# szpajder/dumpvdl2

Measured on AMD Instinct MI355X. Metric: IQ MS/s demodulated end-to-end, higher is better.
Workload: dtype f32

## Files before the change

dumpvdl2_amd/csrc/debug_hooks.inc:

```

static bool hip_ok(hipError_t e) { return e == hipSuccess; }
template<typename T> static bool dbg_up(const DevBuf<T> &d, const void *src, size_t bytes) { return hip_ok(hipMemcpy(d, src, bytes, hipMemcpyHostToDevice)); }
template<typename T> static bool dbg_up(const DevBuf<T> &d, const void *src) { return dbg_up(d, src, d.bytes()); }
template<typename T> static bool dbg_fill(const DevBuf<T> &d, int v) { return hip_ok(hipMemset(d, v, d.bytes())); }
template<typename T> static bool dbg_down(void *dst, const DevBuf<T> &d, size_t bytes) { return hip_ok(hipMemcpy(dst, d, bytes, hipMemcpyDeviceToHost)); }
template<typename T> static bool dbg_down(void *dst, const DevBuf<T> &d) { return dbg_down(dst, d, d.bytes()); }
static bool dbg_tables(const DevBuf<Tables> &d) { auto tab = std::make_unique<Tables>(); build_tables(*tab); return dbg_up(d, tab.get()); }

template<int K> static int prof_read(const void *symbol, unsigned long long *out, int reset) {
	unsigned long long h[64][K];
	if(hipMemcpyFromSymbol(h, symbol, sizeof h) != hipSuccess) return -3;
	for(int k = 0; k < K; k++) { out[k] = 0; for(int s = 0; s < 64; s++) out[k] += h[s][k]; }
	if(reset) { memset(h, 0, sizeof h); if(hipMemcpyToSymbol(symbol, h, sizeof h) != hipSuccess) return -3; }
	return 0;
}

extern "C" {

int vdl2hip_debug_live_resources(long long out[3]) {
	if(!out) return VDL2HIP_E_INVAL;
	for(int i = 0; i < 3; i++) out[i] = hostmem::g_live[i].load();
	return VDL2HIP_OK;
}

int vdl2hip_debug_option(vdl2hip_ctx *c, const char *name, long value) {
	if(!c || !name) return VDL2HIP_E_INVAL;
	OnDevice dev_guard(c);
	int r = collect_pending(c);
	if(r != VDL2HIP_OK && r != VDL2HIP_E_OVERFLOW) return r;
	if(strcmp(name, "no_fuse") == 0) { c->fuse_k2 = value == 0; return VDL2HIP_OK; }
	if(strcmp(name, "force_timeout") == 0) { c->debug_force_timeout = value != 0; return VDL2HIP_OK; }
	if(strcmp(name, "force_mismatch") == 0) { c->debug_force_mismatch = value != 0; return VDL2HIP_OK; }
	if(strcmp(name, "walk_ahead_below") == 0) { c->walk_ahead_below = (double)value; c->walk_ahead_auto = true; return VDL2HIP_OK; }
	if(strcmp(name, "walk_ahead") == 0) { if(value != 0 && value != 1) return VDL2HIP_E_INVAL; c->walk_ahead = (int)value; c->walk_ahead_auto = false; return VDL2HIP_OK; }
	if(strcmp(name, "exact_tier") == 0) { if(value != 0 && value != 1) return VDL2HIP_E_INVAL; c->debug_exact_tier = (int)value; return VDL2HIP_OK; }
	if(strcmp(name, "screen_all") == 0) { c->debug_screen_all = value != 0; return VDL2HIP_OK; }
	if(strcmp(name, "force_again") == 0) { c->debug_force_again = value != 0; return VDL2HIP_OK; }
	if(strcmp(name, "referee") == 0) { if(value && !c->d_refhist) return VDL2HIP_E_INVAL; c->referee = value != 0; return VDL2HIP_OK; }
	if(strcmp(name, "ref_warm") == 0) { if(value < 0 || value > c->ref_T - 4096) return VDL2HIP_E_INVAL; c->ref_warm = value; return VDL2HIP_OK; }
	return VDL2HIP_E_INVAL;
}

int vdl2hip_debug_exact_window_many(vdl2hip_ctx *c, uint32_t chan, int64_t n_lo, int64_t n_hi, uint32_t count, int64_t stride, float *ms) {
	if(!c || !c->d_refhist || chan >= (uint32_t)c->C || c->feed_no == 0 || count == 0 || count > 65536) return VDL2HIP_E_INVAL;
	OnDevice dev_guard(c);
	int r = collect_pending(c);
	if(r != VDL2HIP_OK && r != VDL2HIP_E_OVERFLOW) return r;
	DevBuf<int> d_out; std::vector<int> h(count, 0);
	if(!hip_ok(d_out.alloc(count))) return VDL2HIP_E_NOMEM;
	Event e0, e1;
	if(!hip_ok(e0.ensure()) || !hip_ok(e1.ensure())) return VDL2HIP_E_DEVICE;
	hipExtLaunchKernelGGL(k_ref_probe, dim3(count), dim3(64), 0, c->streams.front, e0, e1, 0, c->d_ref[(c->feed_no - 1) % kSlots].get(), (int)chan, c->C, n_lo, n_hi, stride, d_out.get());
	if(!hip_ok(hipStreamSynchronize(c->streams.front)) || !dbg_down(h.data(), d_out)) return VDL2HIP_E_DEVICE;
	if(ms) { float t = 0.f; (void)hipEventElapsedTime(&t, e0, e1); *ms = t; }
	int n = 0; for(int v : h) n += v;
	return n;
}
int vdl2hip_debug_scan_multi2(vdl2hip_ctx *c, const int32_t *chan, const int64_t *lo, const int64_t *hi, uint32_t count, int with_retry, float *ms) {
	if(!c || !c->d_refhist || c->feed_no == 0 || count == 0 || count > 65536 || !chan || !lo || !hi) return VDL2HIP_E_INVAL;
	OnDevice dev_guard(c);
	int r = collect_pending(c);
	if(r != VDL2HIP_OK && r != VDL2HIP_E_OVERFLOW) return r;
	std::vector<ScanReq> h(count);
	for(uint32_t i = 0; i < count; i++) { if(chan[i] < 0 || chan[i] >= c->C) return VDL2HIP_E_INVAL; h[i] = ScanReq{ chan[i], REF_CANDIDATE, lo[i], hi[i] }; }
	DevBuf<ScanReq> d_sq, d_rt; DevBuf<uint32_t> d_n;
	if(!hip_ok(d_sq.alloc(count)) || !hip_ok(d_n.alloc(2)) || !hip_ok(d_rt.alloc(kRetryScans))) return VDL2HIP_E_NOMEM;
	uint32_t before[8] = {0}, after[8] = {0};
	const uint32_t nn[2] = { count, 0u };
	Event e0, e1;
	if(!hip_ok(e0.ensure()) || !hip_ok(e1.ensure()) || !dbg_up(d_sq, h.data()) || !dbg_up(d_n, nn) || !dbg_down(before, c->d_refstats, sizeof before)) return VDL2HIP_E_DEVICE;
	RefChan *ref = c->d_ref[(c->feed_no - 1) % kSlots];
	launch_scans(c, c->streams.front, ref, 0xfffeu, d_sq, nullptr, d_n, count, c->k_total, with_retry ? d_rt.get() : nullptr, d_n + 1, e0, e1);
	if(!hip_ok(hipStreamSynchronize(c->streams.front)) || !dbg_down(after, c->d_refstats, sizeof after)) return VDL2HIP_E_DEVICE;
	if(ms) { float t = 0.f; (void)hipEventElapsedTime(&t, e0, e1); *ms = t; }
	return (int)(after[0] - before[0]);
}
int vdl2hip_debug_exact_window(vdl2hip_ctx *c, uint32_t chan, int64_t n_lo, int64_t n_hi) { return vdl2hip_debug_exact_window_many(c, chan, n_lo, n_hi, 1, 0, nullptr); }

int vdl2hip_debug_u8_levels(float out[512]) {
	DevBuf<float> d;
	if(!hip_ok(d.alloc(512))) return VDL2HIP_E_NOMEM;
	hipLaunchKernelGGL(k_u8_level_probe, dim3(1), dim3(256), 0, 0, d);
	return dbg_down(out, d) ? VDL2HIP_OK : VDL2HIP_E_DEVICE;
}

int vdl2hip_debug_s8_levels(float out[512]) {
	DevBuf<float> d;
	if(!hip_ok(d.alloc(512))) return VDL2HIP_E_NOMEM;
	hipLaunchKernelGGL(k_s8_level_probe, dim3(1), dim3(256), 0, 0, d);
	return dbg_down(out, d) ? VDL2HIP_OK : VDL2HIP_E_DEVICE;
}

int vdl2hip_debug_dpp_probe(const float in[64], float out[256]) {
	DevBuf<float> d_in, d_out;
	if(!hip_ok(d_in.alloc(64)) || !hip_ok(d_out.alloc(256))) return VDL2HIP_E_NOMEM;
	if(!dbg_up(d_in, in)) return VDL2HIP_E_DEVICE;
	hipLaunchKernelGGL(k_dpp_probe, dim3(1), dim3(64), 0, 0, (const float *)d_in, d_out);
	return dbg_down(out, d_out) ? VDL2HIP_OK : VDL2HIP_E_DEVICE;
}

int vdl2hip_debug_core_probe(int kind, const void *in, size_t n, void *out) {
	if(kind < 0 || kind >= PROBE_KINDS || !in || !out || n == 0 || n > (size_t)1 << 26) return VDL2HIP_E_INVAL;
	DevBuf<float> d_in, d_out; DevBuf<Tables> d_tab;
	if(!hip_ok(d_in.alloc(n * (size_t)core_probe_in_words(kind))) || !hip_ok(d_out.alloc(n * (size_t)core_probe_out_words(kind))) || !hip_ok(d_tab.alloc(1))) return VDL2HIP_E_NOMEM;
	if(!dbg_tables(d_tab) || !dbg_up(d_in, in) || !dbg_fill(d_out, 0)) return VDL2HIP_E_DEVICE;
	hipLaunchKernelGGL(k_core_probe, dim3((unsigned)((n + 255) / 256)), dim3(256), 0, 0, kind, (const float *)d_in, (uint32_t)n, d_out, (const Tables *)d_tab);
	return hip_ok(hipGetLastError()) && dbg_down(out, d_out) ? VDL2HIP_OK : VDL2HIP_E_DEVICE;
}

int vdl2hip_debug_burst_probe(int kind, const void *in, size_t n, unsigned grid, void *out, const uint32_t *freq, uint32_t nchan, const float *y, uint32_t ring_len,
		uint32_t cap_frames, uint32_t cap_pool, uint32_t guard_frames, uint32_t guard_pool, void *frames, uint8_t *pool, void *ctl, unsigned long long *cnt) {
	if(kind < 0 || kind >= BPROBE_KINDS || !in || n == 0 || n > (size_t)1 << 20 || grid == 0 || grid > 1024) return VDL2HIP_E_INVAL;
	const uint32_t nwaves = grid * (uint32_t)kBurstWaves;
	const bool burst = kind == BPROBE_BURST;
	size_t nin = 0, nout = 0;
	if(kind == BPROBE_WAVE) { nin = n * 64 * 4; nout = n * (size_t)kBProbeWaveOut * 4; }
// ... 407 lines not shown
```

dumpvdl2_amd/csrc/kernels.h:

```cpp
#pragma once
#include <hip/hip_runtime.h>
#include <type_traits>
#include "vdl2_core.h"
#include "design.h"

#ifndef VDL2_K1_UNROLL
#define VDL2_K1_UNROLL 5
#endif

#ifndef VDL2_K1_WAVES_PER_EU
#define VDL2_K1_WAVES_PER_EU 3
#endif

namespace vdl2 {

constexpr int kK1Unroll = VDL2_K1_UNROLL;
typedef float v2f __attribute__((ext_vector_type(2)));
typedef float v4f __attribute__((ext_vector_type(4)));

#ifndef VDL2_REF_PRIO
#define VDL2_REF_PRIO 3
#endif
#ifndef VDL2_K1_PRIO
#define VDL2_K1_PRIO 0
// ... 975 lines not shown
		const uint32_t r0 = (uint32_t)(nblk - 150) + tid;
		cf32 v[kFull + 1];
		#pragma unroll
		for(int k = 0; k <= kFull; k++) if(k < kFull || tid < kRest) v[k] = y[(r0 + kK3Threads * k) & a.mask];
		#pragma unroll
		for(int k = 0; k <= kFull; k++) if(k < kFull || tid < kRest) tile[tid + kK3Threads * k] = phase_fast(v[k]);
	} else {
		for(int j = tid; j < kK3Tile + 150; j += kK3Threads) {
			const int64_t t = nblk - 150 + j;
			tile[j] = (t < 0 || t >= a.k1) ? 0.f : phase_fast(y[(uint32_t)t & a.mask]);
		}
	}
	__syncthreads();
	const int s0 = 10 * kK3Share * (tid / 10) + tid % 10;
	constexpr int kEarlyPh = kScreenEarly + kK3Share - 1;
	float ph[kEarlyPh], d[kEarlyPh];
	#pragma unroll
	for(int k = 0; k < kEarlyPh; k++) ph[k] = tile[s0 + 10 * k];
	#pragma unroll
	for(int k = 1; k < kEarlyPh; k++) d[k] = ph[k] - ph[k - 1];
	#pragma unroll
	for(int q = 0; q < kK3Share; q++) {
		ScreenAcc acc;
		screen_begin(acc);
		screen_taps(&d[q], 1, kScreenEarly, acc);
		float ps = screen_value(acc, kScreenEarly);
		if(__any(ps < kScreenEarlyThr)) {
			float pl[kPreamble - kScreenEarly + 1], dl[kPreamble];
			#pragma unroll
			for(int j = 0; j <= kPreamble - kScreenEarly; j++) pl[j] = tile[s0 + 10 * (q + kScreenEarly - 1 + j)];
			#pragma unroll
			for(int j = 0; j < kPreamble - kScreenEarly; j++) dl[kScreenEarly + j] = pl[j + 1] - pl[j];
			screen_taps(dl, kScreenEarly, kPreamble, acc);
			ps = screen_value(acc, kPreamble);
		}
		verdict[s0 + 10 * q] = !(ps >= kScreenThr);
	}
	__syncthreads();
	constexpr int kWordsPerWave = (kK3Tile / 64) / (kK3Threads / 64);
	if(full_tile) {
		const int lane = tid & 63;
		const uint32_t w0 = (uint32_t)(nblk >> 6) + (uint32_t)__builtin_amdgcn_readfirstlane(tid >> 6) * kWordsPerWave;
		uint64_t *frow = a.flag + (size_t)c * (a.cap >> 6);
		const uint8_t *vrow = verdict + 64 * kWordsPerWave * (tid >> 6) + lane;
		const unsigned long long all = a.screen_all != 0 ? ~0ull : 0ull;
		uint8_t vb[kWordsPerWave];
		unsigned long long bits[kWordsPerWave];
		#pragma unroll
		for(int j = 0; j < kWordsPerWave; j++) vb[j] = vrow[64 * j];
		#pragma unroll
		for(int j = 0; j < kWordsPerWave; j++) bits[j] = __builtin_amdgcn_ballot_w64(vb[j] != 0) | all;
		if(lane == 0) {
			#pragma unroll
			for(int j = 0; j < kWordsPerWave; j++) frow[(w0 + j) & (a.mask >> 6)] = bits[j];
		}
		return;
	}
	#pragma unroll
	for(int j = 0; j < kWordsPerWave; j++) {
		const int word = (tid >> 6) * kWordsPerWave + j;
		const int64_t n = nblk + 64 * word + (tid & 63);
		const unsigned long long bits = __ballot(n < a.k1 && (verdict[64 * word + (tid & 63)] != 0 || a.screen_all != 0));
		if((tid & 63) == 0 && n < a.k1) a.flag[(size_t)c * (a.cap >> 6) + ((uint32_t)(n >> 6) & (a.mask >> 6))] = bits;
	}
}

constexpr int kK3bWordsPerLane = 4;
#ifdef VDL2_K3B_PROF
__device__ unsigned long long vdl2_k3b_prof[64][16];
#define K3B_BEGIN() unsigned k3b_t0_ = (unsigned)__builtin_readcyclecounter(), k3b_acc_[6] = {0, 0, 0, 0, 0, 0}, k3b_cnt_[3] = {0, 0, 0}
#define K3B_MARK(k) do { if(__builtin_amdgcn_readfirstlane(threadIdx.x >> 6) == 0) { const unsigned t_ = (unsigned)__builtin_readcyclecounter(); \
	k3b_acc_[k] += t_ - k3b_t0_; k3b_t0_ = t_; } } while(0)
#define K3B_COUNT(k, v) do { k3b_cnt_[k] += (unsigned)__builtin_amdgcn_readfirstlane((int)(v)); } while(0)
#define K3B_END() do { if(threadIdx.x == 0) { const int s_ = (blockIdx.x + blockIdx.y) & 63; for(int k_ = 0; k_ < 6; k_++) atomicAdd(&vdl2_k3b_prof[s_][k_], (unsigned long long)k3b_acc_[k_]); \
	atomicAdd(&vdl2_k3b_prof[s_][8], 1ull); for(int k_ = 0; k_ < 3; k_++) atomicAdd(&vdl2_k3b_prof[s_][9 + k_], (unsigned long long)k3b_cnt_[k_]); } } while(0)
#else
#define K3B_BEGIN() do {} while(0)
#define K3B_MARK(k) do {} while(0)
#define K3B_COUNT(k, v) do {} while(0)
#define K3B_END() do {} while(0)
#endif
template<bool FULL>
__global__ __launch_bounds__(256, 4) void k_sync_exact4(K3Args a) {
	if(blockIdx.x == 0 && blockIdx.y == 0 && threadIdx.x == 0) { reset_out_ctl(a.ctl, a.k5_waves); if(a.ref) *a.ref = a.refv; if(a.rq_n) { a.rq_n[0] = 0u; a.rq_n[1] = 0u; a.rq_n[2] = 0u; a.rq_n[4] = 0u; a.rq_n[5] = 0u; a.rq_n[6] = 0u; } }
	if(blockIdx.x == 0 && threadIdx.x == 0 && a.rq_flag) { a.rq_flag[blockIdx.y] = 0u; a.rq_bad[blockIdx.y].n = 0u; if(a.rq_flag2) a.rq_flag2[blockIdx.y] = 0u; }
	constexpr int kBack = 160, kSpan = kBack + 64;
	__shared__ float psh[4][64 + 6], fsh[4][64 + 6], esh[4][64 + 6], ash[4][64 + 6], bsh[4][64 + 6];
	__shared__ float phs[4][kSpan], e2s[4][kSpan];
	__shared__ uint64_t s_need[4][64 * kK3bWordsPerLane];
	__shared__ uint8_t s_fprev[4][64 * kK3bWordsPerLane];
	__shared__ uint16_t s_list[4][64 * kK3bWordsPerLane];
	const int c = blockIdx.y, lane = threadIdx.x & 63, wave = threadIdx.x >> 6;
	const cf32 *y = a.y + (size_t)c * a.cap;
	const uint64_t *flag = a.flag + (size_t)c * (a.cap >> 6);
	uint64_t *cand = a.cand + (size_t)c * (a.cap >> 6);
	const uint32_t wmask = a.mask >> 6;
	const Tables &T = *a.tab;
	const bool ref_on = a.ref != nullptr && a.ref_on != 0;
	const float ppm_thr = ref_on ? a.ppm_thr[c] : 0.f;
	const int64_t w0 = a.nbase >> 6, w1 = (a.k1 + 63) >> 6;
	const int64_t wb = w0 + ((int64_t)blockIdx.x * 4 + wave) * (64 * a.wpl);
	int nwork = 0;
	K3B_BEGIN();
	for(int g = 0; g < a.wpl; g++) {
		const int64_t w = wb + 64 * g + lane;
		uint64_t need = 0, fprev = 0, fpp = 0, f0 = 0;
		if(w < w1) {
			f0 = flag[(uint32_t)w & wmask];
			fprev = w > 0 ? flag[(uint32_t)(w - 1) & wmask] : 0ull;
			fpp = w > 1 ? flag[(uint32_t)(w - 2) & wmask] : 0ull;
			const uint64_t fnext = w + 1 < w1 ? flag[(uint32_t)(w + 1) & wmask] : 0ull;
			need = f0 | (f0 << 3) | (f0 >> 3) | (fprev >> 61) | (fnext << 61);
			const int64_t base = w << 6;
			if(a.k1 - 3 < base + 64) {
				const int64_t lo = a.k1 - 3 - base;
				need |= lo <= 0 ? ~0ull : (~0ull << lo);
			}
			if(a.k1 < base + 64) need &= (a.k1 - base <= 0) ? 0ull : (~0ull >> (64 - (a.k1 - base)));
			if(need == 0) cand[(uint32_t)w & wmask] = 0;
		}
		const uint64_t need_prev = fprev | (fprev << 3) | (fprev >> 3) | (fpp >> 61) | (f0 << 61);
		s_need[wave][64 * g + lane] = need; s_fprev[wave][64 * g + lane] = (uint8_t)(need_prev >> 58);
		const unsigned long long busy = __ballot(need != 0);
		if(need != 0) s_list[wave][nwork + __builtin_popcountll(busy & ((1ull << lane) - 1ull))] = (uint16_t)(64 * g + lane);
		nwork += __builtin_popcountll(busy);
	}
	WAVE_SYNC();
	K3B_MARK(0); if(wave == 0) K3B_COUNT(0, nwork);
	float *ps = psh[wave], *fs = fsh[wave], *es = esh[wave], *as = ash[wave], *bs = bsh[wave], *ph = phs[wave], *e2 = e2s[wave];
	#pragma unroll 1
	for(int it = 0; it < nwork; it++) {
		const int idx = (int)s_list[wave][it];
		const uint64_t needj = s_need[wave][idx];
		const uint32_t fprevj = s_fprev[wave][idx] & 63u;
		const int64_t wj = wb + idx, r0 = (wj << 6) - kBack;
		{
			cf32 yv[4]; bool in[4];
			#pragma unroll
			for(int k = 0; k < 4; k++) {
				const int64_t t = r0 + lane + 64 * k;
				in[k] = 64 * k + lane < kSpan && t >= 0 && t < a.k1;
				yv[k] = in[k] ? y[(uint32_t)t & a.mask] : cf32{0.f, 0.f};
			}
			#pragma unroll
			for(int k = 0; k < 4; k++) if(64 * k + lane < kSpan) {
				ph[64 * k + lane] = in[k] ? phase_of(yv[k]) : 0.f;
				e2[64 * k + lane] = in[k] ? yv[k].re * yv[k].re + yv[k].im * yv[k].im : -1.f;
			}
		}
		ps[6 + lane] = kPherrBig; if(lane < 6) ps[lane] = kPherrBig;
		WAVE_SYNC();
		K3B_MARK(1); if(wave == 0) { K3B_COUNT(1, __builtin_popcountll(needj) + __builtin_popcount(fprevj)); K3B_COUNT(2, 1 + (fprevj != 0)); }
		if(ref_on) {
			float ev[4];
			#pragma unroll
			for(int k = 0; k < 4; k++) {
				const int i = 64 * k + lane;
				ev[k] = 0.f;
				if(i >= 3 && i < kSpan) {
					const float m0 = e2[i], m1 = e2[i - 1], m2 = e2[i - 2], m3 = e2[i - 3];
					ev[k] = m0 < 0.f ? 0.f : ref_eps2_of(m0, fmaxf(m1, 0.f), fmaxf(m2, 0.f), fmaxf(m3, 0.f));
				}
			}
			WAVE_SYNC();
			#pragma unroll
			for(int k = 0; k < 4; k++) if(64 * k + lane < kSpan) e2[64 * k + lane] = ev[k];
			WAVE_SYNC();
		}
		K3B_MARK(2);
		#pragma unroll 1
		for(int round = 0; round < 2; round++) {
			const int bit = round == 0 ? lane : lane - 6;
			const bool todo = round == 0 ? ((needj >> lane) & 1ull) != 0 : (lane < 6 && ((fprevj >> lane) & 1u) && (wj << 6) + bit >= 0);
			if(todo) {
				const int i0 = bit + kBack - 150;
				float p[kPreamble];
				#pragma unroll
				for(int i = 0; i < kPreamble; i++) p[i] = ph[i0 + 10 * i];
				float pv, fv, E = 0.f, pa, pb;
				if(ref_on) sync_metric_ref(p, e2 + i0, 10, T, pv, fv, E, pa, pb, FULL);
				else { sync_metric(p, T, pv, fv); pa = pb = pv; }
				ps[6 + bit] = pv; fs[6 + bit] = fv; es[6 + bit] = E; as[6 + bit] = pa; bs[6 + bit] = pb;
			}
			K3B_MARK(3 + round);
		}
		WAVE_SYNC();
		const int64_t n = (wj << 6) + lane;
		const float p0 = ps[6 + lane], p3 = ps[3 + lane], p6 = ps[lane];
		int vd = 0;
		if(n >= 3 && n < a.k1) {
			if(!ref_on) vd = is_candidate(p3, p0) ? 1 : 0;
			else vd = ref_candidate_verdict(ref_pherr_range(p0, as[6 + lane], bs[6 + lane], es[6 + lane]), ref_pherr_range(p3, as[3 + lane], bs[3 + lane], es[3 + lane]), fs[3 + lane], es[3 + lane],
			                                ref_pherr_range(p6, as[lane], bs[lane], es[lane]), a.max_ppm, ppm_thr);
		}
		if((needj >> lane) & 1ull) a.pf[(size_t)c * a.cap + ((uint32_t)n & a.mask)] = cf32{ (vd & 2) ? -p0 : p0, fs[6 + lane] };
		const unsigned long long bits = __ballot((vd & 1) != 0);
		if(lane == 0) cand[(uint32_t)wj & wmask] = bits;
		if(a.pq) {
			const unsigned long long mk = __ballot((vd & 2) != 0 && ((needj >> lane) & 1ull) != 0);
			if(mk && lane == 0) {
				const int64_t nf = (wj << 6) + __builtin_ctzll(mk), nl = (wj << 6) + 63 - __builtin_clzll(mk);
				int64_t lo = (nf - kRefPre) & ~255ll, hi = (nl + kRefPost) | 255; if(lo < 0) lo = 0; if(hi > a.k1 - 1) hi = a.k1 - 1;
				const uint32_t i = atomicAdd(a.rq_n + 3, 1u);
				if(i < a.pq_cap) a.pq[i] = ScanReq{ c, REF_CANDIDATE, lo, hi };
			}
		}
		WAVE_SYNC();
		K3B_MARK(5);
	}
	K3B_END();
}

constexpr int kK3dEvals = 320;
constexpr int kK3dFlush = kK3dEvals - 64;
constexpr int kK3dList = kK3dFlush + 256;
constexpr int kK3dMinGroups = 2048;
constexpr int kK3dGroup = 4;
constexpr int kK3dRounds = 32;
static_assert(kK3dEvals >= 70 && kK3dEvals <= 512 && kK3dList * 70 < (1 << 20) && kK3dList < (1 << 11) && kK3dRounds * 256 <= (1 << 16),
              "tile map: 9 bits of word, 7 of position; list head: 11 bits of words, 21 of evaluations; 16 bits of word index");
#define K3D_BARRIER() do { __builtin_amdgcn_fence(__ATOMIC_RELEASE, "workgroup", "local"); __builtin_amdgcn_s_barrier(); __builtin_amdgcn_fence(__ATOMIC_ACQUIRE, "workgroup", "local"); } while(0)
template<bool FULL>
__global__ __launch_bounds__(256, 4) void k_sync_dense(K3Args a) {
	if(blockIdx.x == 0 && blockIdx.y == 0 && threadIdx.x == 0) { reset_out_ctl(a.ctl, a.k5_waves); if(a.ref) *a.ref = a.refv; if(a.rq_n) { a.rq_n[0] = 0u; a.rq_n[1] = 0u; a.rq_n[2] = 0u; a.rq_n[4] = 0u; a.rq_n[5] = 0u; a.rq_n[6] = 0u; } }
	if(blockIdx.x == 0 && threadIdx.x == 0 && a.rq_flag) { a.rq_flag[blockIdx.y] = 0u; a.rq_bad[blockIdx.y].n = 0u; if(a.rq_flag2) a.rq_flag2[blockIdx.y] = 0u; }
	__shared__ uint64_t s_need[kK3dList], s_cbits[kK3dList], s_mbits[kK3dList];
	__shared__ uint32_t s_end[kK3dList];
	__shared__ uint16_t s_word[kK3dList];
	__shared__ uint8_t s_fprev[kK3dList];
	__shared__ uint16_t s_map[kK3dEvals];
	__shared__ float s_res[5][kK3dEvals];
	__shared__ uint8_t s_neg[kK3dEvals];
	__shared__ uint32_t s_head, s_r1;
	__shared__ uint64_t s_flag[256 * kK3dGroup + 3];
	const int c = blockIdx.y, tid = threadIdx.x, lane = threadIdx.x & 63;
	const cf32 *y = a.y + (size_t)c * a.cap;
	const uint64_t *flag = a.flag + (size_t)c * (a.cap >> 6);
	uint64_t *cand = a.cand + (size_t)c * (a.cap >> 6);
	const uint32_t wmask = a.mask >> 6;
	const Tables &T = *a.tab;
	const bool ref_on = a.ref != nullptr && a.ref_on != 0;
	const float ppm_thr = ref_on ? a.ppm_thr[c] : 0.f;
	const int64_t w0 = a.nbase >> 6, w1 = (a.k1 + 63) >> 6;
	const int64_t wb = w0 + (int64_t)blockIdx.x * (256 * a.wpl);
	K3B_BEGIN();
	if(tid == 0) s_head = 0u;
	K3D_BARRIER();
	#pragma unroll 1
	for(int g = 0; g < a.wpl; g++) {
		if(g % kK3dGroup == 0) {
			const int ng = a.wpl - g < kK3dGroup ? a.wpl - g : kK3dGroup;
			for(int i = tid; i < 256 * ng + 3; i += 256) {
				const int64_t w = wb + 256 * g - 2 + i;
				s_flag[i] = w >= 0 && w < w1 ? flag[(uint32_t)w & wmask] : 0ull;
			}
			K3D_BARRIER();
		}
		{
			const int64_t w = wb + 256 * g + tid;
			const int fi = 256 * (g % kK3dGroup) + tid;
			uint64_t need = 0, fprev = 0, fpp = 0, f0 = 0;
			if(w < w1) {
				f0 = s_flag[fi + 2]; fprev = s_flag[fi + 1]; fpp = s_flag[fi];
				const uint64_t fnext = s_flag[fi + 3];
				need = f0 | (f0 << 3) | (f0 >> 3) | (fprev >> 61) | (fnext << 61);
				const int64_t base = w << 6;
				if(a.k1 - 3 < base + 64) {
					const int64_t lo = a.k1 - 3 - base;
					need |= lo <= 0 ? ~0ull : (~0ull << lo);
				}
				if(a.k1 < base + 64) need &= (a.k1 - base <= 0) ? 0ull : (~0ull >> (64 - (a.k1 - base)));
				if(need == 0) cand[(uint32_t)w & wmask] = 0;
			}
			const uint64_t need_prev = fprev | (fprev << 3) | (fprev >> 3) | (fpp >> 61) | (f0 << 61);
			const uint32_t fp6 = w > 0 ? (uint32_t)(need_prev >> 58) : 0u;
			const uint32_t cnt = need != 0 ? (uint32_t)__builtin_popcountll(need) + (uint32_t)__builtin_popcount(fp6) : 0u;
			const uint32_t inc = cnt << 11 | (need != 0 ? 1u : 0u);
			uint32_t incl = inc;
			#pragma unroll
			for(int d = 1; d < 64; d <<= 1) { const uint32_t o = (uint32_t)__shfl_up((int)incl, d); if(lane >= d) incl += o; }
			const uint32_t tot = (uint32_t)__shfl((int)incl, 63);
			uint32_t at = 0;
			if(lane == 0 && tot != 0) at = atomicAdd(&s_head, tot);
			at = (uint32_t)__shfl((int)at, 0) + incl - inc;
			if(need != 0) {
				const uint32_t r = at & 2047u;
				s_need[r] = need; s_fprev[r] = (uint8_t)fp6; s_word[r] = (uint16_t)(256 * g + tid); s_end[r] = (at >> 11) + cnt;
				s_cbits[r] = 0ull; s_mbits[r] = 0ull;
			}
		}
		K3D_BARRIER();
		const uint32_t head = s_head;
		K3D_BARRIER();
		const int nrec = (int)(head & 2047u);
		K3B_MARK(0);
		if((int)(head >> 11) < kK3dFlush && g + 1 < a.wpl) continue;
		K3B_COUNT(0, nrec); K3B_COUNT(1, head >> 11);
		#pragma unroll 1
		for(int r0 = 0; r0 < nrec; ) {
			const uint32_t e0 = r0 ? s_end[r0 - 1] : 0u;
			if(tid == 0) s_r1 = (uint32_t)r0 + 1u;
			K3D_BARRIER();
			{
				uint32_t best = 0;
				for(int r = r0 + 1 + tid; r < nrec && r < r0 + kK3dEvals; r += 256) if(s_end[r] - e0 <= (uint32_t)kK3dEvals) best = (uint32_t)r + 1u;
				if(best) atomicMax(&s_r1, best);
			}
// ... 213 lines not shown
	const cf32 *y; NfState *nf; EvalChunk *log; uint32_t *nlog; int64_t *sc_first; int64_t *sc_cum;
	NfFeed *feed; float *lpbuf; float *ring; uint32_t ring_mask; uint32_t cap, mask, cap_log, cap_comb, cap_hist; int32_t nchan;
};

constexpr int kNfWaves = 4;
__global__ __launch_bounds__(64 * kNfWaves, 4) void k_nf_prepare(K4bArgs a) {
	extern __shared__ __align__(16) unsigned char nf_lds[];
	NfShared *shw = reinterpret_cast<NfShared *>(nf_lds);
	const int wave = threadIdx.x >> 6, c = blockIdx.x * kNfWaves + wave;
	if(c >= a.nchan) return;
	EvalLog lg{ a.log + (size_t)c * a.cap_log, a.nlog + c };
	NfScratch sc{ a.sc_first + (size_t)c * (a.cap_comb + 1), a.sc_cum + (size_t)c * (a.cap_comb + 1) };
	nf_prepare(&a.nf[c], lg, sc, a.cap_comb, &a.feed[c], shw[wave]);
}

__global__ __launch_bounds__(64 * kNfWaves, 4) void k_nf_replay(K4bArgs a) {
	extern __shared__ __align__(16) unsigned char nf_lds[];
	NfShared *shw = reinterpret_cast<NfShared *>(nf_lds);
	const int c = blockIdx.y, wave = threadIdx.x >> 6;
	ChanView v{ a.y + (size_t)c * a.cap, nullptr, nullptr, a.mask };
	NfScratch sc{ a.sc_first + (size_t)c * (a.cap_comb + 1), a.sc_cum + (size_t)c * (a.cap_comb + 1) };
	const NfFeed fd = a.feed[c];
	for(int64_t g = (int64_t)blockIdx.x * kNfWaves + wave; fd.u0 + 1 + kNfGroup * g <= fd.u1; g += (int64_t)gridDim.x * kNfWaves) {
		nf_replay_group(v, sc, fd, g, a.lpbuf + (size_t)c * a.cap_hist, a.cap_hist, shw[wave]);
		WAVE_SYNC();
	}
}

__global__ __launch_bounds__(64 * kNfWaves, 4) void k_nf_finish(K4bArgs a) {
	extern __shared__ __align__(16) unsigned char nf_lds[];
	NfShared *shw = reinterpret_cast<NfShared *>(nf_lds);
	const int wave = threadIdx.x >> 6, c = blockIdx.x * kNfWaves + wave;
	if(c >= a.nchan) return;
	NfScratch sc{ a.sc_first + (size_t)c * (a.cap_comb + 1), a.sc_cum + (size_t)c * (a.cap_comb + 1) };
	nf_finish(&a.nf[c], sc, a.feed[c], a.lpbuf + (size_t)c * a.cap_hist, a.ring + (size_t)c * (a.ring_mask + 1), a.ring_mask, a.cap_hist, shw[wave]);
}

__device__ __forceinline__ void nf_all_body(const K4bArgs &a, unsigned char *lds, int block) {
	NfShared *shw = reinterpret_cast<NfShared *>(lds);
	const int wave = threadIdx.x >> 6, c = block * kNfWaves + wave;
	if(c >= a.nchan) return;
	ChanView v{ a.y + (size_t)c * a.cap, nullptr, nullptr, a.mask };
	EvalLog lg{ a.log + (size_t)c * a.cap_log, a.nlog + c };
	NfScratch sc{ a.sc_first + (size_t)c * (a.cap_comb + 1), a.sc_cum + (size_t)c * (a.cap_comb + 1) };
	nf_prepare(&a.nf[c], lg, sc, a.cap_comb, &a.feed[c], shw[wave]);
	WAVE_SYNC_GLOBAL();
	const NfFeed fd = a.feed[c];
	for(int64_t g = 0; fd.u0 + 1 + kNfGroup * g <= fd.u1; g++) {
		nf_replay_group(v, sc, fd, g, a.lpbuf + (size_t)c * a.cap_hist, a.cap_hist, shw[wave]);
		WAVE_SYNC();
	}
	WAVE_SYNC_GLOBAL();
	nf_finish(&a.nf[c], sc, fd, a.lpbuf + (size_t)c * a.cap_hist, a.ring + (size_t)c * (a.ring_mask + 1), a.ring_mask, a.cap_hist, shw[wave]);
}
__global__ __launch_bounds__(64 * kNfWaves, 4) void k_nf_all(K4bArgs a) {
	extern __shared__ __align__(16) unsigned char nf_lds[];
	nf_all_body(a, nf_lds, (int)blockIdx.x);
}

struct K5Args {
	const cf32 *y; const Tables *tab; unsigned long long *cnt;
	const Burst *bursts; const uint32_t *nb_chan; uint32_t cap_bursts_chan; int32_t nchan;
	OutFrame *frames; uint8_t *pool; OutCtl *ctl; const uint32_t *freq;
	uint32_t cap, mask;
	RefChan *ref;
	uint32_t ref_launch;
	BurstDefer df;
};

constexpr int kScanLanes = 16, kScanProd = 8, kScanBlock = 64, kScanRow = kScanBlock + 4;
#ifndef VDL2_SCAN_WAVES
#define VDL2_SCAN_WAVES 11
#endif
constexpr int kScanWaves = VDL2_SCAN_WAVES;
struct ScanShared {
	alignas(16) float buf[2][2][kScanLanes][kScanRow];
	int64_t s_beg[kScanLanes], len[kScanLanes], n_lo[kScanLanes], n_hi[kScanLanes];
	uint32_t dphi[kScanLanes]; int32_t chan[kScanLanes], kind[kScanLanes]; uint32_t flags[kScanLanes];
	int64_t lmax, smin;
	v4f lut[256];
};
template<int FMT, int OS>
__global__ __launch_bounds__(64 * kScanWaves) void k_ref_scan_multi(RefChan *rp, uint32_t launch, const ScanReq *sq, const RefReq *rq, const uint32_t *n_ptr, uint32_t cap, int64_t k_end,
                      ScanReq *retry_q, uint32_t *retry_n, uint32_t retry_cap, int32_t warm_mul) {
#if VDL2_DEVICE_PASS
	#pragma clang fp contract(off)
	__shared__ ScanShared sh;
	constexpr int BLK = OS ? (kScanBlock / (OS ? OS : 1)) * OS : kScanBlock;
	const uint32_t ntot = *n_ptr < cap ? *n_ptr : cap;
	const uint32_t base = blockIdx.x * (uint32_t)kScanLanes;
	if(base >= ntot) return;
	const int wave = __builtin_amdgcn_readfirstlane(threadIdx.x >> 6), lane = threadIdx.x & 63;
	const int os = rp->os, npiece = rp->npiece;
	const uint32_t mask = rp->mask, cap_y = rp->cap;
	const int64_t warm = rp->warm * (int64_t)(warm_mul > 1 ? warm_mul : 1);
	int64_t ps0[kRefPieces], pn[kRefPieces]; const void *pp[kRefPieces];
	#pragma unroll
	for(int j = 0; j < kRefPieces; j++) { ps0[j] = j < npiece ? rp->piece[j].s0 : 0; pn[j] = j < npiece ? rp->piece[j].n : 0; pp[j] = j < npiece ? rp->piece[j].p : nullptr; }
	const float A0 = rp->A0, A1 = rp->A1, A2 = rp->A2;
	uint32_t *stats = rp->stats;
	static_assert(kScanLanes == 16, "four lanes of the first wavefront per request");
	if(threadIdx.x < 64) {
		const int r = threadIdx.x & (kScanLanes - 1), part = threadIdx.x >> 4;
		int64_t n_lo = 0, n_hi = -1, s_beg = 0, len = 0; int c = 0, kind = 0; uint32_t fl = 0;
		if(base + r < ntot && npiece > 0) {
			if(sq) { const ScanReq q = sq[base + r]; c = q.chan; kind = q.kind; n_lo = q.lo; n_hi = q.hi; }
			else { const RefReq q = rq[base + r]; c = q.chan; kind = q.kind; ref_request_window(q, k_end, n_lo, n_hi); }
			const int64_t in_end = ps0[npiece - 1] + pn[npiece - 1];
			if(n_lo < 0) n_lo = 0;
			if(kind == REF_STALE) kind = REF_CANDIDATE;
			bool go = n_hi >= n_lo;
			if(go) {
				const int64_t last = in_end / os - 1;
				n_lo &= ~255ll;
				if((n_hi | 255) <= last) n_hi |= 255; else if(n_hi < last) n_hi = last;
				const unsigned long long *done = rp->done + (size_t)c * kRefCache;
				const uint32_t ndv = rp->done_n[c], nd = ndv < (uint32_t)kRefCache ? ndv : (uint32_t)kRefCache;
				bool hit = false;
				for(uint32_t i = (uint32_t)part; i < nd; i += 4u) {
					const unsigned long long e = __hip_atomic_load(done + i, __ATOMIC_RELAXED, __HIP_MEMORY_SCOPE_AGENT);
					const int64_t lo = (int64_t)(e >> 32) << 8, hi = lo + ((int64_t)((e >> 16) & 0xffffull) << 8) + 255;
					hit = hit || (lo <= n_lo && n_hi <= hi && ref_entry_visible((uint32_t)(e & 0xffffull), launch));
				}
				int h = hit ? 1 : 0;
				h |= __shfl_xor(h, 16);
				h |= __shfl_xor(h, 32);
				hit = h != 0;
				if(hit) { if(part == 0) atomicAdd(stats + 1, 1u); go = false; }
			}
			if(go) {
				const int64_t s_end = (int64_t)os * (n_hi + 1);
				s_beg = (int64_t)os * n_lo - warm;
				bool refuse = in_end < s_end;
				if(s_beg < 0) s_beg = 0;
				else {
					if(ps0[0] > s_beg) { fl |= 2u; s_beg = (ps0[0] + os - 1) / os * os; }
					if(s_beg > 0 && (int64_t)os * n_lo - s_beg < rp->warm / 4) refuse = true;
				}
				if(refuse) { if(part == 0) atomicAdd(stats + 2, 1u); go = false; }
				else {
					s_beg -= s_beg % os;
					len = s_end - s_beg;
					if(rp->mix[c]) fl |= 1u;
				}
			}
			if(!go) len = 0;
		}
		if(part == 0) {
			sh.s_beg[r] = s_beg; sh.len[r] = len; sh.n_lo[r] = n_lo; sh.n_hi[r] = n_hi; sh.chan[r] = c; sh.kind[r] = kind; sh.flags[r] = fl;
			sh.dphi[r] = len ? rp->dphi[c] : 0u;
		}
	}
	__syncthreads();
	if(threadIdx.x < kScanLanes) {
		const int r = threadIdx.x;
		bool dup = false;
		for(int q = 0; q < r; q++) dup = dup || (sh.len[q] && sh.chan[q] == sh.chan[r] && sh.n_lo[q] == sh.n_lo[r] && sh.n_hi[q] >= sh.n_hi[r]);
		if(dup && sh.len[r]) { atomicAdd(stats + 1, 1u); sh.len[r] = 0; }
	}
	__syncthreads();
	if(threadIdx.x == 0) {
		int64_t m = 0, lo = INT64_MAX;
		for(int r = 0; r < kScanLanes; r++) { m = sh.len[r] > m ? sh.len[r] : m; if(sh.len[r] > 0 && sh.s_beg[r] < lo) lo = sh.s_beg[r]; }
		sh.lmax = m; sh.smin = lo;
		for(int r = 0; r < kScanLanes; r++) if(sh.len[r] <= 0) sh.s_beg[r] = lo;
	}
	__syncthreads();
	const int64_t lmax = sh.lmax;
	if(lmax <= 0) return;
	__builtin_amdgcn_s_setprio(3);
	const int64_t nblk = ((lmax + BLK - 1) / BLK + 2) / 4 * 4 + 1;
	for(int i = threadIdx.x; i < 256; i += blockDim.x) sh.lut[i] = ((ref_gf4 *)rp->lut)[i];
	__syncthreads();

	auto uni64 = [](int64_t v) -> int64_t { return (int64_t)(((uint64_t)(uint32_t)__builtin_amdgcn_readfirstlane((int)(v >> 32)) << 32) | (uint32_t)__builtin_amdgcn_readfirstlane((int)v)); };
	auto lds_barrier = [&]() { asm volatile("s_waitcnt lgkmcnt(0)\n\ts_barrier" ::: "memory"); };
	constexpr int NQ = kScanLanes / kScanProd;
	const int pidx = kScanWaves == 1 + kScanProd ? wave - 1 : (wave == 0 || (wave & 3) == 0) ? -1 : wave - 1 - (wave > 4) - (wave > 8);
	if(wave > 0 && pidx < 0) return;
	if(wave > 0) {
#if defined(VDL2_SCAN_EXP) && VDL2_SCAN_EXP == 3
		__builtin_amdgcn_s_setprio(1);
#endif
		const uint8_t *q_ptr[NQ]; uint32_t q_pend[NQ], q_ph0[NQ], q_len[NQ], q_dphi[NQ];
		int64_t q_beg[NQ];
		float pre[NQ], pim[NQ];
		constexpr int PF = 4;
		uint32_t wq[PF][NQ], wq2[PF][NQ];
		constexpr int SB = FMT == 2 ? 8 : FMT == 1 ? 4 : 2;
// ... 110 lines not shown
		static_assert(BLK % CH == 0 && CH % OS == 0, "chunks of whole decimation periods");
		(void)cnt;
		for(int64_t b = 0; b < nblk; b++) {
			const float *row = &sh.buf[b & 1][comp][r][0];
			v4f cur[NV], nxt[NV];
			#pragma unroll
			for(int j = 0; j < NV; j++) cur[j] = *reinterpret_cast<const v4f *>(row + 4 * j);
			#pragma unroll
			for(int j0 = 0; j0 < BLK; j0 += CH) {
				if(j0 + CH < BLK) {
					#pragma unroll
					for(int j = 0; j < NV; j++) nxt[j] = *reinterpret_cast<const v4f *>(row + j0 + CH + 4 * j);
				}
				#pragma unroll
				for(int j = 0; j < CH; j++) {
#if defined(VDL2_SCAN_EXP) && VDL2_SCAN_EXP == 2
					if(j) continue;
#endif
					const float m = b1 * y1;
					const float sm = m + t2;
					t2 = b2 * y1;
					y1 = cur[j >> 2][j & 3] + sm;
					if((j + 1) % OS == 0) {
						if(k_out >= my_lo && k_out <= my_hi) yout[2 * ((uint32_t)k_out & mask)] = y1;
						if(k_out == my_lo) { w_y1 = y1; w_t2 = t2; }
						k_out++;
					}
				}
				#pragma unroll
				for(int j = 0; j < NV; j++) cur[j] = nxt[j];
			}
			lds_barrier();
		}
	} else {
	constexpr int kChunk = 16;
	for(int64_t b = 0; b < nblk; b++) {
		const float *row = &sh.buf[b & 1][comp][r][0];
		v4f cur[kChunk / 4], nxt[kChunk / 4];
		#pragma unroll
		for(int j = 0; j < kChunk / 4; j++) cur[j] = *reinterpret_cast<const v4f *>(row + 4 * j);
		#pragma unroll
		for(int j0 = 0; j0 < BLK; j0 += kChunk) {
			if(j0 + kChunk < BLK) {
				#pragma unroll
				for(int j = 0; j < kChunk / 4; j++) nxt[j] = *reinterpret_cast<const v4f *>(row + j0 + kChunk + 4 * j);
			}
			#pragma unroll
			for(int j = 0; j < kChunk; j++) {
				const float m = b1 * y1;
				const float sm = m + t2;
				t2 = b2 * y1;
				y1 = cur[j >> 2][j & 3] + sm;
				if(__builtin_expect(++cnt == os, 0)) {
					cnt = 0;
					if(k_out >= my_lo && k_out <= my_hi) yout[2 * ((uint32_t)k_out & mask)] = y1;
					if(k_out == my_lo) { w_y1 = y1; w_t2 = t2; }
					k_out++;
				}
			}
			#pragma unroll
			for(int j = 0; j < kChunk / 4; j++) cur[j] = nxt[j];
		}
		lds_barrier();
	}
	}
	bool unmet = __float_as_uint(__shfl_xor(w_y1, 32)) != __float_as_uint(w_y1) || __float_as_uint(__shfl_xor(w_t2, 32)) != __float_as_uint(w_t2);
	unmet = unmet || __shfl_xor((int)unmet, kScanLanes) != 0;
	if(lane < kScanLanes && sh.len[r] > 0) {
		const int c = sh.chan[r];
		const int64_t n_lo = sh.n_lo[r], n_hi = sh.n_hi[r];
		bool listed = false;
		if(unmet && retry_q) {
			const uint32_t k = atomicAdd(retry_n, 1u);
			if(k < retry_cap) { retry_q[k] = ScanReq{ c, sh.kind[r], n_lo, n_hi }; listed = true; atomicAdd(stats + 10, 1u); }
		}
		if(unmet && !listed) atomicAdd(stats + 9, 1u);
		const uint32_t i = listed ? 0u : atomicAdd(rp->done_n + c, 1u);
		int64_t len = (n_hi - n_lo) >> 8; if(len > 0xffff) len = 0xffff;
		if(((n_hi + 1) & 255) != 0) len -= 1;
		if(listed) len = -1;
		if(len >= 0) __hip_atomic_store(rp->done + (size_t)c * kRefCache + (i % (uint32_t)kRefCache), ((unsigned long long)(n_lo >> 8) << 32) | ((unsigned long long)len << 16) | (unsigned long long)(launch & 0xffffu), __ATOMIC_RELAXED, __HIP_MEMORY_SCOPE_AGENT);
		atomicAdd(stats + 0, 1u); atomicAdd(stats + 4 + sh.kind[r], 1u);
		if(sh.flags[r] & 2u) atomicAdd(stats + 3, 1u);
	}
#else
	(void)rp; (void)launch; (void)sq; (void)rq; (void)n_ptr; (void)cap; (void)k_end;
#endif
}

#ifndef VDL2_K5_WAVES
#define VDL2_K5_WAVES 2
#endif
constexpr int kBurstWaves = VDL2_K5_WAVES;
constexpr int kK5MaxChan = 1024;
enum { BPROBE_WAVE = 0, BPROBE_RS, BPROBE_BURST, BPROBE_KINDS };
constexpr int kBProbeWaveOut = 68, kBProbeRsStride = 256;
struct BurstProbeArgs {
	uint32_t n; const Tables *tab; OutCtl *ctl;
	const uint32_t *win; uint32_t *wout;
	const uint8_t *rin; uint8_t *rout; int32_t *rret;
	const Burst *bursts; const uint32_t *freq; const cf32 *y; uint32_t cap, mask; unsigned long long *cnt; OutFrame *frames; uint8_t *pool;
};
__global__ __launch_bounds__(64 * kBurstWaves) void k_burst_probe_wave(BurstProbeArgs a) {
	extern __shared__ __align__(16) unsigned char k5_lds[];
	BurstShared &sh = reinterpret_cast<BurstShared *>(k5_lds)[threadIdx.x >> 6];
	const uint32_t wave_id = blockIdx.x * kBurstWaves + (threadIdx.x >> 6), nwaves = gridDim.x * kBurstWaves;
	burst_shared_init(*a.tab, wave_id, a.ctl, sh);
	for(uint32_t i = wave_id; i < a.n; i += nwaves) {
		const uint32_t *x = a.win + (size_t)i * 64;
		uint32_t *o = a.wout + (size_t)i * kBProbeWaveOut;
		WAVE_FOR(l)
			sh.lanek[l] = x[l]; sh.flag_err[l] = (int32_t)x[l];
		WAVE_END
		const int first = wave_first_flag(sh.flag_err), count = wave_count_flags(sh.flag_err);
		const uint32_t mn = wave_min64(sh.lanek);
		WAVE_SYNC();
		const uint32_t total = wave_excl_scan64(sh.lanek);
		WAVE_FOR(l)
			o[2 + l] = sh.lanek[l];
			if(l == 0) { o[0] = (uint32_t)first; o[1] = (uint32_t)count; o[66] = total; o[67] = mn; }
		WAVE_END
		WAVE_SYNC();
	}
}
__global__ __launch_bounds__(64 * kBurstWaves) void k_burst_probe_rs(BurstProbeArgs a) {
	extern __shared__ __align__(16) unsigned char k5_lds[];
	BurstShared &sh = reinterpret_cast<BurstShared *>(k5_lds)[threadIdx.x >> 6];
	const uint32_t wave_id = blockIdx.x * kBurstWaves + (threadIdx.x >> 6), nwaves = gridDim.x * kBurstWaves;
	burst_shared_init(*a.tab, wave_id, a.ctl, sh);
	for(uint32_t i = wave_id; i < a.n; i += nwaves) {
		const uint8_t *x = a.rin + (size_t)i * kBProbeRsStride;
		uint8_t *o = a.rout + (size_t)i * kBProbeRsStride;
		WAVE_FOR(l)
			for(int j = l; j < kRsN; j += 64) sh.tab[j] = x[j];
		WAVE_END
		[[clang::always_inline]] rs_decode_row(sh.tab, (int)x[kRsN], sh);
		WAVE_FOR(l)
			for(int j = l; j < kRsN; j += 64) o[j] = sh.tab[j];
			if(l == 0) a.rret[i] = sh.u_ret;
		WAVE_END
		WAVE_SYNC();
	}
}

__device__ __forceinline__ void burst_body(const K5Args &a, unsigned char *k5_lds, uint32_t block, uint32_t nblocks) {
	if((threadIdx.x >> 6) >= kBurstWaves) return;
	BurstShared &sh = reinterpret_cast<BurstShared *>(k5_lds)[threadIdx.x >> 6];
	uint32_t *bb = reinterpret_cast<uint32_t *>(k5_lds + sizeof(BurstShared) * kBurstWaves) + (size_t)(threadIdx.x >> 6) * (kK5MaxChan + 1);
	const int lane = threadIdx.x & 63;
	const uint32_t wave_id = block * kBurstWaves + (threadIdx.x >> 6);
	uint32_t total = 0;
	for(int c0 = 0; c0 < a.nchan; c0 += 64) {
		const uint32_t v = c0 + lane < a.nchan ? a.nb_chan[c0 + lane] : 0u;
		uint32_t inc = v;
		#pragma unroll
		for(int d = 1; d < 64; d <<= 1) { const uint32_t o = __shfl_up(inc, d); if(lane >= d) inc += o; }
		if(c0 + lane < a.nchan) bb[c0 + lane] = total + inc - v;
		total += __shfl(inc, 63);
	}
	if(lane == 0) { bb[a.nchan] = total; if(wave_id == 0 && a.df.pass != 2) a.ctl->nbursts = total; }
	WAVE_SYNC();
	if(a.df.pass == 2) {
		const uint32_t nd = *a.df.dq_n < a.df.dq_cap ? *a.df.dq_n : a.df.dq_cap;
		if(wave_id >= nd) return;
		burst_shared_init(*a.tab, wave_id, a.ctl, sh, true);
		for(uint32_t i = wave_id; i < nd; i += nblocks * kBurstWaves) {
			const uint32_t g = a.df.dq[i];
			int lo = 0, hi = a.nchan;
			while(hi - lo > 1) { const int mid = (lo + hi) >> 1; if(bb[mid] <= g) lo = mid; else hi = mid; }
			const int c = lo;
			const Burst b = a.bursts[(size_t)c * a.cap_bursts_chan + (g - bb[c])];
			ChanView v{ a.y + (size_t)c * a.cap, nullptr, nullptr, a.mask, a.ref, c, a.ref_launch };
			decode_burst(b, a.freq[c], *a.tab, v, a.cnt + (size_t)c * kNumCounters, a.frames, a.pool, a.ctl, sh, &a.df, g);
			WAVE_SYNC();
		}
		burst_reserve_done(a.frames, sh);
		return;
	}
	if(wave_id >= total) {
		const uint32_t slot = wave_id * (uint32_t)kResSlots + (uint32_t)lane;
		if(lane < kResSlots && slot < a.ctl->cap_frames) { OutFrame &f = a.frames[slot]; f.chan = -1; f.len = 0; f.pool_off = 0; f.nf_upd = 0; }
		return;
	}
	burst_shared_init(*a.tab, wave_id, a.ctl, sh);
	for(uint32_t g = wave_id; g < total; g += nblocks * kBurstWaves) {
		int lo = 0, hi = a.nchan;
		while(hi - lo > 1) { const int mid = (lo + hi) >> 1; if(bb[mid] <= g) lo = mid; else hi = mid; }
		const int c = lo;
		const Burst b = a.bursts[(size_t)c * a.cap_bursts_chan + (g - bb[c])];
		ChanView v{ a.y + (size_t)c * a.cap, nullptr, nullptr, a.mask, a.ref, c, a.ref_launch };
		decode_burst(b, a.freq[c], *a.tab, v, a.cnt + (size_t)c * kNumCounters, a.frames, a.pool, a.ctl, sh, a.df.pass ? &a.df : nullptr, g);
		WAVE_SYNC();
	}
	burst_reserve_done(a.frames, sh);
}

__global__ __launch_bounds__(256, 4) void k_burst(K5Args a) {
	extern __shared__ __align__(16) unsigned char k5_lds[];
	burst_body(a, k5_lds, blockIdx.x, gridDim.x);
}

static_assert(kNfWaves >= kBurstWaves, "a workgroup of the joint launch holds either kind");
__global__ __launch_bounds__(64 * kNfWaves, 4) void k_nf_burst(K4bArgs nf, K5Args k5, uint32_t nf_blocks) {
	extern __shared__ __align__(16) unsigned char back_lds[];
	if(blockIdx.x < nf_blocks) nf_all_body(nf, back_lds, (int)blockIdx.x);
	else burst_body(k5, back_lds, blockIdx.x - nf_blocks, gridDim.x - nf_blocks);
}

constexpr int kFrameWaves = 4, kFrameChunk = 16;
constexpr int kMailFrames = 8, kMailPool = 2048;
struct OutMail { OutCtl ctl; OutFrame frames[kMailFrames]; uint8_t pool[kMailPool]; };
__global__ __launch_bounds__(64 * kFrameWaves) void k_frame_finish(OutFrame *frames, const uint8_t *pool, OutMail *mail, const Tables *tab,
		unsigned long long *acnt, const float *ring, uint32_t ring_mask, OutFrame *frames_out, uint8_t *pool_out) {
	__shared__ FrameShared shw[kFrameWaves];
	__shared__ uint32_t s_off[kFrameWaves][64];
	OutCtl *ctl = &mail->ctl;
	const int wave = threadIdx.x >> 6, lane = threadIdx.x & 63;
	const uint32_t n = ctl->nframes < ctl->cap_frames ? ctl->nframes : ctl->cap_frames;
	const uint32_t first = (blockIdx.x * kFrameWaves + wave) * (uint32_t)kFrameChunk;
	if(first >= n) return;
	FrameShared &sh = shw[wave];
	bool init = false;
	for(uint32_t c0 = first; c0 < n; c0 += gridDim.x * kFrameWaves * (uint32_t)kFrameChunk) {
		const uint32_t i = c0 + (uint32_t)lane;
		const bool valid = lane < kFrameChunk && i < n && frames[i].chan >= 0;
		const uint32_t padded = valid ? (frames[i].len + 3u) & ~3u : 0u;
		const unsigned long long vm = __ballot(valid);
		if(!vm) continue;
		uint32_t inc = padded;
		#pragma unroll
		for(int d = 1; d < kFrameChunk; d <<= 1) { const uint32_t o = __shfl_up(inc, d); if(lane >= d) inc += o; }
		s_off[wave][lane] = inc - padded;
		const uint32_t tot = __shfl(inc, kFrameChunk - 1), cnt = (uint32_t)__popcll(vm);
		uint32_t slot0 = 0, off0 = 0;
		if(lane == 0) { slot0 = atomicAdd(&ctl->nvalid, cnt); off0 = atomicAdd(&ctl->pool_out_used, tot); }
		if(!init) { frame_shared_init(*tab, sh); init = true; }
		slot0 = __shfl(slot0, 0); off0 = __shfl(off0, 0);
		WAVE_SYNC();
		uint32_t rank = 0;
		for(unsigned long long m = vm; m; m &= m - 1, rank++) {
			const int l = __builtin_ctzll(m);
			OutFrame &f = frames[c0 + (uint32_t)l];
			const int c = f.chan;
			finish_frame(f, pool, *tab, acnt + (size_t)c * kNumAvlcCounters, ring + (size_t)c * (ring_mask + 1), ring_mask, sh);
			const uint32_t len = f.len, src_off = f.pool_off, dst_off = off0 + s_off[wave][l], slot = slot0 + rank;
			const bool in_mail = slot < (uint32_t)kMailFrames && dst_off + len <= (uint32_t)kMailPool;
			if(lane == 0) { OutFrame g = f; g.pool_off = dst_off; frames_out[slot] = g; if(slot < (uint32_t)kMailFrames) mail->frames[slot] = g; }
			for(uint32_t k = (uint32_t)lane; k < len; k += 64) {
				const uint8_t o = k < (uint32_t)sizeof sh.buf ? sh.buf[k] : pool[src_off + k];
				pool_out[dst_off + k] = o;
				if(in_mail) mail->pool[dst_off + k] = o;
			}
			WAVE_SYNC();
		}
	}
}

__global__ __launch_bounds__(64 * kBurstWaves) void k_burst_probe(BurstProbeArgs a) {
	extern __shared__ __align__(16) unsigned char k5_lds[];
	BurstShared &sh = reinterpret_cast<BurstShared *>(k5_lds)[threadIdx.x >> 6];
	const uint32_t wave_id = blockIdx.x * kBurstWaves + (threadIdx.x >> 6), nwaves = gridDim.x * kBurstWaves;
	burst_shared_init(*a.tab, wave_id, a.ctl, sh);
	for(uint32_t i = wave_id; i < a.n; i += nwaves) {
		const Burst b = a.bursts[i];
		ChanView v{ a.y + (size_t)i * a.cap, nullptr, nullptr, a.mask };
		decode_burst(b, a.freq[b.chan], *a.tab, v, a.cnt + (size_t)b.chan * kNumCounters, a.frames, a.pool, a.ctl, sh);
		WAVE_SYNC();
	}
	burst_reserve_done(a.frames, sh);
}

}
```

dumpvdl2_amd/csrc/vdl2_core.h:

```cpp
#pragma once
#include <cstdint>
#include <cmath>

#if defined(__HIP_DEVICE_COMPILE__)
#define VDL2_DEVICE_PASS 1
#else
#define VDL2_DEVICE_PASS 0
#endif

#if defined(__HIPCC__)
#define VDL2_HD __host__ __device__ inline
#else
#define VDL2_HD inline
#endif

#if VDL2_DEVICE_PASS
#define VDL2_LANE() ((int)(threadIdx.x & 63))
#define WAVE_SYNC() do { __builtin_amdgcn_fence(__ATOMIC_ACQ_REL, "wavefront"); __builtin_amdgcn_wave_barrier(); } while(0)
#define WAVE_SYNC_GLOBAL() do { __builtin_amdgcn_fence(__ATOMIC_ACQ_REL, "workgroup"); __builtin_amdgcn_wave_barrier(); } while(0)
#define WAVE_FOR(l) { const int l = VDL2_LANE();
#define WAVE_END } WAVE_SYNC();
#define LANE0 if(VDL2_LANE() == 0) {
#define LANE0_END } WAVE_SYNC();
#else
// ... 2005 lines not shown
		for(int i = 0; i < kRsPar; i++) root[i] = 0;
		for(int q = 0; q < 4; q++)
			for(int l = 0; l < 64; l++)
				if((sh.rs_hits[l] >> q) & 1u) {
					const int i = 1 + l + 64 * q;
					for(int c = 0; c < kRsPar; c++) if(c == count) root[c] = i;
					count++;
				}
		int ret;
		if(deg != count) ret = -1;
		else {
			int lam[kRsPar + 1], syn[kRsPar], om[kRsPar];
			for(int i = 0; i <= kRsPar; i++) lam[i] = sh.rs_lam[i];
			for(int i = 0; i < kRsPar; i++) syn[i] = LOG[sh.syn[i]];
			const int deg_om = deg - 1;
			for(int i = 0; i < kRsPar; i++) {
				int acc = 0;
				for(int j = 0; j < kRsPar; j++)
					if(i <= deg_om && j <= i) { const int sy = syn[i - j < 0 ? 0 : i - j]; if(sy != A0 && lam[j] != A0) acc ^= EXP[sy + lam[j]]; }
				om[i] = LOG[acc];
			}
			for(int c = 0; c < kRsPar; c++) {
				if(c < count) {
					const int rt = root[c];
					int num1 = 0, den = 0;
					for(int i = 0; i < kRsPar; i++) if(i <= deg_om && om[i] != A0) num1 ^= EXP[gf_mod255(om[i] + (i * rt) % 255)];
					const int num2 = EXP[gf_mod255((rt * (FCR - 1)) % 255 + 255)];
					const int top = (deg < kRsPar - 1 ? deg : kRsPar - 1) & ~1;
					for(int i = 0; i <= 4; i += 2) if(i <= top && lam[i + 1] != A0) den ^= EXP[gf_mod255(lam[i + 1] + (i * rt) % 255)];
					if(num1 != 0) row[rt - 1] ^= EXP[gf_mod255(LOG[num1] + LOG[num2] + 255 - LOG[den])];
				}
			}
			ret = count;
		}
		sh.u_ret = ret;
	LANE0_END
}


constexpr int kResSlots = 8, kResPool = 1024;
VDL2_HD uint32_t burst_reserve_initial_frames(uint32_t nwaves) { return nwaves * (uint32_t)kResSlots; }
VDL2_HD uint32_t burst_reserve_initial_pool(uint32_t nwaves) { return nwaves * (uint32_t)kResPool; }
VDL2_HD void burst_reserve_release(OutFrame *frames, BurstShared &sh) {
	for(uint32_t i = 0; i < sh.res_nslot; i++) {
		const uint32_t slot = sh.res_slot + i;
		if(slot < sh.res_capf) { OutFrame &f = frames[slot]; f.chan = -1; f.len = 0; f.pool_off = 0; f.nf_upd = 0; }
	}
	sh.res_nslot = 0; sh.res_npool = 0;
}
VDL2_HD void burst_reserve_done(OutFrame *frames, BurstShared &sh) {
	LANE0
		burst_reserve_release(frames, sh);
	LANE0_END
}

VDL2_HD void burst_shared_init(const Tables &T, uint32_t wave, const OutCtl *ctl, BurstShared &sh, bool no_reserve = false) {
	WAVE_FOR(l)
		for(int i = l; i < 512; i += 64) sh.gf_exp[i] = T.gf_exp[i];
		for(int i = l; i < 256; i += 64) sh.gf_log[i] = T.gf_log[i];
	WAVE_END
	WAVE_FOR(l)
		if(l < 2) {
			const int n_era = 2 + 2 * l, npar = kRsPar - n_era;
			int lam[kRsPar + 1];
			for(int i = 0; i <= kRsPar; i++) lam[i] = 0;
			lam[0] = 1;
			lam[1] = sh.gf_exp[gf_mod255(254 - (kRsK + npar))];
			for(int i = 1; i < n_era; i++) {
				const int u = gf_mod255(254 - (kRsK + npar + i));
				for(int j = i + 1; j > 0; j--) { const int lg = sh.gf_log[lam[j - 1]]; if(lg != 255) lam[j] ^= sh.gf_exp[u + lg]; }
			}
			for(int i = 0; i <= kRsPar; i++) sh.gam[l][i] = (uint8_t)lam[i];
		}
		if(l == 0) {
			sh.res_slot = wave * (uint32_t)kResSlots; sh.res_nslot = (uint32_t)kResSlots; sh.res_off = wave * (uint32_t)kResPool; sh.res_npool = (uint32_t)kResPool;
			if(no_reserve) { sh.res_nslot = 0; sh.res_npool = 0; }
			sh.res_capf = ctl->cap_frames; sh.res_capp = ctl->cap_pool;
		}
	WAVE_END
}

constexpr int kRefPieceBits = 10;
struct ScanReq { int32_t chan, kind; int64_t lo, hi; };
struct BurstDefer { uint32_t *dq, *dq_n; uint32_t dq_cap; ScanReq *sq; uint32_t *sq_n; uint32_t sq_cap; int32_t pass; };

VDL2_HD __attribute__((always_inline)) void decode_burst(const Burst &b, uint32_t freq, const Tables &T, const ChanView &v, unsigned long long *cnt,
		OutFrame *frames, uint8_t *pool, OutCtl *ctl, BurstShared &sh, const BurstDefer *df = nullptr, uint32_t tag = 0) {
	const uint32_t octets = b.tl_bits / 8 + (b.tl_bits % 8 != 0);
	uint32_t nblk = octets / kRsK, last = octets % kRsK;
	uint32_t fec = nblk * kRsPar;
	if(last != 0) nblk++;
	fec += (uint32_t)fec_octets_for(last);
	if(last == 0) last = kRsK;
	const int npar_last = fec_octets_for(last);
	const int nsym = b.nsym;
	K5_BEGIN();

	const int per_lane = (nsym + 63) / 64;
	const bool ref_on = v.ref != nullptr;
	float vdphi = b.vdphi, ppm = b.ppm;
	const float verr = fabsf(b.vdphi_err);
	WAVE_FOR(l)
		float pw = 0.f; int neg = 0; float qmin = kRefBig;
		const int m0 = l * per_lane, m1 = m0 + per_lane < nsym ? m0 + per_lane : nsym;
		float prev = b.prev_phi0, pim2 = 0.f, pm2 = 0.f;
		if(m0 < nsym) {
			const int64_t tp = m0 > 0 ? b.t_first + (int64_t)(m0 - 1) * kSpsDec : b.prev_n;
			if(tp >= 0) { const cf32 yp = v.Y(tp); if(m0 > 0) prev = phase_of(yp); pim2 = ref_inv_mag2(yp); pm2 = yp.re * yp.re + yp.im * yp.im; }
			else if(tp == -2) pim2 = kRefBig;
		}
		for(int mb = m0; mb < m1; mb += 4) {
			cf32 yv[4];
			for(int q = 0; q < 4; q++) yv[q] = mb + q < m1 ? v.Y(b.t_first + (int64_t)(mb + q) * kSpsDec) : cf32{0.f, 0.f};
			for(int q = 0; q < 4 && mb + q < m1; q++) {
				const float cur = phase_of(yv[q]);
				int neg1 = 0;
				const int idx = slice_symbol(cur, prev, vdphi, neg1);
				uint8_t sy = (uint8_t)((idx ^ (idx >> 1)) | (neg1 << 6));
				neg += neg1;
				const float m2 = yv[q].re * yv[q].re + yv[q].im * yv[q].im;
				if(ref_on) {
					const float im2 = ref_inv_mag2(yv[q]), a2 = fmaxf(m2, pm2);
					const float d = ref_symbol_dist(cur, prev, vdphi) - verr - 2e-6f, w = sqrtf(im2) + sqrtf(pim2);
					if(d <= kRefKappa * sqrtf(a2) * w) sy |= 0x80;
					const float qv = w > 0.f ? d / w : kRefBig;
					qmin = qv < qmin ? qv : qmin;
					pim2 = im2; pm2 = m2;
				}
				sh.sym[mb + q] = sy;
				prev = cur;
				pw += m2;
			}
		}
		sh.pw[l] = pw; sh.neg[l] = neg; sh.qmin[l] = qmin;
	WAVE_END
	LANE0
		double s = 0.0; int negs = 0;
		for(int l = 0; l < 64; l++) { s += (double)sh.pw[l]; negs += sh.neg[l]; }
		sh.u_pwr = (float)(s / (double)nsym);
		sh.u_negs = negs;
	LANE0_END
	if(ref_on) {
		const float athr = kRefKappa * 2.0f * sqrtf(sh.u_pwr);
		WAVE_FOR(l)
			const int m0 = l * per_lane, m1 = m0 + per_lane < nsym ? m0 + per_lane : nsym;
			uint32_t first = 0xffffffffu, last = 0u;
			if(m0 < nsym) {
				const bool again = sh.qmin[l] <= athr;
				float prev = b.prev_phi0, pim2 = 0.f;
				if(again) {
					const int64_t tp = m0 > 0 ? b.t_first + (int64_t)(m0 - 1) * kSpsDec : b.prev_n;
					if(tp >= 0) { const cf32 yp = v.Y(tp); if(m0 > 0) prev = phase_of(yp); pim2 = ref_inv_mag2(yp); }
					else if(tp == -2) pim2 = kRefBig;
				}
				for(int m = m0; m < m1; m++) {
					if(again) {
						const cf32 y = v.Y(b.t_first + (int64_t)m * kSpsDec);
						const float cur = phase_of(y), im2 = ref_inv_mag2(y);
						if(ref_symbol_dist(cur, prev, vdphi) - verr - 2e-6f <= athr * (sqrtf(im2) + sqrtf(pim2))) sh.sym[m] |= 0x80;
						prev = cur; pim2 = im2;
					}
					if(sh.sym[m] & 0x80) { if(first == 0xffffffffu) first = (uint32_t)m; last = (uint32_t)m; }
				}
			}
			sh.lanek[l] = first; sh.lanet[l] = ~last;
		WAVE_END
		const uint32_t mfirst = wave_min64(sh.lanek), mlast = ~wave_min64(sh.lanet);
		WAVE_SYNC();
		if(mfirst != 0xffffffffu) {
			const bool redo_slope = b.vdphi_err > 0.f;
			const int64_t t_lo = mfirst > 0 ? b.t_first + (int64_t)(mfirst - 1) * kSpsDec : (b.prev_n >= 0 ? b.prev_n : b.t_first);
			const int64_t hi = b.t_first + (int64_t)mlast * kSpsDec;
			const int64_t s_lo = b.sync_sample - kRefPre;
			const int64_t w_lo = (redo_slope && s_lo < t_lo) ? (s_lo < 0 ? 0 : s_lo) : t_lo;
			const int64_t P0 = w_lo >> kRefPieceBits;
			const bool wide = (hi >> kRefPieceBits) - P0 >= 128;
			const int pass = df ? df->pass : 0;
			LANE0
				uint32_t pm[4] = { 0u, 0u, 0u, 0u };
				if(wide) pm[0] = 1u;
				else {
					if(redo_slope) for(int64_t q = ((s_lo < 0 ? 0 : s_lo) >> kRefPieceBits) - P0; q <= (b.sync_sample >> kRefPieceBits) - P0; q++) if(q >= 0 && q < 128) pm[q >> 5] |= 1u << (q & 31);
					for(int l = 0; l < 64; l++) {
						const uint32_t first = sh.lanek[l], last = ~sh.lanet[l];
						if(first == 0xffffffffu) continue;
						const int64_t a_ = first > 0 ? b.t_first + (int64_t)(first - 1) * kSpsDec : (b.prev_n >= 0 ? b.prev_n : b.t_first);
						const int64_t b_ = b.t_first + (int64_t)last * kSpsDec;
						for(int64_t q = (a_ >> kRefPieceBits) - P0; q <= (b_ >> kRefPieceBits) - P0; q++) if(q >= 0 && q < 128) pm[q >> 5] |= 1u << (q & 31);
					}
				}
				for(int i = 0; i < 4; i++) sh.u_pm[i] = pm[i];
				sh.u_defer = 0;
				if(pass == 1) {
#if VDL2_DEVICE_PASS
					const uint32_t i = atomicAdd(df->dq_n, 1u);
#else
					const uint32_t i = (*df->dq_n)++;
#endif
					if(i < df->dq_cap) {
						df->dq[i] = tag; sh.u_defer = 1;
						uint32_t np = 0;
						for(int q = 0; q < 4; q++) np += (uint32_t)popc32(pm[q]);
#if VDL2_DEVICE_PASS
						uint32_t j = atomicAdd(df->sq_n, np);
#else
						uint32_t j = *df->sq_n; *df->sq_n += np;
#endif
						for(int q = 0; q < 128; q++) {
							if(!((pm[q >> 5] >> (q & 31)) & 1u)) continue;
							int64_t lo_ = (P0 + q) << kRefPieceBits, hi_ = ((P0 + q + 1) << kRefPieceBits) - 1;
							if(wide) { lo_ = w_lo; hi_ = hi; }
							if(lo_ < w_lo) lo_ = w_lo;
							if(hi_ > hi) hi_ = hi;
							if(j < df->sq_cap) df->sq[j] = ScanReq{ v.ref_chan, REF_SYMBOLS, lo_, hi_ };
							j++;
						}
					}
				}
			LANE0_END
			if(sh.u_defer) { K5_END(); return; }
			bool ok = true;
			{
				for(int q = 0; q < 128 && ok; ) {
					if(!((sh.u_pm[q >> 5] >> (q & 31)) & 1u)) { q++; continue; }
					int q1 = q;
					if(pass != 2) while(q1 + 1 < 128 && ((sh.u_pm[(q1 + 1) >> 5] >> ((q1 + 1) & 31)) & 1u)) q1++;
					int64_t lo_ = (P0 + q) << kRefPieceBits, hi_ = ((P0 + q1 + 1) << kRefPieceBits) - 1;
					if(wide) { lo_ = w_lo; hi_ = hi; }
					if(lo_ < w_lo) lo_ = w_lo;
					if(hi_ > hi) hi_ = hi;
					ok = ref_exact_window(v, lo_, hi_, sh.xw, REF_SYMBOLS);
					q = q1 + 1;
				}
			}
			if(ok && redo_slope) {
				float *phs = reinterpret_cast<float *>(sh.keptw);
				WAVE_FOR(l)
					if(l < 16) phs[l] = v.Phi(b.sync_sample - 3 - 150 + 10 * l);
				WAVE_END
				LANE0
					float p_, f_;
					sync_metric(phs, T, p_, f_);
					sh.u_pwr_db = f_;
				LANE0_END
				vdphi = sh.u_pwr_db; ppm = ppm_of(vdphi, freq);
				WAVE_SYNC();
			}
			WAVE_FOR(l)
				int negd = 0;
				if(ok) for(uint32_t m = mfirst + (uint32_t)l; m <= mlast; m += 64) {
					if(!(sh.sym[m] & 0x80)) continue;
					const int64_t t = b.t_first + (int64_t)m * kSpsDec;
					const float cur = v.Phi(t);
					const float prev = m > 0 ? v.Phi(t - kSpsDec) : (b.prev_n >= 0 ? v.Phi(b.prev_n) : b.prev_phi0);
					int neg = 0;
					const int idx = slice_symbol(cur, prev, vdphi, neg);
					negd += neg - (int)((sh.sym[m] >> 6) & 1);
					sh.sym[m] = (uint8_t)(idx ^ (idx >> 1));
				}
				sh.neg[l] = negd;
			WAVE_END
			LANE0
				int d = 0;
				for(int l = 0; l < 64; l++) d += sh.neg[l];
				sh.u_negs += d;
			LANE0_END
		}
	}
	LANE0
		if(sh.u_negs > 0) VDL2_CNT_ADD(cnt, CNT_SLICER_NEG_IDX, sh.u_negs);
	LANE0_END

	K5_MARK(0);
	const uint32_t ntot = octets + fec;
	WAVE_FOR(l)
		for(uint32_t i = l; i < ntot; i += 64) {
			uint32_t o = 0, bit0 = kHdrBits + 8 * i;
			for(int j = 0; j < 8; j++) {
				uint32_t bb = bit0 + j;
				o |= (((uint32_t)sh.sym[bb / 3] >> (2 - bb % 3)) & 1u) << j;
			}
			sh.oct[i] = (uint8_t)(o ^ T.prbs_oct[i]);
		}
		for(uint32_t i = l; i < nblk * 256; i += 64) sh.tab[i] = 0;
	WAVE_END

	K5_MARK(1);
	uint32_t fec_rows = nblk; if(npar_last == 0) fec_rows--;
	uint32_t flast = fec % kRsPar; if(flast == 0) flast = kRsPar;
	WAVE_FOR(l)
		for(uint32_t i = l; i < octets; i += 64) {
			uint32_t row, col;
			if(i < last * nblk) { col = i / nblk; row = i - col * nblk; }
			else { uint32_t r = i - last * nblk; col = last + r / (nblk - 1); row = r % (nblk - 1); }
			sh.tab[row * 256 + col] = sh.oct[i];
		}
		for(uint32_t i = l; i < fec; i += 64) {
			uint32_t row, col;
			if(i < flast * fec_rows) { col = i / fec_rows; row = i - col * fec_rows; }
			else { uint32_t r = i - flast * fec_rows; col = flast + r / (fec_rows - 1); row = r % (fec_rows - 1); }
			sh.tab[row * 256 + kRsK + col] = sh.oct[octets + i];
		}
	WAVE_END

	K5_MARK(2);
	int fec_fixed = 0; int failed = 0;
	for(uint32_t r = 0; r < nblk && !failed; r++) {
		const int npar = (r == nblk - 1) ? npar_last : kRsPar;
		uint8_t *row = &sh.tab[r * 256];
		rs_decode_row(row, npar, sh);
		LANE0
			VDL2_CNT_ADD(cnt, CNT_BLOCKS_PROCESSED, 1);
			if(sh.u_ret < 0) VDL2_CNT_ADD(cnt, CNT_ERR_FEC_BAD, 1);
// ... 194 lines not shown
```

dumpvdl2_amd/csrc/vdl2hip.hip:

```cpp
#include <hip/hip_runtime.h>
#include <hip/hip_ext.h>
#include <algorithm>
#include <cmath>
#include <cstddef>
#include <cstdio>
#include <cstdlib>
#include <cstring>
#include <deque>
#include <map>
#include <memory>
#include <mutex>
#include <new>
#include <string>
#include <vector>
#include "../../include/vdl2hip.h"
#include "kernels.h"
#include "resample.h"
#include "resample_design.h"
#include "spectrum.h"
#include "spectrum_design.h"
#include "activity.h"
#include "txlog.h"
#include "capture.h"
#include "tables.h"
#include "hostmem.h"

using namespace vdl2;
using hostmem::DevBuf; using hostmem::PinnedBuf; using hostmem::Event;

static_assert(VDL2HIP_NUM_COUNTERS == kNumCounters, "counter enum out of sync");

namespace {

struct HostFrame {
	OutFrame f;
	std::shared_ptr<std::vector<uint8_t>> pool;
	const uint8_t *octets() const { return pool && f.pool_off + f.len <= pool->size() ? pool->data() + f.pool_off : nullptr; }
};

#ifndef VDL2_K1_RUN
#define VDL2_K1_RUN 2
#endif
constexpr int kRun = VDL2_K1_RUN;
constexpr int kRunGeneric = 2;
constexpr int kHistory = 65536;
constexpr int kNumEv = 12;
constexpr int kColdParts = 4;
constexpr size_t kColdMinBytes = 8u << 20;
constexpr uint32_t kRetryScans = 64;
constexpr uint32_t kPreScans = 4096;
constexpr uint32_t kDeferBursts = 4096, kDeferScans = 8192, kDeferScansMax = 1u << 17;
static uint32_t defer_scans_for(int64_t D, int C) {
	const uint64_t want = (uint64_t)(D > 0 ? D : 0) * (uint64_t)C / 8192u;
	const uint64_t cap = std::min<uint64_t>(kDeferScansMax, std::max<uint64_t>(kDeferScans, want));
	return (uint32_t)((cap + 63) / 64 * 64);
}
constexpr int kSidePre = 3, kSideBurst = 2;
struct StreamSet {
	int device = -1; hipStream_t front = nullptr, copy = nullptr, out = nullptr, back = nullptr, nf = nullptr, pre[kSidePre] = {}, burst[kSideBurst] = {};
	template<typename F> void each(F f) { for(hipStream_t *p : { &front, &copy, &out, &back, &nf }) f(*p); for(auto &x : pre) f(x); for(auto &x : burst) f(x); }
};
constexpr int kSlots = VDL2HIP_MAX_DRAIN_LAG + 1;

}

struct KernelTimes {
	Event ev[4]; int n = 0; bool armed = false;
	bool arm(bool timed) { armed = timed; if(timed) for(auto &x : ev) if(x.ensure() != hipSuccess) armed = false; return armed; }
	hipEvent_t e(int i) const { return armed ? (hipEvent_t)ev[i] : (hipEvent_t) nullptr; }
	void launched(int pairs) { n = armed ? pairs : 0; }
	void collect(double &ms) {
		for(int i = 0; i < n; i++) { float t = 0.f; if(hipEventElapsedTime(&t, ev[2 * i], ev[2 * i + 1]) == hipSuccess) ms += t; else (void)hipGetLastError(); }
		n = 0;
	}
};

struct TapRead {
	Event last; bool queued = false; hipStream_t rd = nullptr; PinnedBuf land;
	~TapRead() { if(rd) (void)hipStreamDestroy(rd); }
	hipError_t mark(hipStream_t front) { const hipError_t e = hipEventRecord(last, front); if(e == hipSuccess) queued = true; return e; }
	hipError_t fetch(void *dst_host, const void *src_dev, size_t bytes) {
		hipError_t e = hipStreamWaitEvent(rd, last, 0);
		if(e == hipSuccess) e = hipMemcpyAsync(dst_host, src_dev, bytes, hipMemcpyDeviceToHost, rd);
		return e == hipSuccess ? hipStreamSynchronize(rd) : e;
	}
};

struct OutSlot {
	DevBuf<Burst> d_bursts; DevBuf<uint32_t> d_nbchan;
	DevBuf<OutFrame> d_frames; DevBuf<uint8_t> d_pool;
	DevBuf<OutMail> d_mail; OutCtl *d_ctl = nullptr;
	DevBuf<OutFrame> d_frames_out; DevBuf<uint8_t> d_pool_out;
	DevBuf<EvalChunk> d_log; DevBuf<uint32_t> d_nlog;
	DevBuf<uint32_t> d_dq; DevBuf<ScanReq> d_sq;
	DevBuf<RefReq> d_rq; DevBuf<uint32_t> d_rqn, d_rqflag; DevBuf<RefBad> d_rqbad;
	DevBuf<ScanReq> d_retry;
	DevBuf<ScanReq> d_pq; Event ev_pre;
	PinnedBuf h_mail;
	Event done, ev_front, ev_walk, ev_nf, ev[kNumEv];
	bool pending = false, ev_valid = false, fused = false; int ev_level = 0;
	uint64_t seq = 0;
	int64_t back_D = 0, back_k0 = 0;
	bool k1_timed = false;
	bool prescan = false;
	bool rest_pending = false, has_chk = false; int nseg = 1; int64_t seglen = 0; K4Args k4{}; SpecOut *d_spec_of = nullptr;
	Event ev_stitch, ev_chk; DevBuf<uint32_t> d_rqflag2;
	KernelTimes rs_t, mon_t, act_t, cap_t, txl_t;
	struct { DevBuf<CapHdr> d_hdr; CapRec *d_rec = nullptr; DevBuf<CapPlan> d_plan; DevBuf<uint64_t> d_tot; DevBuf<cf32> d_pool; PinnedBuf h_mail; } cap;
	bool cap_on = false;
	struct { DevBuf<TxHdr> d_hdr; TxRec *d_rec = nullptr; PinnedBuf h_mail; } txl;
	bool txl_on = false;
	unsigned k5_waves = 0; bool small = false;
};

struct vdl2hip_ctx {
	vdl2hip_cfg cfg{};
	int C = 0, chan_first = 0, os = 0, fmt = 0, run = kRun, cr = 1;
	int in_fmt = 0;
	struct {
		bool on = false; uint32_t L = 0, M = 0, T = 0, span_cap = 0; size_t lds = 0; bool taps_lds = false;
		DevBuf<float> d_taps; DevBuf<float2> d_tail[2]; int tail_sel = 0;
		DevBuf<float2> d_out[kSlots]; uint64_t cap = 0;
		uint64_t first[kSlots] = {}, count[kSlots] = {};
		uint64_t n_in = 0, n_out = 0;
	} rs;
	struct {
		bool on = false; uint32_t nfft = 0, window = 0, stride = 1, log2n = 0, threads = 0; size_t lds = 0;
		double sum_w = 0.0, enbw = 0.0; uint64_t pos = 0, segments = 0; uint32_t ncarry = 0; int carry_sel = 0;
		struct { DevBuf<float> d_w; DevBuf<float2> d_tw, d_carry[2]; DevBuf<double> d_rows, d_acc; } buf;
		TapRead tap; double kernel_ms = 0.0;
	} mon;
	struct {
		bool on = false; uint32_t B = 0, H = 0, S = 0; float thr_dbfs = 0.f, thr = 0.f; int64_t k_on = 0; uint64_t bins = 0;
		struct { DevBuf<float> d_series, d_carry[2], d_edges; DevBuf<ActChan> d_acc; DevBuf<ActState> d_st; } buf;
		int carry_sel = 0; TapRead tap; double kernel_ms = 0.0;
	} act;
	struct CapItem { vdl2hip_burst r; std::shared_ptr<std::vector<float>> iq; };
	struct {
		bool on = false; uint32_t pre = 0, post = 0, flags = 0, pool = 0;
		uint64_t bursts = 0, iq_samples = 0, iq_dropped = 0; double kernel_ms = 0.0;
		PinnedBuf stage;
		std::deque<CapItem> queue;
	} capt;
	struct TxFrame { int64_t sync_sample, burst_ord; bool ok; };
	struct {
		bool on = false; uint32_t pool = 0, flags = 0;
		uint64_t transmissions = 0, decoded = 0, dropped = 0, matched = 0, unmatched = 0; double kernel_ms = 0.0;
		struct { DevBuf<TxState> d_st; DevBuf<uint32_t> d_cnt; PinnedBuf stage; } buf;
		std::deque<vdl2hip_tx> queue; std::vector<std::deque<TxFrame>> wait;
	} txl;
	uint64_t dmax = 0;
	bool specialised = false;
	std::vector<uint32_t> freqs, dphi, all_freqs;
	LpfCoeffs lpf{};
	BlockForm bf{};
	StreamSet streams;
	DevBuf<BlockForm> d_bf; DevBuf<Lut4> d_lut; DevBuf<Tables> d_tab;
	DevBuf<uint32_t> d_dphi, d_freq; DevBuf<float> d_ppmthr;
	DevBuf<uint8_t> d_in[kSlots]; Event ev_copied[kSlots]; size_t in_cap = 0;
	hipEvent_t pinned_pending = nullptr;
	struct { int n = 0; uint64_t samples[kColdParts] = {}; Event ev[kColdParts]; } cold;
	PinnedBuf stage;
	DevBuf<uint8_t> d_carry[2]; int carry_sel = 0; uint32_t ncarry = 0;
	DevBuf<cf32> d_y, d_pf; DevBuf<uint64_t> d_cand, d_flag;
	uint32_t cap = 0;
	DevBuf<float4> d_segend; uint32_t nseg_cap = 0;
	DevBuf<float4> d_qpow;
	DevBuf<float4> d_tcarry[2]; int tcarry_sel = 0;
	DevBuf<unsigned long long> d_segpub; DevBuf<uint32_t> d_synctmo; bool fuse_k2 = true;
	DevBuf<WalkState> d_ws; DevBuf<unsigned long long> d_cnt, d_acnt;
	unsigned long long *d_wcnt = nullptr;
	DevBuf<NfState> d_nf; DevBuf<int64_t> d_scfirst, d_sccum;
	DevBuf<float> d_nfring, d_lpbuf; DevBuf<NfFeed> d_nffeed; uint32_t cap_log = 0, cap_comb = 0, cap_hist = 0, nf_ring = 0;
	uint32_t cap_bursts_chan = 0;
	DevBuf<SpecOut> d_spec[2]; DevBuf<uint32_t> d_segstats; int seg_max = 1; int64_t seg_min = 16384;
	OutSlot slot[kSlots];
	uint64_t feed_no = 0; int drain_lag = 0;
	OutCtl ctl_template{};
	bool pooled = false;
	bool avlc_filter = false, failed = false; int debug_force_timeout = 0, debug_force_again = 0, debug_exact_tier = 1, debug_screen_all = 0;
	bool referee = true; bool ref_prescan = false;    int64_t ref_warm = 3 << 16 , ref_T = 0; DevBuf<uint8_t> d_refhist; uint64_t ref_cap = 0, ref_wp = 0;
	struct HistPiece { int64_t s0, n; uint64_t pos; }; std::vector<HistPiece> ref_pieces;
	DevBuf<WalkState> d_ws_snap[2], d_ws_tmp; DevBuf<unsigned long long> d_cnt_snap[2], d_cnt_tmp; uint32_t rq_cap = 8192; uint32_t sq_alloc = 8192;
	int walk_ahead = 1; bool walk_ahead_auto = true; double walk_ahead_below = 1.1e8; int debug_force_mismatch = 0;
	int ref_retry_mul = 2;
	DevBuf<RefChan> d_ref[kSlots]; DevBuf<unsigned long long> d_refdone; DevBuf<uint32_t> d_refdonen, d_refstats; DevBuf<uint8_t> d_mix;
	std::vector<uint64_t> statsd_prev;
	std::vector<HostFrame> queue;
	int64_t k_total = 0; uint64_t n_total = 0;
	int profiling = 0;
	vdl2hip_stats stats{};
};

#define HIPCHK(expr) do { hipError_t e_ = (expr); if(e_ != hipSuccess) { \
	fprintf(stderr, "vdl2hip: %s failed: %s (%s:%d)\n", #expr, hipGetErrorString(e_), __FILE__, __LINE__); return VDL2HIP_E_DEVICE; } } while(0)

constexpr int kFmtS8 = 3;
static int fmt_code(uint32_t sample_fmt) {
	switch(sample_fmt) {
		case VDL2HIP_FMT_U8: case VDL2HIP_FMT_S16LE: case VDL2HIP_FMT_CF32: return (int)sample_fmt;
		case VDL2HIP_FMT_S8: return kFmtS8;
		default: return -1;
	}
}
static size_t sample_bytes(int fmt) { return fmt == VDL2HIP_FMT_CF32 ? 8 : fmt == VDL2HIP_FMT_S16LE ? 4 : 2; }

struct OnDevice {
	int prev = -1; bool switched = false;
	explicit OnDevice(const vdl2hip_ctx *c) { if(c && hipGetDevice(&prev) == hipSuccess && prev != c->cfg.device) switched = hipSetDevice(c->cfg.device) == hipSuccess; }
	~OnDevice() { if(switched) (void)hipSetDevice(prev); }
};

#define LAUNCH_EV(kernel, grid, block, stream, e0, e1, ...) hipExtLaunchKernelGGL(kernel, grid, block, 0u, stream, e0, e1, 0, __VA_ARGS__)
#define EV(i) (prof_all ? (hipEvent_t)ev[i] : (hipEvent_t) nullptr)

template<int OS, int R>
static void launch_chanfir(vdl2hip_ctx *c, const K1Args &a, int cr, size_t lds, hipEvent_t e0, hipEvent_t e1) {
	const int groups = (c->C + cr - 1) / cr;
	K1Args b = a;
	b.gy = (groups + 3) / 4;
	const int nseg8 = (a.seg1 - a.seg0 + 7) / 8 * 8;
	dim3 grid((unsigned)(nseg8 * b.gy)), block(256);
	if(c->fmt == VDL2HIP_FMT_CF32) {
		switch(cr) {
			case 4: hipExtLaunchKernelGGL((k_chanfir<OS, R, 4, false, true>), grid, block, (uint32_t)lds, c->streams.front, e0, e1, 0, b); break;
			case 2: hipExtLaunchKernelGGL((k_chanfir<OS, R, 2, false, true>), grid, block, (uint32_t)lds, c->streams.front, e0, e1, 0, b); break;
			default: hipExtLaunchKernelGGL((k_chanfir<OS, R, 1, false, true>), grid, block, (uint32_t)lds, c->streams.front, e0, e1, 0, b); break;
		}
		return;
	}
	switch(cr) {
		case 4:
			if constexpr(OS == 20 || OS == 10) { if(c->fmt == VDL2HIP_FMT_U8) { hipExtLaunchKernelGGL((k_chanfir<OS, R, 4, true>), grid, block, (uint32_t)lds, c->streams.front, e0, e1, 0, b); break; } }
			if constexpr(OS == 20 || OS == 10) { if(c->fmt == kFmtS8) { hipExtLaunchKernelGGL((k_chanfir<OS, R, 4, false, false, true>), grid, block, (uint32_t)lds, c->streams.front, e0, e1, 0, b); break; } }
			hipExtLaunchKernelGGL((k_chanfir<OS, R, 4>), grid, block, (uint32_t)lds, c->streams.front, e0, e1, 0, b); break;
		case 2: hipExtLaunchKernelGGL((k_chanfir<OS, R, 2>), grid, block, (uint32_t)lds, c->streams.front, e0, e1, 0, b); break;
		default: hipExtLaunchKernelGGL((k_chanfir<OS, R, 1>), grid, block, (uint32_t)lds, c->streams.front, e0, e1, 0, b); break;
	}
}

static int launch_back(vdl2hip_ctx *c, OutSlot &sl);
static int capture_launch(vdl2hip_ctx *c, OutSlot &sl, hipStream_t st);
static void capture_free(vdl2hip_ctx *c);
static int launch_rest(vdl2hip_ctx *c, OutSlot &sl, struct OutSlot *succ);
static int flush_rest(vdl2hip_ctx *c, const OutSlot *upto);
static bool feed_is_small(const vdl2hip_ctx *c, int64_t D);

static int capture_collect(vdl2hip_ctx *c, OutSlot &sl, const OutFrame *fr, uint32_t nf);
static int txlog_collect(vdl2hip_ctx *c, OutSlot &sl, const OutFrame *fr, uint32_t nf);
static int collect_slot(vdl2hip_ctx *c, OutSlot &sl) {
	if(!sl.pending) return VDL2HIP_OK;
	if(sl.rest_pending) { int r = flush_rest(c, &sl); if(r != VDL2HIP_OK) return r; }
	HIPCHK(hipEventSynchronize(sl.done));
	sl.pending = false;
	sl.rs_t.collect(c->stats.resample_ms);
	sl.mon_t.collect(c->mon.kernel_ms);
	sl.act_t.collect(c->act.kernel_ms);
	sl.cap_t.collect(c->capt.kernel_ms);
	sl.txl_t.collect(c->txl.kernel_ms);
	if(c->profiling && sl.ev_valid) {
		const Event *ev = sl.ev;
		float ms = 0.f;
		if(sl.k1_timed && hipEventElapsedTime(&ms, ev[0], ev[1]) == hipSuccess) { c->stats.chanfir_ms += ms; c->stats.chanfir_launches++; }
		if(sl.ev_level >= 2) {
		if(!sl.fused && hipEventElapsedTime(&ms, ev[2], ev[3]) == hipSuccess) c->stats.phase_ms += ms;
		if(hipEventElapsedTime(&ms, ev[4], sl.ev_front) == hipSuccess) c->stats.sync_ms += ms;
		if(hipEventElapsedTime(&ms, ev[6], ev[7]) == hipSuccess) c->stats.walk_ms += ms;
// ... 256 lines not shown
	KernelTimes &t = sl.rs_t;
	t.arm(c->profiling >= 2);
	if(c->in_fmt == VDL2HIP_FMT_CF32) launch_resample<2>(c, a, grid, t.e(0), t.e(1));
	else if(c->in_fmt == VDL2HIP_FMT_S16LE) launch_resample<1>(c, a, grid, t.e(0), t.e(1));
	else if(c->in_fmt == kFmtS8) launch_resample<3>(c, a, grid, t.e(0), t.e(1));
	else launch_resample<0>(c, a, grid, t.e(0), t.e(1));
	HIPCHK(hipGetLastError());
	t.launched(1);
	rs.tail_sel ^= 1; rs.first[k] = n0; rs.count[k] = nout; rs.n_in = N1; rs.n_out = n1;
	int r = feed_common(c, rs.d_out[k], (size_t)nout * sizeof(float2));
	c->stats.input_samples += nin - nout;
	c->stats.resampled_samples += nout;
	return r;
}

template<int FMT>
static void launch_spectrum(vdl2hip_ctx *c, const SpecArgs &a, unsigned grid, hipEvent_t e0, hipEvent_t e1) {
	#define SPEC_LAUNCH(PER) hipExtLaunchKernelGGL((k_spectrum<FMT, PER>), dim3(grid), dim3(c->mon.threads), (uint32_t)c->mon.lds, c->streams.front, e0, e1, 0, a)
	switch(c->mon.nfft / c->mon.threads) {
		case 1: SPEC_LAUNCH(1); break;
		case 2: SPEC_LAUNCH(2); break;
		case 4: SPEC_LAUNCH(4); break;
		case 8: SPEC_LAUNCH(8); break;
		default: SPEC_LAUNCH(16); break;
	}
	#undef SPEC_LAUNCH
}
static int monitor_block(vdl2hip_ctx *c, const void *dev_in, size_t nbytes) {
	auto &m = c->mon;
	const uint64_t nin = nbytes / sample_bytes(c->in_fmt);
	if(nin == 0) return VDL2HIP_OK;
	if(nin >= (1ull << 32)) return VDL2HIP_E_TOOBIG;
	const uint64_t N = m.nfft, pos0 = m.pos, pos1 = pos0 + nin;
	const uint64_t j0 = pos0 / N, j1 = pos1 / N;
	const uint64_t ja = (j0 + m.stride - 1) / m.stride * m.stride;
	const uint64_t nseg = ja < j1 ? (j1 - 1 - ja) / m.stride + 1 : 0;
	const uint32_t o1 = (uint32_t)(pos1 % N);
	const uint32_t ncarry_out = j1 % m.stride == 0 ? o1 : 0;
	m.pos = pos1;
	if(nseg == 0 && ncarry_out == 0) { m.ncarry = 0; return VDL2HIP_OK; }
	SpecArgs a{};
	a.in = dev_in; a.carry_in = m.buf.d_carry[m.carry_sel]; a.carry_out = m.buf.d_carry[m.carry_sel ^ 1]; a.w = m.buf.d_w; a.tw = m.buf.d_tw; a.rows = m.buf.d_rows;
	a.rel0 = (int64_t)(ja * N) - (int64_t)pos0; a.carry_rel = (int64_t)(j1 * N) - (int64_t)pos0; a.seg_step = (uint64_t)m.stride * N;
	a.nin = (uint32_t)nin; a.ncarry = m.ncarry; a.ncarry_out = ncarry_out; a.nseg = (uint32_t)nseg;
	a.run = (uint32_t)std::max<uint64_t>(1, (nseg + kSpecMaxRows - 1) / kSpecMaxRows); a.N = m.nfft; a.log2n = m.log2n;
	const unsigned grid = (unsigned)std::max<uint64_t>(1, (nseg + a.run - 1) / a.run);
	if(grid > kSpecMaxRows || (int64_t)a.ncarry + a.rel0 < 0) return VDL2HIP_E_INVAL;
	OutSlot &sl = c->slot[c->feed_no % kSlots];
	{ int r = collect_slot(c, sl); if(r != VDL2HIP_OK && r != VDL2HIP_E_OVERFLOW) return r; }
	KernelTimes &t = sl.mon_t;
	t.arm(c->profiling >= 2);
	if(c->in_fmt == VDL2HIP_FMT_CF32) launch_spectrum<2>(c, a, grid, t.e(0), t.e(1));
	else if(c->in_fmt == VDL2HIP_FMT_S16LE) launch_spectrum<1>(c, a, grid, t.e(0), t.e(1));
	else if(c->in_fmt == kFmtS8) launch_spectrum<3>(c, a, grid, t.e(0), t.e(1));
	else launch_spectrum<0>(c, a, grid, t.e(0), t.e(1));
	if(nseg) {
		const uint32_t W = m.nfft + kSpecLevels;
		hipExtLaunchKernelGGL(k_spectrum_reduce, dim3((W + 255) / 256), dim3(256), 0u, c->streams.front, t.e(2), t.e(3), 0,
		                      (const double *)m.buf.d_rows, m.buf.d_acc.get(), (uint32_t)grid, m.nfft);
	}
	HIPCHK(hipGetLastError());
	HIPCHK(m.tap.mark(c->streams.front));
	t.launched(nseg ? 2 : 1);
	m.segments += nseg; m.carry_sel ^= 1; m.ncarry = ncarry_out;
	return VDL2HIP_OK;
}
static void monitor_free(vdl2hip_ctx *c) {
	auto &m = c->mon;
	if(m.tap.queued) (void)hipEventSynchronize(m.tap.last);
	m.buf = {};
	m.on = false; m.tap.queued = false; m.nfft = 0;
}

static bool feed_is_small(const vdl2hip_ctx *c, int64_t D) {
	const int nseg = (int)std::min<int64_t>(c->seg_max, D / c->seg_min);
	return D > 0 && D < 2 * c->seg_min && nseg < 2;
}
#define LAUNCH_SCAN_MULTI(how, ...) do { \
	if(c->fmt == 2) { if(c->os == 20) how((k_ref_scan_multi<2, 20>), __VA_ARGS__); else if(c->os == 10) how((k_ref_scan_multi<2, 10>), __VA_ARGS__); else how((k_ref_scan_multi<2, 0>), __VA_ARGS__); } \
	else if(c->fmt == 1) { if(c->os == 20) how((k_ref_scan_multi<1, 20>), __VA_ARGS__); else if(c->os == 10) how((k_ref_scan_multi<1, 10>), __VA_ARGS__); else how((k_ref_scan_multi<1, 0>), __VA_ARGS__); } \
	else if(c->fmt == 3) { if(c->os == 20) how((k_ref_scan_multi<3, 20>), __VA_ARGS__); else if(c->os == 10) how((k_ref_scan_multi<3, 10>), __VA_ARGS__); else how((k_ref_scan_multi<3, 0>), __VA_ARGS__); } \
	else { if(c->os == 20) how((k_ref_scan_multi<0, 20>), __VA_ARGS__); else if(c->os == 10) how((k_ref_scan_multi<0, 10>), __VA_ARGS__); else how((k_ref_scan_multi<0, 0>), __VA_ARGS__); } } while(0)
static void launch_scans(vdl2hip_ctx *c, hipStream_t st, RefChan *ref, uint32_t launch, const ScanReq *sq, const RefReq *rq, const uint32_t *n, uint32_t cap, int64_t k_end,
                         ScanReq *retry, uint32_t *retry_n, hipEvent_t e0 = nullptr, hipEvent_t e1 = nullptr) {
	const int rty = retry ? c->ref_retry_mul : 0;
	LAUNCH_SCAN_MULTI(hipExtLaunchKernelGGL, dim3((cap + kScanLanes - 1) / kScanLanes), dim3(64 * kScanWaves), 0, st, e0, rty ? (hipEvent_t) nullptr : e1, 0, ref, launch,
	                  sq, rq, n, cap, k_end, rty ? retry : (ScanReq *) nullptr, retry_n, kRetryScans, 1);
	if(rty) LAUNCH_SCAN_MULTI(hipExtLaunchKernelGGL, dim3(kRetryScans / kScanLanes), dim3(64 * kScanWaves), 0, st, (hipEvent_t) nullptr, e1, 0, ref, launch,
	                  (const ScanReq *)retry, (const RefReq *) nullptr, (const uint32_t *)retry_n, kRetryScans, k_end, (ScanReq *) nullptr, (uint32_t *) nullptr, 0u, rty);
}
static int launch_rest(vdl2hip_ctx *c, OutSlot &sl, OutSlot *succ);
static void launch_stitch(vdl2hip_ctx *c, hipStream_t st, const OutSlot &sl, const K4Args &k4, int again, hipEvent_t e1 = nullptr) {
	K4sArgs k4s{ k4, sl.d_spec_of, (uint32_t)(3 * (c->seg_max - 1)), sl.nseg, sl.back_k0, sl.seglen, c->d_segstats, again };
	hipExtLaunchKernelGGL(k_walk_stitch, dim3((unsigned)((c->C + kStitchWaves - 1) / kStitchWaves)), dim3(64 * kStitchWaves), (unsigned)(sizeof(StitchLds) * kStitchWaves), st, (hipEvent_t) nullptr, e1, 0, k4s);
}

static int walk_ahead_of(const vdl2hip_ctx *c, int64_t D) {
	if(!c->walk_ahead_auto) return c->walk_ahead;
	return c->C >= 16 && (double)D * (double)c->C < c->walk_ahead_below ? 1 : 0;
}

static int launch_back(vdl2hip_ctx *c, OutSlot &sl) {
	const int64_t D = sl.back_D, k0 = sl.back_k0;
	const int wa = walk_ahead_of(c, D);
	int nseg = (int)std::min<int64_t>(c->seg_max, D / c->seg_min);
	const bool small = feed_is_small(c, D);
	hipStream_t sb_ = small ? c->streams.front : c->streams.back;
	const Event *ev = sl.ev;
	const bool prof_all = sl.ev_valid && sl.ev_level >= 2;
	sl.small = small; sl.has_chk = false; sl.nseg = 1; sl.seglen = D;
	OutSlot &pv = c->slot[(sl.seq + kSlots - 1) % kSlots];
	const bool opt = c->referee && D > 0;
	const uint32_t rq_cap = small ? std::min<uint32_t>(c->rq_cap, 16u * kScanLanes) : c->rq_cap;
	const bool ahead = wa && opt && nseg >= 2 && sl.seq > 0 && pv.pending && pv.rest_pending && pv.has_chk && pv.nseg >= 2;
	if(!ahead) { int r = flush_rest(c, nullptr); if(r != VDL2HIP_OK) return r; }
	if(small) {
		if(sl.seq > 0 && pv.pending && !pv.small) HIPCHK(hipStreamWaitEvent(sb_, pv.done, 0));
	} else {
		HIPCHK(hipStreamWaitEvent(sb_, sl.ev_front, 0));
	}
	if(D <= 0) hipLaunchKernelGGL(k_reset_ctl, dim3(1), dim3(1), 0, sb_, sl.d_ctl, 0u);
	hipStream_t sp_ = small ? c->streams.front : c->streams.pre[sl.seq % kSidePre];
	if(D > 0 && sl.prescan) {
		if(!small) HIPCHK(hipStreamWaitEvent(sp_, sl.ev_front, 0));
		launch_scans(c, sp_, c->d_ref[sl.seq % kSlots], (uint32_t)(16 * sl.seq + 8), sl.d_pq, nullptr, sl.d_rqn + 3, kPreScans, k0 + D, sl.d_retry, sl.d_rqn + 4);
		if(!small) { HIPCHK(hipEventRecord(sl.ev_pre, sp_)); HIPCHK(hipStreamWaitEvent(sb_, sl.ev_pre, 0)); }
	}
	if(D > 0) {
		const int64_t k1 = k0 + D;
		const int par = (int)(sl.seq % 2);
		sl.k4 = K4Args{ c->d_y, c->d_pf, c->d_cand, c->d_tab, c->d_ws, c->d_wcnt, sl.d_bursts, sl.d_nbchan, c->cap_bursts_chan, sl.d_ctl, c->d_freq,
		           sl.d_log, sl.d_nlog, c->cap_log, k1, c->cfg.max_ppm, c->cap, c->cap - 1, c->chan_first, c->C, c->d_ppmthr, c->referee ? c->d_ref[sl.seq % kSlots] : nullptr, (uint32_t)(16 * sl.seq + 1),
		           opt ? sl.d_rq : nullptr, sl.d_rqn, rq_cap, sl.d_rqflag, c->d_ws_snap[par], c->d_cnt_snap[par], sl.d_rqbad, sl.prescan ? 1 : 0, c->debug_force_again,
		           c->d_ws_tmp, c->d_cnt_tmp, nullptr, nullptr, sl.d_rqflag2, nullptr, c->debug_force_mismatch };
		const K4Args &k4 = sl.k4;
		sl.d_spec_of = c->d_spec[par];
		if(nseg >= 2) {
			sl.seglen = (D + nseg - 1) / nseg;
			nseg = (int)((D + sl.seglen - 1) / sl.seglen);
			sl.nseg = nseg;
			K4sArgs k4s{ k4, sl.d_spec_of, (uint32_t)(3 * (c->seg_max - 1)), nseg, k0, sl.seglen, c->d_segstats, 0 };
			LAUNCH_EV(k_walk_spec, dim3((unsigned)((1 + 3 * (nseg - 1) + kWalkWaves - 1) / kWalkWaves), (unsigned)c->C), dim3(64 * kWalkWaves), sb_, EV(6), (hipEvent_t) nullptr, k4s);
			launch_stitch(c, sb_, sl, k4, 0, EV(7));
		} else {
			LAUNCH_EV(k_walk, dim3((unsigned)c->C), dim3(64), sb_, EV(6), EV(7), k4);
		}
		if(k4.rq) {
			sl.has_chk = true;
			hipStream_t sc_ = wa ? sp_ : sb_;
			if(sc_ != sb_) { HIPCHK(hipEventRecord(sl.ev_stitch, sb_)); HIPCHK(hipStreamWaitEvent(sc_, sl.ev_stitch, 0)); }
			launch_scans(c, sc_, k4.ref, k4.ref_launch - 1u, nullptr, k4.rq, k4.rq_n, rq_cap, k1, sl.d_retry + kRetryScans, sl.d_rqn + 5);
			hipLaunchKernelGGL(k_ref_verify, dim3(small ? 64 : 1024), dim3(64), 0, sc_, k4);
			HIPCHK(hipEventRecord(sl.ev_chk, sc_));
		}
	}
	sl.rest_pending = true;
	for(;;) {
		OutSlot *old = nullptr;
		for(auto &x : c->slot) if(x.pending && x.rest_pending && (!old || x.seq < old->seq)) old = &x;
		if(!old || old == &sl || sl.seq - old->seq < (uint64_t)wa) break;
		int r = flush_rest(c, old); if(r != VDL2HIP_OK) return r;
	}
	if(!(wa && sl.has_chk && sl.nseg >= 2)) return flush_rest(c, nullptr);
	HIPCHK(hipGetLastError());
	return VDL2HIP_OK;
}

static int flush_rest(vdl2hip_ctx *c, const OutSlot *upto) {
	for(;;) {
		OutSlot *old = nullptr;
		for(auto &x : c->slot) if(x.pending && x.rest_pending && (!old || x.seq < old->seq)) old = &x;
		if(!old || (upto && old->seq > upto->seq)) return VDL2HIP_OK;
		OutSlot *s1 = &c->slot[(old->seq + 1) % kSlots];
		if(!(s1->pending && s1->rest_pending && s1->seq == old->seq + 1)) s1 = nullptr;
		int r = launch_rest(c, *old, s1); if(r != VDL2HIP_OK) return r;
	}
}

static_assert(kCapMaxPre + 56320 + 200 < kHistory + 1024, "a window begins inside what the ring keeps behind a feed");
static_assert(sizeof(CapRec) == sizeof(vdl2hip_burst) && sizeof(vdl2hip_burst) == 128 && offsetof(CapRec, iq_first) == offsetof(vdl2hip_burst, iq_first)
              && offsetof(CapRec, frames) == offsetof(vdl2hip_burst, frames) && offsetof(CapRec, mean_power) == offsetof(vdl2hip_burst, mean_power)
              && offsetof(CapRec, phase_err_max) == offsetof(vdl2hip_burst, phase_err_max), "the host copies the device's records as they are");
static_assert(sizeof(vdl2hip_capture_cfg) == 24 && sizeof(vdl2hip_capture_info) == 56 && sizeof(CapHdr) == 16, "vdl2hip.h states these sizes");
static_assert(kCapMaxChan == kK5MaxChan, "k_capture_copy keeps every channel's offsets in LDS");
constexpr uint32_t kCapMailRecs = 32;
constexpr size_t kCapMailBytes = sizeof(CapHdr) + kCapMailRecs * sizeof(CapRec);
constexpr uint32_t kTxMailRecs = 32, kTxMaxWait = 4096;
constexpr size_t kTxMailBytes = sizeof(TxHdr) + kTxMailRecs * sizeof(TxRec);

static int capture_launch(vdl2hip_ctx *c, OutSlot &sl, hipStream_t st) {
	auto &m = c->capt;
	CapArgs a{};
	a.y = c->d_y; a.bursts = sl.d_bursts; a.nb_chan = sl.d_nbchan; a.freq = c->d_freq;
	a.plan = sl.cap.d_plan; a.tot = sl.cap.d_tot; a.rec = sl.cap.d_rec; a.pool = sl.cap.d_pool; a.hdr = sl.cap.d_hdr;
	a.k_end = sl.back_k0 + sl.back_D; a.pool_samples = m.pool; a.cap_bursts_chan = c->cap_bursts_chan; a.nchan = (uint32_t)c->C; a.chan_first = (uint32_t)c->chan_first;
	a.cap = c->cap; a.mask = c->cap - 1; a.pre = m.pre; a.post = m.post;
	KernelTimes &t = sl.cap_t;
	t.arm(c->profiling >= 2);
	hipExtLaunchKernelGGL(k_capture_plan, dim3((unsigned)c->C), dim3(64), 0u, st, t.e(0), t.e(1), 0, a);
	const unsigned grid = std::min(512u, std::max(8u, sl.k5_waves / 4));
	hipExtLaunchKernelGGL(k_capture_copy, dim3(grid), dim3(kCapThreads), 0u, st, t.e(2), t.e(3), 0, a);
	HIPCHK(hipGetLastError());
	HIPCHK(hipMemcpyAsync(sl.cap.h_mail, sl.cap.d_hdr, kCapMailBytes, hipMemcpyDeviceToHost, st));
	t.launched(2);
	return VDL2HIP_OK;
}
static int capture_collect(vdl2hip_ctx *c, OutSlot &sl, const OutFrame *fr, uint32_t nf) {
	auto &m = c->capt;
	if(!m.on || !sl.cap.h_mail) return VDL2HIP_OK;
	const CapHdr h = *sl.cap.h_mail.as<CapHdr>();
	const uint32_t nrec = (uint32_t)std::min<uint64_t>(h.nrec, (uint64_t)c->C * c->cap_bursts_chan);
	const uint64_t pairs = std::min<uint64_t>(h.pairs, m.pool);
	if(nrec == 0) return VDL2HIP_OK;
	const CapRec *rec = reinterpret_cast<const CapRec *>(sl.cap.h_mail + sizeof(CapHdr));
	const size_t rec_bytes = nrec > kCapMailRecs ? sizeof(CapRec) * (size_t)nrec : 0, need = rec_bytes + (size_t)pairs * sizeof(cf32);
	HIPCHK(m.stage.reserve(need));
	if(rec_bytes) { HIPCHK(hipMemcpyAsync(m.stage, sl.cap.d_rec, rec_bytes, hipMemcpyDeviceToHost, c->streams.out)); rec = m.stage.as<CapRec>(); }
	if(pairs) HIPCHK(hipMemcpyAsync(m.stage + rec_bytes, sl.cap.d_pool, (size_t)pairs * sizeof(cf32), hipMemcpyDeviceToHost, c->streams.out));
	if(need) HIPCHK(hipStreamSynchronize(c->streams.out));
	const float *iqp = reinterpret_cast<const float *>(m.stage + rec_bytes);
	auto iq = pairs ? std::make_shared<std::vector<float>>(iqp, iqp + 2 * (size_t)pairs) : std::make_shared<std::vector<float>>();
	struct Join { uint32_t frames = 0, ok = 0; int32_t fec = -1, last_idx = -1; };
	std::map<std::pair<int32_t, int64_t>, Join> join;
	for(uint32_t i = 0; i < nf; i++) {
		if(fr[i].chan < 0 || fr[i].chan >= c->C) continue;
		Join &j = join[{ fr[i].chan + c->chan_first, fr[i].burst_ord }];
		j.frames++; if(fr[i].avlc_status == AVLC_OK) j.ok++;
		if(fr[i].idx >= j.last_idx) { j.last_idx = fr[i].idx; j.fec = fr[i].num_fec_corrections; }
	}
	for(uint32_t i = 0; i < nrec; i++) {
		vdl2hip_burst r;
		memcpy(&r, rec + i, sizeof r);
		if(r.iq_off + r.iq_count > pairs) { r.iq_count = 0; r.iq_off = 0; r.flags |= VDL2HIP_BURST_NO_ROOM; }
		m.bursts++; m.iq_samples += r.iq_count; if(r.flags & VDL2HIP_BURST_NO_ROOM) m.iq_dropped++;
// ... 49 lines not shown
	const TxRec *rec = reinterpret_cast<const TxRec *>(sl.txl.h_mail + sizeof(TxHdr));
	if(nrec > kTxMailRecs) {
		const size_t bytes = sizeof(TxRec) * (size_t)nrec;
		HIPCHK(m.buf.stage.reserve(bytes));
		HIPCHK(hipMemcpyAsync(m.buf.stage, sl.txl.d_rec, bytes, hipMemcpyDeviceToHost, c->streams.out));
		HIPCHK(hipStreamSynchronize(c->streams.out));
		rec = m.buf.stage.as<TxRec>();
	}
	const int64_t close_bins = (int64_t)c->act.H + 2, B = c->act.B;
	for(uint32_t i = 0; i < nrec; i++) {
		vdl2hip_tx r;
		memcpy(&r, rec + i, sizeof(TxRec));
		r.frames = r.frames_ok = 0; r.first_burst_ord = -1;
		const int64_t close_sample = c->act.k_on + ((int64_t)r.last_bin + close_bins) * B;
		int64_t first_sync = 0;
		if(r.chan >= (uint32_t)c->chan_first && r.chan < (uint32_t)(c->chan_first + c->C)) {
			auto &w = m.wait[r.chan - (uint32_t)c->chan_first];
			size_t keep = 0;
			for(const auto &f : w) {
				if(f.sync_sample < r.first_sample) m.unmatched++;
				else if(f.sync_sample < close_sample) {
					if(!r.frames || f.sync_sample < first_sync) { first_sync = f.sync_sample; r.first_burst_ord = f.burst_ord; }
					r.frames++; if(f.ok) r.frames_ok++;
				} else w[keep++] = f;
			}
			w.resize(keep);
		}
		m.transmissions++; m.matched += r.frames; if(r.frames_ok) m.decoded++;
		if((m.flags & VDL2HIP_TXLOG_UNDECODED_ONLY) && r.frames_ok != 0) continue;
		m.queue.push_back(r);
	}
	return VDL2HIP_OK;
}
static void txlog_free(vdl2hip_ctx *c) {
	for(auto &sl : c->slot) { sl.txl = {}; sl.txl_on = false; sl.txl_t.n = 0; }
	auto &m = c->txl;
	m.buf = {}; m.queue.clear(); m.wait.clear();
	m.on = false;
}
static int txlog_off(vdl2hip_ctx *c) {
	if(!c->txl.on) return VDL2HIP_OK;
	if(!c->failed) { int r = collect_pending(c); if(r != VDL2HIP_OK && r != VDL2HIP_E_OVERFLOW) return r; }
	(void)hipStreamSynchronize(c->streams.front);
	txlog_free(c);
	return VDL2HIP_OK;
}
static int launch_rest(vdl2hip_ctx *c, OutSlot &sl, OutSlot *succ) {
	const int64_t D = sl.back_D, k0 = sl.back_k0;
	const bool small = sl.small;
	hipStream_t sb_ = small ? c->streams.front : c->streams.back, sn_ = small ? c->streams.front : c->streams.nf, s5_ = small ? c->streams.front : c->streams.burst[sl.seq % kSideBurst];

	const Event *ev = sl.ev;
	const bool prof_all = sl.ev_valid && sl.ev_level >= 2;
	sl.rest_pending = false;
	if(D > 0 && sl.has_chk) {
		HIPCHK(hipStreamWaitEvent(sb_, sl.ev_chk, 0));
		K4Args k4 = sl.k4;
		if(succ) { k4.ws_snap_next = succ->k4.ws_snap; k4.cnt_snap_next = succ->k4.cnt_snap; k4.rq_flag2_next = succ->d_rqflag2; }
		if(sl.nseg >= 2) launch_stitch(c, sb_, sl, k4, succ ? 2 : 1);
		else hipLaunchKernelGGL(k_walk_again, dim3((unsigned)c->C), dim3(64), 0, sb_, k4);
	}
	if(!small) {
		HIPCHK(hipEventRecord(sl.ev_walk, sb_));
		HIPCHK(hipStreamWaitEvent(sn_, sl.ev_walk, 0));
		HIPCHK(hipStreamWaitEvent(s5_, sl.ev_walk, 0));
	}
	if(succ) launch_stitch(c, sb_, *succ, succ->k4, 3);
	if(D > 0) {
		K4bArgs k4b{ c->d_y, c->d_nf, sl.d_log, sl.d_nlog, c->d_scfirst, c->d_sccum, c->d_nffeed, c->d_lpbuf, c->d_nfring, c->nf_ring - 1,
		             c->cap, c->cap - 1, c->cap_log, c->cap_comb, c->cap_hist, c->C };
		const unsigned nf_lds = (unsigned)(sizeof(NfShared) * kNfWaves), nf_grid = (unsigned)((c->C + kNfWaves - 1) / kNfWaves);
		if(small) {
		} else {
			hipExtLaunchKernelGGL(k_nf_prepare, dim3(nf_grid), dim3(64 * kNfWaves), nf_lds, sn_, EV(8), (hipEvent_t) nullptr, 0, k4b);
			const unsigned ngrp = (unsigned)std::min<uint64_t>(64, (c->cap_hist + kNfGroup * kNfWaves - 1) / (kNfGroup * kNfWaves));
			hipLaunchKernelGGL(k_nf_replay, dim3(ngrp, (unsigned)c->C), dim3(64 * kNfWaves), nf_lds, sn_, k4b);
			hipExtLaunchKernelGGL(k_nf_finish, dim3(nf_grid), dim3(64 * kNfWaves), nf_lds, sn_, (hipEvent_t) nullptr, EV(9), 0, k4b);
			HIPCHK(hipEventRecord(sl.ev_nf, sn_));
		}
		K5Args k5{ c->d_y, c->d_tab, c->d_cnt, sl.d_bursts, sl.d_nbchan, c->cap_bursts_chan, c->C,
		           sl.d_frames, sl.d_pool, sl.d_ctl, c->d_freq, c->cap, c->cap - 1, c->referee ? c->d_ref[sl.seq % kSlots] : nullptr, (uint32_t)(16 * sl.seq + 5), BurstDefer{} };
		const bool defer5 = c->referee;
		const uint32_t sq_cap = small ? kDeferScans / 16 : std::min(c->sq_alloc, defer_scans_for(D, c->C)), dq_cap = sq_cap / 2;
		if(defer5) k5.df = BurstDefer{ sl.d_dq, sl.d_rqn + 1, dq_cap, sl.d_sq, sl.d_rqn + 2, sq_cap, 1 };
		const unsigned k5_lds = (unsigned)((sizeof(BurstShared) + 4 * (kK5MaxChan + 1)) * kBurstWaves);
		hipEvent_t ev_last5 = defer5 ? (hipEvent_t) nullptr : EV(11);
		if(small) hipExtLaunchKernelGGL(k_nf_burst, dim3(nf_grid + sl.k5_waves / kBurstWaves), dim3(64 * kNfWaves), std::max(nf_lds, k5_lds), s5_, EV(8), ev_last5, 0, k4b, k5, (uint32_t)nf_grid);
		else hipExtLaunchKernelGGL(k_burst, dim3(sl.k5_waves / kBurstWaves), dim3(64 * kBurstWaves), k5_lds, s5_, EV(10), ev_last5, 0, k5);
		if(defer5) {
			launch_scans(c, s5_, k5.ref, (uint32_t)(16 * sl.seq + 6), sl.d_sq, nullptr, sl.d_rqn + 2, sq_cap, k0 + D, sl.d_retry + 2 * kRetryScans, sl.d_rqn + 6);
			K5Args k5b = k5; k5b.df.pass = 2; k5b.ref_launch = (uint32_t)(16 * sl.seq + 7);
			hipExtLaunchKernelGGL(k_burst, dim3(std::max(1u, dq_cap / kBurstWaves / 4)), dim3(64 * kBurstWaves), k5_lds, s5_, (hipEvent_t) nullptr, EV(11), 0, k5b);
		}
		if(!small) HIPCHK(hipStreamWaitEvent(s5_, sl.ev_nf, 0));
		const unsigned ff_grid = std::min(256u, (sl.k5_waves * (unsigned)kResSlots * 2 / kFrameChunk + kFrameWaves - 1) / kFrameWaves);
		hipLaunchKernelGGL(k_frame_finish, dim3(ff_grid), dim3(64 * kFrameWaves), 0, s5_, sl.d_frames, (const uint8_t *)sl.d_pool, sl.d_mail, (const Tables *)c->d_tab,
		                   c->d_acnt, (const float *)c->d_nfring, c->nf_ring - 1, sl.d_frames_out, sl.d_pool_out);
		if(sl.cap_on) { int r = capture_launch(c, sl, s5_); if(r != VDL2HIP_OK) return r; }
		if(sl.txl_on) HIPCHK(hipMemcpyAsync(sl.txl.h_mail, sl.txl.d_hdr, kTxMailBytes, hipMemcpyDeviceToHost, s5_));
	}
	HIPCHK(hipMemcpyAsync(sl.h_mail, sl.d_mail, sizeof(OutMail), hipMemcpyDeviceToHost, s5_));
	HIPCHK(hipEventRecord(sl.done, s5_));
	HIPCHK(hipGetLastError());
	return VDL2HIP_OK;
}

static void sort_queue(vdl2hip_ctx *c) {
	std::stable_sort(c->queue.begin(), c->queue.end(), [](const HostFrame &a, const HostFrame &b) {
		if(a.f.end_sample != b.f.end_sample) return a.f.end_sample < b.f.end_sample;
		if(a.f.chan != b.f.chan) return a.f.chan < b.f.chan;
		return a.f.idx < b.f.idx;
	});
}

static void fill_frame(const vdl2hip_ctx *c, const HostFrame &h, vdl2hip_frame &f) {
	f.chan = (uint32_t)(h.f.chan + c->chan_first); f.freq = c->freqs[h.f.chan]; f.idx = h.f.idx;
	f.len = h.f.len; f.octets = h.octets();
	f.synd_weight = h.f.synd_weight; f.datalen_octets = h.f.datalen_octets; f.num_fec_corrections = h.f.num_fec_corrections;
	f.frame_pwr_dbfs = h.f.frame_pwr_dbfs; f.nf_pwr_dbfs = h.f.nf_pwr_dbfs; f.ppm_error = h.f.ppm_error;
	f.burst_ord = h.f.burst_ord; f.sync_sample = h.f.sync_sample; f.end_sample = h.f.end_sample;
	f.avlc_status = h.f.avlc_status; f.dst_addr = h.f.dst_addr; f.src_addr = h.f.src_addr;
}

namespace {
std::mutex g_pool_mutex;
std::vector<StreamSet> g_pool;
}

extern "C" {

int vdl2hip_abi_version(void) { return VDL2HIP_ABI_VERSION; }

const char *vdl2hip_strerror(int err) {
	switch(err) {
		case VDL2HIP_OK: return "ok";
		case VDL2HIP_E_INVAL: return "invalid argument";
		case VDL2HIP_E_NOMEM: return "out of memory";
		case VDL2HIP_E_DEVICE: return "HIP device error";
		case VDL2HIP_E_TOOBIG: return "block larger than max_block_bytes";
		case VDL2HIP_E_OVERFLOW: return "device output buffer overflow";
		default: return "unknown error";
	}
}

void vdl2hip_destroy(vdl2hip_ctx *c) {
	if(!c) return;
	OnDevice dev_guard(c);
	c->streams.each([](hipStream_t st) { if(st) (void)hipStreamSynchronize(st); });
	if(c->streams.front && c->pooled) {
		std::lock_guard<std::mutex> lk(g_pool_mutex);
		g_pool.push_back(c->streams);
	} else c->streams.each([](hipStream_t st) { if(st) (void)hipStreamDestroy(st); });
	delete c;
}

static int cfg_read(const vdl2hip_cfg *in, vdl2hip_cfg &cfg) {
	if(!in || in->struct_size < VDL2HIP_CFG_SIZE_V1) return VDL2HIP_E_INVAL;
	memset(&cfg, 0, sizeof cfg);
	memcpy(&cfg, in, in->struct_size >= sizeof(vdl2hip_cfg) ? sizeof(vdl2hip_cfg) : (size_t)VDL2HIP_CFG_SIZE_V1);
	cfg.struct_size = sizeof(vdl2hip_cfg); cfg.reserved0 = 0;
	return cfg.reserved1 ? VDL2HIP_E_INVAL : VDL2HIP_OK;
}

int vdl2hip_create(const vdl2hip_cfg *cfg_in, vdl2hip_ctx **out) {
	vdl2hip_cfg cfg_v;
	if(!out || cfg_read(cfg_in, cfg_v) != VDL2HIP_OK) return VDL2HIP_E_INVAL;
	const vdl2hip_cfg *cfg = &cfg_v;
// ... 82 lines not shown
	DEV_ALLOC(c->d_bf, 1); DEV_ALLOC(c->d_lut, 256); DEV_ALLOC(c->d_tab, 1);
	if(resample) {
		auto &rs = c->rs;
		if(!design_resampler(cfg->input_rate, fs, rd)) { vdl2hip_destroy(c); return VDL2HIP_E_INVAL; }
		rs.L = rd.L; rs.M = rd.M; rs.T = rd.T; rs.cap = rs_max_out;
		rs.span_cap = (uint32_t)((255ull * rs.M + rs.L - 1) / rs.L) + rs.T;
		const size_t ntaps = (size_t)rs.L * rs.T, tap_bytes = ntaps * sizeof(float);
		rs.taps_lds = tap_bytes <= kResTapsLds;
		rs.lds = (size_t)rs.span_cap * sizeof(float2) + (rs.taps_lds ? tap_bytes : 0);
		std::vector<float> walk(ntaps);
		for(uint32_t j = 0; j < rs.T; j++) for(uint32_t q = 0; q < rs.L; q++) walk[(size_t)j * rs.L + q] = rd.taps[(size_t)j * rs.L + (size_t)((uint64_t)q * rs.M % rs.L)];
		DEV_ALLOC(rs.d_taps, ntaps);
		DEV_CHK(hipMemcpy(rs.d_taps, walk.data(), tap_bytes, hipMemcpyHostToDevice));
		for(auto &t : rs.d_tail) DEV_ALLOC(t, rs.T, true);
		for(auto &o : rs.d_out) DEV_ALLOC(o, (size_t)rs.cap + 2);
	}
	DEV_ALLOC(c->d_dphi, count); DEV_ALLOC(c->d_freq, count); DEV_ALLOC(c->d_ppmthr, count);
	DEV_ALLOC(c->d_carry[0], sb * kMaxOversample); DEV_ALLOC(c->d_carry[1], sb * kMaxOversample);
	const size_t nring = (size_t)count * cap;
	static_assert(sizeof(cf32) == 8 && sizeof(float4) == 16 && sizeof(unsigned long long) == 8, "the sizes the counts below stand for");
	DEV_ALLOC(c->d_y, nring, true); DEV_ALLOC(c->d_pf, nring, true);
	DEV_ALLOC(c->d_cand, nring / 64, true); DEV_ALLOC(c->d_flag, nring / 64, true);
	DEV_ALLOC(c->d_segend, (size_t)count * c->nseg_cap, true);
	DEV_ALLOC(c->d_qpow, 64);
	DEV_ALLOC(c->d_tcarry[0], count, true); DEV_ALLOC(c->d_tcarry[1], count, true);
	DEV_ALLOC(c->d_segpub, (size_t)count * c->nseg_cap * 4, true); DEV_ALLOC(c->d_synctmo, 1, true);
	c->fuse_k2 = getenv("VDL2HIP_NO_FUSE") == nullptr;
	DEV_ALLOC(c->d_ws, count); DEV_ALLOC(c->d_cnt, 2 * (size_t)count * kNumCounters, true); c->d_wcnt = c->d_cnt + (size_t)count * kNumCounters;
	DEV_ALLOC(c->d_acnt, (size_t)count * kNumAvlcCounters, true);
	c->cap_bursts_chan = (uint32_t)(dmax / 220 + 4);
	uint64_t cap_b = (uint64_t)count * c->cap_bursts_chan;
	uint64_t cap_f = cap_b * 2; if(cap_f < 4096) cap_f = 4096;
	cap_f += 2048 * kResSlots;
	uint64_t cap_p = cap_b * 512; if(cap_p < (1u << 22)) cap_p = 1u << 22; if(cap_p > (1u << 30)) cap_p = 1u << 30;
	c->cap_log = 8192; c->cap_comb = c->cap_log + kNfTail; c->cap_hist = (uint32_t)(dmax / 3000 + 8);
	cap_p += 2048 * kResPool;
	c->ctl_template = OutCtl{ 0, 0, 0, 0, (uint32_t)cap_b, (uint32_t)cap_f, (uint32_t)cap_p, c->cap_log, 0, 0, {0, 0} };
	DEV_ALLOC(c->d_nf, count);
	DEV_ALLOC(c->d_scfirst, (size_t)count * (c->cap_comb + 1)); DEV_ALLOC(c->d_sccum, (size_t)count * (c->cap_comb + 1));
	c->nf_ring = 64; while(c->nf_ring < (kSlots + 2) * c->cap_hist) c->nf_ring <<= 1;
	DEV_ALLOC(c->d_nfring, (size_t)count * c->nf_ring, true);
	DEV_ALLOC(c->d_lpbuf, (size_t)count * c->cap_hist, true); DEV_ALLOC(c->d_nffeed, count, true);
	{
		const char *e = getenv("VDL2HIP_SEG_MIN");
		if(e && atoll(e) >= 64) c->seg_min = atoll(e);
		int64_t smax = std::min<int64_t>(16, 8192 / (3 * (int64_t)count));
		smax = std::min<int64_t>(smax, dmax / c->seg_min);
		e = getenv("VDL2HIP_SEG_MAX");
		if(e) smax = std::min<int64_t>(smax, atoll(e));
		c->seg_max = (int)std::max<int64_t>(1, smax);
		if(c->seg_max >= 2) for(auto &sp_ : c->d_spec) DEV_ALLOC(sp_, (size_t)count * 3 * (c->seg_max - 1));
		DEV_ALLOC(c->d_segstats, (size_t)count * 2, true);
	}
	for(auto &sl : c->slot) {
		DEV_ALLOC(sl.d_bursts, cap_b); DEV_ALLOC(sl.d_nbchan, count, true);
		DEV_ALLOC(sl.d_frames, cap_f); DEV_ALLOC(sl.d_pool, cap_p); DEV_ALLOC(sl.d_mail, 1, true);
		sl.d_ctl = &sl.d_mail.get()->ctl;
		DEV_CHK(hipMemcpy(sl.d_ctl, &c->ctl_template, sizeof(OutCtl), hipMemcpyHostToDevice));
		DEV_ALLOC(sl.d_frames_out, cap_f); DEV_ALLOC(sl.d_pool_out, cap_p);
		DEV_ALLOC(sl.d_log, (size_t)count * c->cap_log); DEV_ALLOC(sl.d_nlog, count, true);
		DEV_CHK(sl.h_mail.alloc(sizeof(OutMail), true));
	}

	if(const char *e = getenv("VDL2HIP_REFEREE")) c->referee = atoi(e) != 0;
	c->ref_prescan = count <= 64;
	if(const char *e = getenv("VDL2HIP_REF_PRESCAN")) c->ref_prescan = atoi(e) != 0;
	if(const char *e = getenv("VDL2HIP_REF_RETRY")) { const int v = atoi(e); if(v == 0 || (v >= 2 && v <= 8)) c->ref_retry_mul = v; }
	if(const char *e = getenv("VDL2HIP_REF_WARM")) { const long long v = atoll(e); if(v >= 1024 && v <= (1ll << 24)) c->ref_warm = v; }
	if(c->referee) {
		c->ref_T = std::max(1, c->ref_retry_mul) * c->ref_warm + (int64_t)(kHistory + 256) * c->os + 4096;
		c->ref_cap = 1; while(c->ref_cap < (uint64_t)(kSlots + 2) * (uint64_t)c->ref_T) c->ref_cap <<= 1;
		DEV_ALLOC(c->d_refhist, c->ref_cap * sb);
		for(auto &r : c->d_ref) DEV_ALLOC(r, 1, true);
		DEV_ALLOC(c->d_refdone, (size_t)count * kRefCache, true); DEV_ALLOC(c->d_refdonen, count, true); DEV_ALLOC(c->d_refstats, 16, true); DEV_ALLOC(c->d_mix, count);
		std::vector<uint8_t> mix(count);
		for(uint32_t i = 0; i < count; i++) mix[i] = cfg->centerfreq != c->freqs[i];
		DEV_CHK(hipMemcpy(c->d_mix, mix.data(), count, hipMemcpyHostToDevice));
		for(int k = 0; k < 2; k++) { DEV_ALLOC(c->d_ws_snap[k], count); DEV_ALLOC(c->d_cnt_snap[k], (size_t)count * kNumCounters); }
		DEV_ALLOC(c->d_ws_tmp, count); DEV_ALLOC(c->d_cnt_tmp, (size_t)count * kNumCounters);
		c->walk_ahead = (count >= 16 && count <= 64) ? 1 : 0;
		c->sq_alloc = defer_scans_for((int64_t)dmax, (int)count);
		for(auto &sl : c->slot) {
			DEV_ALLOC(sl.d_rq, c->rq_cap); DEV_ALLOC(sl.d_rqn, 8, true); DEV_ALLOC(sl.d_retry, 3 * (size_t)kRetryScans); DEV_ALLOC(sl.d_rqflag, count, true);
			DEV_ALLOC(sl.d_dq, c->sq_alloc / 2); DEV_ALLOC(sl.d_sq, c->sq_alloc);
			DEV_ALLOC(sl.d_pq, kPreScans); DEV_CHK(sl.ev_pre.ensure(hipEventDisableTiming));
			DEV_ALLOC(sl.d_rqbad, count, true);
			DEV_ALLOC(sl.d_rqflag2, count, true);
			DEV_CHK(sl.ev_stitch.ensure(hipEventDisableTiming)); DEV_CHK(sl.ev_chk.ensure(hipEventDisableTiming));
		}
	}

	Lut4 lut[256]; build_nco_lut(lut);
	auto tab = std::make_unique<Tables>(); build_tables(*tab);
	std::vector<WalkState> ws(count);
	for(auto &w : ws) { memset(&w, 0, sizeof w); walk_state_init(w); }
	DEV_CHK(hipMemcpy(c->d_bf, &c->bf, sizeof(BlockForm), hipMemcpyHostToDevice));
	DEV_CHK(hipMemcpy(c->d_qpow, c->bf.Qpow, 64 * sizeof(float4), hipMemcpyHostToDevice));
	DEV_CHK(hipMemcpy(c->d_lut, lut, sizeof lut, hipMemcpyHostToDevice));
	DEV_CHK(hipMemcpy(c->d_tab, tab.get(), sizeof(Tables), hipMemcpyHostToDevice));
	DEV_CHK(hipMemcpy(c->d_dphi, c->dphi.data(), 4 * count, hipMemcpyHostToDevice));
	DEV_CHK(hipMemcpy(c->d_freq, c->freqs.data(), 4 * count, hipMemcpyHostToDevice));
	{
		std::vector<float> thr(count);
		for(uint32_t i = 0; i < count; i++) thr[i] = ppm_gate_threshold(c->freqs[i], cfg->max_ppm);
		DEV_CHK(hipMemcpy(c->d_ppmthr, thr.data(), 4 * count, hipMemcpyHostToDevice));
	}
	DEV_CHK(hipMemcpy(c->d_ws, ws.data(), count * sizeof(WalkState), hipMemcpyHostToDevice));
	{
		std::vector<NfState> nfs(count);
		for(auto &n : nfs) { memset(&n, 0, sizeof n); nf_state_init(n); }
		DEV_CHK(hipMemcpy(c->d_nf, nfs.data(), count * sizeof(NfState), hipMemcpyHostToDevice));
	}
	const size_t lds = (size_t)c->run * c->os * 65 * sizeof(float2) + 8192;
	if(lds > 65536) { vdl2hip_destroy(c); return VDL2HIP_E_INVAL; }
	DEV_CHK(hipDeviceSynchronize());
	#undef DEV_ALLOC
	#undef DEV_CHK
	*out = c;
	return VDL2HIP_OK;
}

static int feed_host(vdl2hip_ctx *c, const void *buf, size_t nbytes, bool wait_copy) {
	if(!c || (!buf && nbytes)) return VDL2HIP_E_INVAL;
	OnDevice dev_guard(c);
	if(c->failed) return VDL2HIP_E_DEVICE;
	if(nbytes == 0) return VDL2HIP_OK;
	if(nbytes > c->in_cap) return VDL2HIP_E_TOOBIG;
	nbytes -= nbytes % sample_bytes(c->in_fmt);
	if(c->pinned_pending) { HIPCHK(hipEventSynchronize(c->pinned_pending)); c->pinned_pending = nullptr; }
	const int k = (int)(c->feed_no % kSlots);
	{ int r = collect_slot(c, c->slot[k]); if(r != VDL2HIP_OK && r != VDL2HIP_E_OVERFLOW) return r; }
	if(!c->d_in[k]) {
		if(c->d_in[k].alloc(c->in_cap + 16) != hipSuccess) return VDL2HIP_E_NOMEM;
		HIPCHK(c->ev_copied[k].ensure(hipEventDisableTiming));
	}
	bool parts = !wait_copy && nbytes >= kColdMinBytes && !c->rs.on && !c->mon.on;
	for(auto &sl : c->slot) if(sl.pending) parts = false;
	c->cold.n = 0;
	if(parts) {
		const size_t piece = (nbytes / kColdParts) & ~(size_t)4095;
		static_assert(4096 % 8 == 0 && 4096 % 4 == 0, "a piece of a cold-start block ends on a sample boundary in every format");
		if(piece % sample_bytes(c->fmt)) return VDL2HIP_E_INVAL;
		size_t off = 0;
		for(int p = 0; p < kColdParts; p++) {
			const size_t len = p == kColdParts - 1 ? nbytes - off : piece;
			HIPCHK(c->cold.ev[p].ensure(hipEventDisableTiming));
			HIPCHK(hipMemcpyAsync(c->d_in[k] + off, (const uint8_t *)buf + off, len, hipMemcpyHostToDevice, c->streams.copy));
			HIPCHK(hipEventRecord(c->cold.ev[p], c->streams.copy));
			off += len;
			c->cold.samples[p] = off / sample_bytes(c->fmt);
		}
		c->cold.n = kColdParts;
	} else if(wait_copy) {
		HIPCHK(hipMemcpy(c->d_in[k], buf, nbytes, hipMemcpyHostToDevice));
	} else {
		HIPCHK(hipMemcpyAsync(c->d_in[k], buf, nbytes, hipMemcpyHostToDevice, c->streams.copy));
	}
	if(!wait_copy) {
		HIPCHK(hipEventRecord(c->ev_copied[k], c->streams.copy));
		c->pinned_pending = c->ev_copied[k];
		if(!parts) HIPCHK(hipStreamWaitEvent(c->streams.front, c->ev_copied[k], 0));
	}
	int r = feed_block(c, c->d_in[k], nbytes, parts);
	if(r == VDL2HIP_E_DEVICE) c->failed = true;
	return r;
}

// ... 118 lines not shown

int vdl2hip_avlc_counters(vdl2hip_ctx *c, uint32_t chan, uint64_t out[VDL2HIP_NUM_AVLC_COUNTERS]) {
	if(!c || !out || chan < (uint32_t)c->chan_first || chan >= (uint32_t)(c->chan_first + c->C)) return VDL2HIP_E_INVAL;
	OnDevice dev_guard(c);
	int r = collect_pending(c);
	if(r != VDL2HIP_OK && r != VDL2HIP_E_OVERFLOW) return r;
	HIPCHK(hipMemcpy(out, c->d_acnt + (size_t)(chan - c->chan_first) * kNumAvlcCounters, 8 * kNumAvlcCounters, hipMemcpyDeviceToHost));
	return VDL2HIP_OK;
}

int vdl2hip_set_avlc_filter(vdl2hip_ctx *c, int on) {
	if(!c) return VDL2HIP_E_INVAL;
	c->avlc_filter = on != 0;
	return VDL2HIP_OK;
}

static const char *const kCounterNames[VDL2HIP_NUM_COUNTERS] = {
	"demod.sync.good", "decoder.crc.good", "decoder.crc.bad", "decoder.errors.no_header", "decoder.errors.too_long",
	"decoder.errors.no_fec", "decoder.errors.data_truncated", "decoder.errors.fec_truncated", "decoder.errors.deinterleave_data",
	"decoder.errors.deinterleave_fec", "decoder.errors.fec_bad", "decoder.errors.bitstream", "decoder.errors.truncated_octets",
	"decoder.errors.unstuff", "decoder.blocks.processed", "decoder.blocks.fec_ok", "decoder.msg.good", "decoder.msg.good_loud",
	"demod.ppm_reject", "demod.slicer_neg_idx" };
static const char *const kAvlcCounterNames[VDL2HIP_NUM_AVLC_COUNTERS] = {
	"avlc.frames.processed", "avlc.errors.too_short", "avlc.frames.good", "avlc.errors.bad_fcs", "avlc.msg.air2gnd",
	"avlc.msg.air2air", "avlc.msg.air2all", "avlc.msg.gnd2air", "avlc.msg.gnd2gnd", "avlc.msg.gnd2all" };

int vdl2hip_statsd_lines(vdl2hip_ctx *c, const char *ns, char *out, size_t cap) {
	if(!c || !ns || !out) return VDL2HIP_E_INVAL;
	OnDevice dev_guard(c);
	int r = collect_pending(c);
	if(r != VDL2HIP_OK && r != VDL2HIP_E_OVERFLOW) return r;
	const size_t per = VDL2HIP_NUM_COUNTERS + VDL2HIP_NUM_AVLC_COUNTERS;
	std::vector<uint64_t> now((size_t)c->C * per);
	{
		std::vector<uint64_t> a(2 * (size_t)c->C * kNumCounters), b((size_t)c->C * kNumAvlcCounters);
		HIPCHK(hipMemcpy(a.data(), c->d_cnt, a.size() * 8, hipMemcpyDeviceToHost));
		for(size_t k = 0, n = a.size() / 2; k < n; k++) a[k] += a[n + k];
		HIPCHK(hipMemcpy(b.data(), c->d_acnt, b.size() * 8, hipMemcpyDeviceToHost));
		for(int ch = 0; ch < c->C; ch++) {
			std::copy(a.begin() + (size_t)ch * kNumCounters, a.begin() + (size_t)(ch + 1) * kNumCounters, now.begin() + ch * per);
			std::copy(b.begin() + (size_t)ch * kNumAvlcCounters, b.begin() + (size_t)(ch + 1) * kNumAvlcCounters, now.begin() + ch * per + kNumCounters);
		}
	}
	const bool first = c->statsd_prev.empty();
	if(first) c->statsd_prev.assign(now.size(), 0);
	std::string txt;
	char line[320];
	for(int ch = 0; ch < c->C; ch++)
		for(size_t k = 0; k < per; k++) {
			const uint64_t d = now[ch * per + k] - c->statsd_prev[ch * per + k];
			if(!first && d == 0) continue;
			const char *name = k < (size_t)kNumCounters ? kCounterNames[k] : kAvlcCounterNames[k - kNumCounters];
			snprintf(line, sizeof line, "%s.%u.%s:%llu|c\n", ns, c->freqs[ch], name, (unsigned long long)d);
			txt += line;
		}
	if(txt.size() + 1 > cap) { if(first) c->statsd_prev.clear(); return VDL2HIP_E_TOOBIG; }
	memcpy(out, txt.c_str(), txt.size() + 1);
	c->statsd_prev = now;
	return (int)txt.size();
}

int vdl2hip_set_profiling(vdl2hip_ctx *c, int on) {
	if(!c) return VDL2HIP_E_INVAL;
	OnDevice dev_guard(c);
	int r = collect_pending(c);
	c->profiling = on < 0 ? 0 : on > 2 ? 2 : on;
	return r == VDL2HIP_E_OVERFLOW ? VDL2HIP_OK : r;
}

int vdl2hip_get_stats_sized(vdl2hip_ctx *c, vdl2hip_stats *out, size_t size) {
	if(!c || !out) return VDL2HIP_E_INVAL;
	OnDevice dev_guard(c);
	int r = collect_pending(c);
	{
		std::vector<uint32_t> ss((size_t)c->C * 2);
		if(hipMemcpy(ss.data(), c->d_segstats, ss.size() * 4, hipMemcpyDeviceToHost) != hipSuccess) return VDL2HIP_E_DEVICE;
		c->stats.seg_adopted = c->stats.seg_walked = 0;
		uint32_t tmo = 0;
		if(hipMemcpy(&tmo, c->d_synctmo, 4, hipMemcpyDeviceToHost) != hipSuccess) return VDL2HIP_E_DEVICE;
		c->stats.front_sync_timeouts = tmo;
		for(int i = 0; i < c->C; i++) { c->stats.seg_adopted += ss[2 * i]; c->stats.seg_walked += ss[2 * i + 1]; }
	}
	if(c->d_refstats) {
		uint32_t rs[11] = {0, 0, 0, 0, 0, 0, 0, 0, 0, 0, 0};
		if(hipMemcpy(rs, c->d_refstats, sizeof rs, hipMemcpyDeviceToHost) != hipSuccess) return VDL2HIP_E_DEVICE;
		c->stats.referee_scans = rs[0]; c->stats.referee_cached = rs[1]; c->stats.referee_refused = rs[2]; c->stats.referee_short = rs[3];
		c->stats.referee_candidate_scans = rs[4]; c->stats.referee_header_scans = rs[5]; c->stats.referee_symbol_scans = rs[6]; c->stats.referee_rewalks = rs[7]; c->stats.referee_redone_next = rs[8]; c->stats.referee_unmet = rs[9]; c->stats.referee_retried = rs[10];
	}
	memcpy(out, &c->stats, std::min(size, sizeof c->stats));
	return (r == VDL2HIP_E_OVERFLOW || c->failed) ? VDL2HIP_OK : r;
}
int vdl2hip_get_stats(vdl2hip_ctx *c, vdl2hip_stats *out) { return vdl2hip_get_stats_sized(c, out, sizeof(vdl2hip_stats)); }

void *vdl2hip_stream(vdl2hip_ctx *c) { return c ? (void *)c->streams.front : nullptr; }

int vdl2hip_set_drain_lag(vdl2hip_ctx *c, int lag) {
	if(!c || lag < 0 || lag > kSlots - 1) return VDL2HIP_E_INVAL;
	c->drain_lag = lag;
	return VDL2HIP_OK;
}

int vdl2hip_get_lpf(vdl2hip_ctx *c, float A[3], float B[3]) {
	if(!c) return VDL2HIP_E_INVAL;
	memcpy(A, c->lpf.A, sizeof c->lpf.A); memcpy(B, c->lpf.B, sizeof c->lpf.B);
	return VDL2HIP_OK;
}

int vdl2hip_get_nco_step(vdl2hip_ctx *c, uint32_t chan, uint32_t *dphi) {
	if(!c || !dphi || chan < (uint32_t)c->chan_first || chan >= (uint32_t)(c->chan_first + c->C)) return VDL2HIP_E_INVAL;
	*dphi = nco_step(c->cfg.centerfreq, c->freqs[chan - c->chan_first], (uint32_t)kSymbolRate * kSps * c->os);
	return VDL2HIP_OK;
}

int vdl2hip_read_decimated(vdl2hip_ctx *c, uint32_t chan, int64_t first, float *dst, size_t cap) {
	if(!c || !dst || chan < (uint32_t)c->chan_first || chan >= (uint32_t)(c->chan_first + c->C)) return VDL2HIP_E_INVAL;
	OnDevice dev_guard(c);
	int r = collect_pending(c);
	if(r != VDL2HIP_OK && r != VDL2HIP_E_OVERFLOW) return r;
	if(first < 0 || first > c->k_total || c->k_total - first > (int64_t)c->cap) return VDL2HIP_E_INVAL;
	size_t n = std::min<size_t>(cap, (size_t)(c->k_total - first));
	const cf32 *base = c->d_y + (size_t)(chan - c->chan_first) * c->cap;
	size_t done = 0;
	while(done < n) {
		uint32_t slot = (uint32_t)(first + (int64_t)done) & (c->cap - 1);
		size_t m = std::min<size_t>(n - done, c->cap - slot);
		HIPCHK(hipMemcpy(dst + 2 * done, base + slot, m * sizeof(cf32), hipMemcpyDeviceToHost));
		done += m;
	}
	return (int)n;
}

int vdl2hip_read_resampled(vdl2hip_ctx *c, int64_t first, float *dst, size_t cap) {
	if(!c || !dst || !c->rs.on) return VDL2HIP_E_INVAL;
	OnDevice dev_guard(c);
	int r = collect_pending(c);
	if(r != VDL2HIP_OK && r != VDL2HIP_E_OVERFLOW) return r;
	if(first < 0 || (uint64_t)first > c->rs.n_out) return VDL2HIP_E_INVAL;
	size_t done = 0;
	const size_t n = (size_t)std::min<uint64_t>(cap, c->rs.n_out - (uint64_t)first);
	while(done < n) {
		const uint64_t pos = (uint64_t)first + done;
		int k = -1;
		for(int i = 0; i < kSlots; i++) if(c->rs.count[i] && pos >= c->rs.first[i] && pos < c->rs.first[i] + c->rs.count[i]) k = i;
		if(k < 0) return done ? (int)done : VDL2HIP_E_INVAL;
		const size_t m = (size_t)std::min<uint64_t>(n - done, c->rs.first[k] + c->rs.count[k] - pos);
		HIPCHK(hipMemcpy(dst + 2 * done, c->rs.d_out[k] + (pos - c->rs.first[k]), m * sizeof(float2), hipMemcpyDeviceToHost));
		done += m;
	}
	return (int)n;
}

int vdl2hip_resampler_design(uint32_t input_rate, uint32_t output_rate, uint32_t *L, uint32_t *M, uint32_t *T, float *taps, size_t cap) {
	ResamplerDesign d;
	if(!design_resampler(input_rate, output_rate, d, false)) return VDL2HIP_E_INVAL;
	if(L) *L = d.L;
	if(M) *M = d.M;
	if(T) *T = d.T;
	if(!taps || (size_t)d.L * d.T > cap) return VDL2HIP_E_TOOBIG;
	if(!design_resampler(input_rate, output_rate, d)) return VDL2HIP_E_INVAL;
	memcpy(taps, d.taps.data(), d.taps.size() * sizeof(float));
	return (int)d.taps.size();
}

int vdl2hip_spectrum_window(uint32_t nfft, uint32_t window, float *w, size_t cap) {
	SpectrumDesign d;
	if(!design_spectrum(nfft, window, d, false)) return VDL2HIP_E_INVAL;
	if(!w || cap < nfft) return VDL2HIP_E_TOOBIG;
	memcpy(w, d.w.data(), (size_t)nfft * sizeof(float));
	return (int)nfft;
}
// ... 311 lines not shown
```

dumpvdl2_amd/vdl2hip.py:

```python
from __future__ import annotations

import ctypes as C
import os
from typing import List, Optional, Sequence

import numpy as np

HERE = os.path.dirname(os.path.abspath(__file__))
LIB_PATH = os.path.join(HERE, "libvdl2hip.so")

FMT_U8, FMT_S16LE, FMT_CF32 = 0, 1, 2
FMT_S8 = 4
COUNTER_NAMES = [
    "demod.sync.good", "decoder.crc.good", "decoder.crc.bad", "decoder.errors.no_header",
    "decoder.errors.too_long", "decoder.errors.no_fec", "decoder.errors.data_truncated",
    "decoder.errors.fec_truncated", "decoder.errors.deinterleave_data",
    "decoder.errors.deinterleave_fec", "decoder.errors.fec_bad", "decoder.errors.bitstream",
    "decoder.errors.truncated_octets", "decoder.errors.unstuff", "decoder.blocks.processed",
    "decoder.blocks.fec_ok", "decoder.msg.good", "decoder.msg.good_loud",
    "demod.ppm_reject", "demod.slicer_neg_idx",
]
NUM_COUNTERS = len(COUNTER_NAMES)
AVLC_COUNTER_NAMES = [
    "avlc.frames.processed", "avlc.errors.too_short", "avlc.frames.good", "avlc.errors.bad_fcs",
    "avlc.msg.air2gnd", "avlc.msg.air2air", "avlc.msg.air2all", "avlc.msg.gnd2air", "avlc.msg.gnd2gnd", "avlc.msg.gnd2all",
]
NUM_AVLC_COUNTERS = len(AVLC_COUNTER_NAMES)
AVLC_OK, AVLC_TOO_SHORT, AVLC_BAD_FCS = 0, 1, 2
ABI_VERSION = 6
MAX_DRAIN_LAG = int(os.environ.get("VDL2HIP_PY_MAX_DRAIN_LAG", "5"))
EXPORTS = [
    "vdl2hip_abi_version", "vdl2hip_strerror", "vdl2hip_create", "vdl2hip_destroy", "vdl2hip_feed",
    "vdl2hip_feed_device", "vdl2hip_sync", "vdl2hip_drain", "vdl2hip_counters", "vdl2hip_set_profiling",
    "vdl2hip_drain_packed", "vdl2hip_pack_raw_frame", "vdl2hip_get_stats", "vdl2hip_get_stats_sized", "vdl2hip_stream", "vdl2hip_set_drain_lag", "vdl2hip_get_lpf", "vdl2hip_get_nco_step", "vdl2hip_read_decimated",
    "vdl2hip_avlc_counters", "vdl2hip_set_avlc_filter", "vdl2hip_statsd_lines", "vdl2hip_feed_pinned",
    "vdl2hip_group_create", "vdl2hip_group_destroy", "vdl2hip_group_feed", "vdl2hip_group_feed_pinned", "vdl2hip_group_sync", "vdl2hip_group_drain",
    "vdl2hip_group_set_drain_lag", "vdl2hip_group_counters", "vdl2hip_group_avlc_counters", "vdl2hip_group_size", "vdl2hip_group_ctx",
    "vdl2hip_group_uses_rccl", "vdl2hip_group_set_exchange", "vdl2hip_group_exchange",
    "vdl2hip_read_resampled", "vdl2hip_resampler_design",
    "vdl2hip_spectrum_window", "vdl2hip_spectrum_enable", "vdl2hip_spectrum_read", "vdl2hip_spectrum_channels",
    "vdl2hip_activity_edges", "vdl2hip_activity_enable", "vdl2hip_activity_disable", "vdl2hip_activity_read", "vdl2hip_activity_series",
    "vdl2hip_capture_enable", "vdl2hip_capture_disable", "vdl2hip_capture_info_get", "vdl2hip_capture_read",
    "vdl2hip_txlog_enable", "vdl2hip_txlog_disable", "vdl2hip_txlog_info_get", "vdl2hip_txlog_read",
]
TXLOG_UNDECODED_ONLY, TX_PARTIAL = 1, 1
CAPTURE_FAILED_ONLY, BURST_NO_ROOM = 1, 1
WIN_RECT, WIN_HANN, WIN_BH4 = 0, 1, 2


class Cfg(C.Structure):
    _fields_ = [("struct_size", C.c_uint32), ("centerfreq", C.c_uint32), ("oversample", C.c_uint32),
                ("sample_fmt", C.c_uint32), ("nchan", C.c_uint32), ("freqs", C.POINTER(C.c_uint32)),
                ("max_ppm", C.c_float), ("device", C.c_int32), ("max_block_bytes", C.c_uint32),
                ("chan_first", C.c_uint32), ("chan_count", C.c_uint32),
                ("reserved0", C.c_uint32), ("input_rate", C.c_uint32), ("reserved1", C.c_uint32)]


class CFrame(C.Structure):
    _fields_ = [("chan", C.c_uint32), ("freq", C.c_uint32), ("idx", C.c_int32), ("len", C.c_uint32),
                ("octets", C.POINTER(C.c_uint8)), ("synd_weight", C.c_uint32), ("datalen_octets", C.c_uint32),
                ("num_fec_corrections", C.c_int32), ("frame_pwr_dbfs", C.c_float), ("nf_pwr_dbfs", C.c_float),
                ("ppm_error", C.c_float), ("burst_ord", C.c_int64), ("sync_sample", C.c_int64),
                ("end_sample", C.c_int64), ("avlc_status", C.c_uint32), ("dst_addr", C.c_uint32), ("src_addr", C.c_uint32)]


class Stats(C.Structure):
    _fields_ = [("feeds", C.c_uint64), ("input_samples", C.c_uint64), ("chan_samples", C.c_uint64),
                ("chanfir_launches", C.c_uint64), ("chanfir_ms", C.c_double), ("phase_ms", C.c_double),
                ("sync_ms", C.c_double), ("walk_ms", C.c_double), ("burst_ms", C.c_double), ("nf_ms", C.c_double),
                ("bursts", C.c_uint64), ("frames", C.c_uint64),
                ("seg_adopted", C.c_uint64), ("seg_walked", C.c_uint64), ("front_sync_timeouts", C.c_uint64),
                ("overflow_feeds", C.c_uint64), ("cold_start_feeds", C.c_uint64),
                ("referee_scans", C.c_uint64), ("referee_cached", C.c_uint64), ("referee_refused", C.c_uint64), ("referee_short", C.c_uint64), ("referee_rewalks", C.c_uint64),
                ("referee_candidate_scans", C.c_uint64), ("referee_header_scans", C.c_uint64), ("referee_symbol_scans", C.c_uint64),
                ("referee_redone_next", C.c_uint64), ("referee_unmet", C.c_uint64), ("referee_retried", C.c_uint64),
                ("resampled_samples", C.c_uint64), ("resample_ms", C.c_double)]


class SpectrumCfg(C.Structure):
    _fields_ = [("struct_size", C.c_uint32), ("nfft", C.c_uint32), ("window", C.c_uint32), ("stride", C.c_uint32)]


class SpectrumInfo(C.Structure):
    _fields_ = [("struct_size", C.c_uint32), ("nfft", C.c_uint32), ("window", C.c_uint32), ("stride", C.c_uint32),
                ("sample_rate", C.c_uint32), ("centerfreq", C.c_uint32),
                ("segments", C.c_uint64), ("samples", C.c_uint64), ("clipped", C.c_uint64),
                ("enbw_bins", C.c_double), ("mean_power", C.c_double), ("dc_i", C.c_double), ("dc_q", C.c_double),
                ("peak", C.c_float), ("kernel_ms", C.c_float)]


class ActivityCfg(C.Structure):
    _fields_ = [("struct_size", C.c_uint32), ("bin_samples", C.c_uint32), ("hang_bins", C.c_uint32), ("series_bins", C.c_uint32),
                ("threshold_dbfs", C.c_float), ("reserved", C.c_uint32)]


class ActivityInfo(C.Structure):
    _fields_ = [("struct_size", C.c_uint32), ("bin_samples", C.c_uint32), ("hang_bins", C.c_uint32), ("series_bins", C.c_uint32),
                ("threshold_dbfs", C.c_float), ("threshold_power", C.c_float), ("first_sample", C.c_int64), ("bins", C.c_uint64),
                ("kernel_ms", C.c_float), ("reserved", C.c_uint32)]


class ActivityChan(C.Structure):
    _fields_ = [("bins", C.c_uint64), ("busy_bins", C.c_uint64), ("transmissions", C.c_uint64), ("longest_bins", C.c_uint64),
                ("sum_power", C.c_double), ("max_power", C.c_float), ("min_power", C.c_float), ("open", C.c_uint32), ("reserved", C.c_uint32),
                ("hist", C.c_uint64 * 64)]


ACTIVITY_CHAN_DTYPE = np.dtype([("bins", "<u8"), ("busy_bins", "<u8"), ("transmissions", "<u8"), ("longest_bins", "<u8"),
                                ("sum_power", "<f8"), ("max_power", "<f4"), ("min_power", "<f4"), ("open", "<u4"), ("reserved", "<u4"),
                                ("hist", "<u8", (64,))])


class CaptureCfg(C.Structure):
    _fields_ = [("struct_size", C.c_uint32), ("pre_samples", C.c_uint32), ("post_samples", C.c_uint32), ("flags", C.c_uint32),
                ("pool_samples", C.c_uint32), ("reserved", C.c_uint32)]


class CaptureInfo(C.Structure):
    _fields_ = [("struct_size", C.c_uint32), ("pre_samples", C.c_uint32), ("post_samples", C.c_uint32), ("flags", C.c_uint32),
                ("pool_samples", C.c_uint32), ("reserved", C.c_uint32), ("bursts", C.c_uint64), ("iq_samples", C.c_uint64),
                ("iq_dropped", C.c_uint64), ("kernel_ms", C.c_float), ("reserved2", C.c_uint32)]


BURST_DTYPE = np.dtype([("chan", "<u4"), ("freq", "<u4"), ("burst_ord", "<i8"), ("sync_sample", "<i8"), ("end_sample", "<i8"), ("first_symbol", "<i8"),
                        ("nsym", "<u4"), ("tl_bits", "<u4"), ("ppm_error", "<f4"), ("dphi", "<f4"), ("prev_phase", "<f4"), ("flags", "<u4"),
                        ("iq_first", "<i8"), ("iq_count", "<u4"), ("reserved", "<u4"), ("iq_off", "<u8"),
                        ("frames", "<u4"), ("frames_ok", "<u4"), ("fec_corrections", "<i4"), ("weak_symbols", "<u4"),
                        ("mean_power", "<f4"), ("min_power", "<f4"), ("max_power", "<f4"),
                        ("phase_err_rms", "<f4"), ("phase_err_mean", "<f4"), ("phase_err_max", "<f4")])


class TxlogCfg(C.Structure):
    _fields_ = [("struct_size", C.c_uint32), ("pool_records", C.c_uint32), ("flags", C.c_uint32), ("reserved", C.c_uint32)]


class TxlogInfo(C.Structure):
    _fields_ = [("struct_size", C.c_uint32), ("pool_records", C.c_uint32), ("flags", C.c_uint32), ("reserved", C.c_uint32),
                ("transmissions", C.c_uint64), ("decoded", C.c_uint64), ("dropped", C.c_uint64),
                ("frames_matched", C.c_uint64), ("frames_unmatched", C.c_uint64), ("kernel_ms", C.c_float), ("reserved2", C.c_uint32)]


TX_DTYPE = np.dtype([("chan", "<u4"), ("freq", "<u4"), ("first_bin", "<u8"), ("last_bin", "<u8"), ("peak_bin", "<u8"),
                     ("first_sample", "<i8"), ("last_sample", "<i8"), ("busy_bins", "<u4"), ("flags", "<u4"),
                     ("peak_power", "<f4"), ("mean_power", "<f4"), ("frames", "<u4"), ("frames_ok", "<u4"),
                     ("first_burst_ord", "<i8")])


class PackedFrame(C.Structure):
    _fields_ = [("frame", CFrame), ("octets_off", C.c_uint64)]


FRAME_CB = C.CFUNCTYPE(None, C.POINTER(CFrame), C.c_void_p)
_lib = None


def load_library(path: str = None):
    global _lib
    if _lib is not None:
        return _lib
# ... 618 lines not shown
```

include/vdl2hip.h:

```cpp
#ifndef VDL2HIP_H
#define VDL2HIP_H
#include <stddef.h>
#include <stdint.h>

#ifdef __cplusplus
extern "C" {
#endif

#define VDL2HIP_ABI_VERSION 6

#define VDL2HIP_FMT_U8     0
#define VDL2HIP_FMT_S16LE  1
#define VDL2HIP_FMT_CF32   2
#define VDL2HIP_FMT_S8     4

#define VDL2HIP_OK            0
#define VDL2HIP_E_INVAL      -1
#define VDL2HIP_E_NOMEM      -2
#define VDL2HIP_E_DEVICE     -3
#define VDL2HIP_E_TOOBIG     -4
#define VDL2HIP_E_OVERFLOW   -5

enum {
	VDL2HIP_CNT_SYNC_GOOD = 0,
// ... 89 lines not shown
	uint32_t reserved2;
} vdl2hip_capture_info;

#define VDL2HIP_TXLOG_UNDECODED_ONLY 1u
#define VDL2HIP_TX_PARTIAL           1u
typedef struct { uint32_t struct_size, pool_records, flags, reserved; } vdl2hip_txlog_cfg;
typedef struct {
	uint32_t chan, freq;
	uint64_t first_bin, last_bin;
	uint64_t peak_bin;
	int64_t  first_sample, last_sample;
	uint32_t busy_bins, flags;
	float    peak_power, mean_power;
	uint32_t frames, frames_ok;
	int64_t  first_burst_ord;
} vdl2hip_tx;
typedef struct {
	uint32_t struct_size, pool_records, flags, reserved;
	uint64_t transmissions, decoded, dropped;
	uint64_t frames_matched, frames_unmatched;
	float    kernel_ms;
	uint32_t reserved2;
} vdl2hip_txlog_info;

typedef struct {
	uint32_t chan;
	uint32_t freq;
	int32_t  idx;
	uint32_t len;
	const uint8_t *octets;
	uint32_t synd_weight;
	uint32_t datalen_octets;
	int32_t  num_fec_corrections;
	float    frame_pwr_dbfs;
	float    nf_pwr_dbfs;
	float    ppm_error;
	int64_t  burst_ord;
	int64_t  sync_sample;
	int64_t  end_sample;
	uint32_t avlc_status;
	uint32_t dst_addr, src_addr;
} vdl2hip_frame;

enum { VDL2HIP_AVLC_OK = 0, VDL2HIP_AVLC_TOO_SHORT = 1, VDL2HIP_AVLC_BAD_FCS = 2 };

enum {
	VDL2HIP_ACNT_FRAMES_PROCESSED = 0,
	VDL2HIP_ACNT_ERR_TOO_SHORT,
	VDL2HIP_ACNT_FRAMES_GOOD,
	VDL2HIP_ACNT_ERR_BAD_FCS,
	VDL2HIP_ACNT_MSG_AIR2GND, VDL2HIP_ACNT_MSG_AIR2AIR, VDL2HIP_ACNT_MSG_AIR2ALL,
	VDL2HIP_ACNT_MSG_GND2AIR, VDL2HIP_ACNT_MSG_GND2GND, VDL2HIP_ACNT_MSG_GND2ALL,
	VDL2HIP_NUM_AVLC_COUNTERS
};

typedef void (*vdl2hip_frame_cb)(const vdl2hip_frame *frame, void *user);

typedef struct {
	uint64_t feeds;
	uint64_t input_samples;
	uint64_t chan_samples;
	uint64_t chanfir_launches;
	double   chanfir_ms;
	double   phase_ms, sync_ms, walk_ms, burst_ms;
	double   nf_ms;
	uint64_t bursts;
	uint64_t frames;
	uint64_t seg_adopted;
	uint64_t seg_walked;
	uint64_t front_sync_timeouts;
	uint64_t overflow_feeds;
	uint64_t cold_start_feeds;
	uint64_t referee_scans;
	uint64_t referee_cached;
	uint64_t referee_refused;
	uint64_t referee_short;
	uint64_t referee_rewalks;
	uint64_t referee_candidate_scans, referee_header_scans, referee_symbol_scans;
	uint64_t referee_redone_next;
	uint64_t referee_unmet;
	uint64_t referee_retried;
	uint64_t resampled_samples;
	double   resample_ms;
} vdl2hip_stats;

int  vdl2hip_abi_version(void);
const char *vdl2hip_strerror(int err);

int  vdl2hip_create(const vdl2hip_cfg *cfg, vdl2hip_ctx **out);
void vdl2hip_destroy(vdl2hip_ctx *ctx);

int  vdl2hip_feed(vdl2hip_ctx *ctx, const void *buf, size_t nbytes);
int  vdl2hip_feed_pinned(vdl2hip_ctx *ctx, const void *buf, size_t nbytes);
int  vdl2hip_feed_device(vdl2hip_ctx *ctx, const void *dev_buf, size_t nbytes);

#ifndef VDL2HIP_MAX_DRAIN_LAG
#define VDL2HIP_MAX_DRAIN_LAG 5
#endif
int  vdl2hip_set_drain_lag(vdl2hip_ctx *ctx, int lag);

int  vdl2hip_sync(vdl2hip_ctx *ctx);
int  vdl2hip_drain(vdl2hip_ctx *ctx, vdl2hip_frame_cb cb, void *user);

typedef struct {
	vdl2hip_frame frame;
	uint64_t octets_off;
} vdl2hip_packed_frame;
int  vdl2hip_drain_packed(vdl2hip_ctx *ctx, vdl2hip_packed_frame *frames, size_t cap_frames,
		uint8_t *octets, size_t cap_octets, size_t *octets_used);

int  vdl2hip_pack_raw_frame(const vdl2hip_frame *frame, const char *station_id, int64_t tv_sec, int64_t tv_usec,
		uint8_t *out, size_t cap);

int  vdl2hip_counters(vdl2hip_ctx *ctx, uint32_t chan, uint64_t out[VDL2HIP_NUM_COUNTERS]);
int  vdl2hip_avlc_counters(vdl2hip_ctx *ctx, uint32_t chan, uint64_t out[VDL2HIP_NUM_AVLC_COUNTERS]);
int  vdl2hip_set_avlc_filter(vdl2hip_ctx *ctx, int on);
int  vdl2hip_statsd_lines(vdl2hip_ctx *ctx, const char *ns, char *out, size_t cap);
int  vdl2hip_set_profiling(vdl2hip_ctx *ctx, int level);
int  vdl2hip_get_stats(vdl2hip_ctx *ctx, vdl2hip_stats *out);
int  vdl2hip_get_stats_sized(vdl2hip_ctx *ctx, vdl2hip_stats *out, size_t size);
void *vdl2hip_stream(vdl2hip_ctx *ctx);

typedef struct vdl2hip_group vdl2hip_group;
enum { VDL2HIP_GROUP_ALLGATHER = 0, VDL2HIP_GROUP_BROADCAST = 1 };
int  vdl2hip_group_create(const vdl2hip_cfg *cfg, const int32_t *devices, uint32_t ndev, vdl2hip_group **out);
void vdl2hip_group_destroy(vdl2hip_group *g);
int  vdl2hip_group_feed(vdl2hip_group *g, const void *buf, size_t nbytes);
int  vdl2hip_group_feed_pinned(vdl2hip_group *g, const void *buf, size_t nbytes);
int  vdl2hip_group_sync(vdl2hip_group *g);
int  vdl2hip_group_drain(vdl2hip_group *g, vdl2hip_frame_cb cb, void *user);
int  vdl2hip_group_set_drain_lag(vdl2hip_group *g, int lag);
int  vdl2hip_group_counters(vdl2hip_group *g, uint32_t chan, uint64_t out[VDL2HIP_NUM_COUNTERS]);
int  vdl2hip_group_avlc_counters(vdl2hip_group *g, uint32_t chan, uint64_t out[VDL2HIP_NUM_AVLC_COUNTERS]);
uint32_t vdl2hip_group_size(vdl2hip_group *g);
vdl2hip_ctx *vdl2hip_group_ctx(vdl2hip_group *g, uint32_t member);
int  vdl2hip_group_uses_rccl(vdl2hip_group *g);
int  vdl2hip_group_set_exchange(vdl2hip_group *g, int form);
int  vdl2hip_group_exchange(vdl2hip_group *g);

int  vdl2hip_get_lpf(vdl2hip_ctx *ctx, float A[3], float B[3]);
int  vdl2hip_get_nco_step(vdl2hip_ctx *ctx, uint32_t chan, uint32_t *dphi);
int  vdl2hip_read_decimated(vdl2hip_ctx *ctx, uint32_t chan, int64_t first, float *dst, size_t cap);
int  vdl2hip_read_resampled(vdl2hip_ctx *ctx, int64_t first, float *dst, size_t cap);
int  vdl2hip_resampler_design(uint32_t input_rate, uint32_t output_rate, uint32_t *L, uint32_t *M, uint32_t *T, float *taps, size_t cap);

int  vdl2hip_spectrum_window(uint32_t nfft, uint32_t window, float *w, size_t cap);
int  vdl2hip_spectrum_enable(vdl2hip_ctx *ctx, const vdl2hip_spectrum_cfg *cfg);
int  vdl2hip_spectrum_read(vdl2hip_ctx *ctx, vdl2hip_spectrum_info *info, double *power, size_t cap, int reset);
int  vdl2hip_spectrum_channels(vdl2hip_ctx *ctx, float *dbfs, size_t cap);

int  vdl2hip_activity_edges(float *edges, size_t cap);
int  vdl2hip_activity_enable(vdl2hip_ctx *ctx, const vdl2hip_activity_cfg *cfg);
int  vdl2hip_activity_disable(vdl2hip_ctx *ctx);
int  vdl2hip_activity_read(vdl2hip_ctx *ctx, vdl2hip_activity_info *info, vdl2hip_activity_chan *chans, size_t cap_chans, int reset);
int  vdl2hip_activity_series(vdl2hip_ctx *ctx, uint32_t chan, int64_t first_bin, float *dst, size_t cap);

int  vdl2hip_capture_enable(vdl2hip_ctx *ctx, const vdl2hip_capture_cfg *cfg);
int  vdl2hip_capture_disable(vdl2hip_ctx *ctx);
int  vdl2hip_capture_info_get(vdl2hip_ctx *ctx, vdl2hip_capture_info *info);
int  vdl2hip_capture_read(vdl2hip_ctx *ctx, vdl2hip_burst *recs, size_t cap_recs, float *iq, size_t cap_pairs, size_t *pairs_used);

int  vdl2hip_txlog_enable(vdl2hip_ctx *ctx, const vdl2hip_txlog_cfg *cfg);
int  vdl2hip_txlog_disable(vdl2hip_ctx *ctx);
int  vdl2hip_txlog_info_get(vdl2hip_ctx *ctx, vdl2hip_txlog_info *info);
int  vdl2hip_txlog_read(vdl2hip_ctx *ctx, vdl2hip_tx *recs, size_t cap_recs);

// ... 5 lines not shown
```

Measured before the change: 5432.

## Pre-mark burst symbol windows and fold them into the earlier referee scan launch

Adds a k_burst_mark kernel that, before the referee scans run, walks the bursts and queues the symbol-window reference scans they will need. Those requests are appended as a second queue to the existing multi-scan launch. The burst decoder then checks whether all its windows are already done, and if so skips both deferral and the inline exact-window scans. The aim is to remove the deferred second burst pass and the inline scans by doing that work earlier in the existing scan stage. The cost is an extra marking kernel per feed, a larger scan grid, and new stats counters.

```diff
diff --git a/dumpvdl2_amd/csrc/debug_hooks.inc b/dumpvdl2_amd/csrc/debug_hooks.inc
--- a/dumpvdl2_amd/csrc/debug_hooks.inc
+++ b/dumpvdl2_amd/csrc/debug_hooks.inc
@@ -32,6 +32,7 @@
 	if(strcmp(name, "force_timeout") == 0) { c->debug_force_timeout = value != 0; return VDL2HIP_OK; }
 	if(strcmp(name, "force_mismatch") == 0) { c->debug_force_mismatch = value != 0; return VDL2HIP_OK; }
 	if(strcmp(name, "walk_ahead_below") == 0) { c->walk_ahead_below = (double)value; c->walk_ahead_auto = true; return VDL2HIP_OK; }
+	if(strcmp(name, "mark_cap") == 0) { if(value < 0 || value > (long long)kDeferScansMax) return VDL2HIP_E_INVAL; c->debug_mark_cap = (uint32_t)value; return VDL2HIP_OK; }
 	if(strcmp(name, "walk_ahead") == 0) { if(value != 0 && value != 1) return VDL2HIP_E_INVAL; c->walk_ahead = (int)value; c->walk_ahead_auto = false; return VDL2HIP_OK; }
 	if(strcmp(name, "exact_tier") == 0) { if(value != 0 && value != 1) return VDL2HIP_E_INVAL; c->debug_exact_tier = (int)value; return VDL2HIP_OK; }
 	if(strcmp(name, "screen_all") == 0) { c->debug_screen_all = value != 0; return VDL2HIP_OK; }
diff --git a/dumpvdl2_amd/csrc/kernels.h b/dumpvdl2_amd/csrc/kernels.h
--- a/dumpvdl2_amd/csrc/kernels.h
+++ b/dumpvdl2_amd/csrc/kernels.h
@@ -1081,7 +1081,7 @@
 #endif
 template<bool FULL>
 __global__ __launch_bounds__(256, 4) void k_sync_exact4(K3Args a) {
-	if(blockIdx.x == 0 && blockIdx.y == 0 && threadIdx.x == 0) { reset_out_ctl(a.ctl, a.k5_waves); if(a.ref) *a.ref = a.refv; if(a.rq_n) { a.rq_n[0] = 0u; a.rq_n[1] = 0u; a.rq_n[2] = 0u; a.rq_n[4] = 0u; a.rq_n[5] = 0u; a.rq_n[6] = 0u; } }
+	if(blockIdx.x == 0 && blockIdx.y == 0 && threadIdx.x == 0) { reset_out_ctl(a.ctl, a.k5_waves); if(a.ref) *a.ref = a.refv; if(a.rq_n) { a.rq_n[0] = 0u; a.rq_n[1] = 0u; a.rq_n[2] = 0u; a.rq_n[4] = 0u; a.rq_n[5] = 0u; a.rq_n[6] = 0u; a.rq_n[7] = 0u; } }
 	if(blockIdx.x == 0 && threadIdx.x == 0 && a.rq_flag) { a.rq_flag[blockIdx.y] = 0u; a.rq_bad[blockIdx.y].n = 0u; if(a.rq_flag2) a.rq_flag2[blockIdx.y] = 0u; }
 	constexpr int kBack = 160, kSpan = kBack + 64;
 	__shared__ float psh[4][64 + 6], fsh[4][64 + 6], esh[4][64 + 6], ash[4][64 + 6], bsh[4][64 + 6];
@@ -1221,7 +1221,7 @@
 #define K3D_BARRIER() do { __builtin_amdgcn_fence(__ATOMIC_RELEASE, "workgroup", "local"); __builtin_amdgcn_s_barrier(); __builtin_amdgcn_fence(__ATOMIC_ACQUIRE, "workgroup", "local"); } while(0)
 template<bool FULL>
 __global__ __launch_bounds__(256, 4) void k_sync_dense(K3Args a) {
-	if(blockIdx.x == 0 && blockIdx.y == 0 && threadIdx.x == 0) { reset_out_ctl(a.ctl, a.k5_waves); if(a.ref) *a.ref = a.refv; if(a.rq_n) { a.rq_n[0] = 0u; a.rq_n[1] = 0u; a.rq_n[2] = 0u; a.rq_n[4] = 0u; a.rq_n[5] = 0u; a.rq_n[6] = 0u; } }
+	if(blockIdx.x == 0 && blockIdx.y == 0 && threadIdx.x == 0) { reset_out_ctl(a.ctl, a.k5_waves); if(a.ref) *a.ref = a.refv; if(a.rq_n) { a.rq_n[0] = 0u; a.rq_n[1] = 0u; a.rq_n[2] = 0u; a.rq_n[4] = 0u; a.rq_n[5] = 0u; a.rq_n[6] = 0u; a.rq_n[7] = 0u; } }
 	if(blockIdx.x == 0 && threadIdx.x == 0 && a.rq_flag) { a.rq_flag[blockIdx.y] = 0u; a.rq_bad[blockIdx.y].n = 0u; if(a.rq_flag2) a.rq_flag2[blockIdx.y] = 0u; }
 	__shared__ uint64_t s_need[kK3dList], s_cbits[kK3dList], s_mbits[kK3dList];
 	__shared__ uint32_t s_end[kK3dList];
@@ -1601,12 +1601,13 @@
 };
 template<int FMT, int OS>
 __global__ __launch_bounds__(64 * kScanWaves) void k_ref_scan_multi(RefChan *rp, uint32_t launch, const ScanReq *sq, const RefReq *rq, const uint32_t *n_ptr, uint32_t cap, int64_t k_end,
-                      ScanReq *retry_q, uint32_t *retry_n, uint32_t retry_cap, int32_t warm_mul) {
+                      ScanReq *retry_q, uint32_t *retry_n, uint32_t retry_cap, int32_t warm_mul, const ScanReq *sq2, const uint32_t *n2_ptr, uint32_t cap2) {
 #if VDL2_DEVICE_PASS
 	#pragma clang fp contract(off)
 	__shared__ ScanShared sh;
 	constexpr int BLK = OS ? (kScanBlock / (OS ? OS : 1)) * OS : kScanBlock;
-	const uint32_t ntot = *n_ptr < cap ? *n_ptr : cap;
+	const uint32_t n1 = *n_ptr < cap ? *n_ptr : cap;
+	const uint32_t ntot = n1 + (sq2 ? (*n2_ptr < cap2 ? *n2_ptr : cap2) : 0u);
 	const uint32_t base = blockIdx.x * (uint32_t)kScanLanes;
 	if(base >= ntot) return;
 	const int wave = __builtin_amdgcn_readfirstlane(threadIdx.x >> 6), lane = threadIdx.x & 63;
@@ -1623,7 +1624,8 @@
 		const int r = threadIdx.x & (kScanLanes - 1), part = threadIdx.x >> 4;
 		int64_t n_lo = 0, n_hi = -1, s_beg = 0, len = 0; int c = 0, kind = 0; uint32_t fl = 0;
 		if(base + r < ntot && npiece > 0) {
-			if(sq) { const ScanReq q = sq[base + r]; c = q.chan; kind = q.kind; n_lo = q.lo; n_hi = q.hi; }
+			if(base + r >= n1) { const ScanReq q = sq2[base + r - n1]; c = q.chan; kind = q.kind; n_lo = q.lo; n_hi = q.hi; fl |= 4u; }
+			else if(sq) { const ScanReq q = sq[base + r]; c = q.chan; kind = q.kind; n_lo = q.lo; n_hi = q.hi; }
 			else { const RefReq q = rq[base + r]; c = q.chan; kind = q.kind; ref_request_window(q, k_end, n_lo, n_hi); }
 			const int64_t in_end = ps0[npiece - 1] + pn[npiece - 1];
 			if(n_lo < 0) n_lo = 0;
@@ -1900,9 +1902,10 @@
 		if(len >= 0) __hip_atomic_store(rp->done + (size_t)c * kRefCache + (i % (uint32_t)kRefCache), ((unsigned long long)(n_lo >> 8) << 32) | ((unsigned long long)len << 16) | (unsigned long long)(launch & 0xffffu), __ATOMIC_RELAXED, __HIP_MEMORY_SCOPE_AGENT);
 		atomicAdd(stats + 0, 1u); atomicAdd(stats + 4 + sh.kind[r], 1u);
 		if(sh.flags[r] & 2u) atomicAdd(stats + 3, 1u);
+		if(sh.flags[r] & 4u) atomicAdd(stats + 11, 1u);
 	}
 #else
-	(void)rp; (void)launch; (void)sq; (void)rq; (void)n_ptr; (void)cap; (void)k_end;
+	(void)rp; (void)launch; (void)sq; (void)rq; (void)n_ptr; (void)cap; (void)k_end; (void)sq2; (void)n2_ptr; (void)cap2;
 #endif
 }
 
@@ -1961,22 +1964,33 @@
 	}
 }
 
+__device__ __forceinline__ uint32_t burst_offsets(const uint32_t *nb_chan, int nchan, uint32_t *bb, int lane) {
+	uint32_t total = 0;
+	for(int c0 = 0; c0 < nchan; c0 += 64) {
+		const uint32_t v = c0 + lane < nchan ? nb_chan[c0 + lane] : 0u;
+		uint32_t inc = v;
+		#pragma unroll
+		for(int d = 1; d < 64; d <<= 1) { const uint32_t o = __shfl_up(inc, d); if(lane >= d) inc += o; }
+		if(c0 + lane < nchan) bb[c0 + lane] = total + inc - v;
+		total += __shfl(inc, 63);
+	}
+	if(lane == 0) bb[nchan] = total;
+	return total;
+}
+__device__ __forceinline__ int burst_chan_of(const uint32_t *bb, int nchan, uint32_t g) {
+	int lo = 0, hi = nchan;
+	while(hi - lo > 1) { const int mid = (lo + hi) >> 1; if(bb[mid] <= g) lo = mid; else hi = mid; }
+	return lo;
+}
+
 __device__ __forceinline__ void burst_body(const K5Args &a, unsigned char *k5_lds, uint32_t block, uint32_t nblocks) {
 	if((threadIdx.x >> 6) >= kBurstWaves) return;
 	BurstShared &sh = reinterpret_cast<BurstShared *>(k5_lds)[threadIdx.x >> 6];
 	uint32_t *bb = reinterpret_cast<uint32_t *>(k5_lds + sizeof(BurstShared) * kBurstWaves) + (size_t)(threadIdx.x >> 6) * (kK5MaxChan + 1);
 	const int lane = threadIdx.x & 63;
 	const uint32_t wave_id = block * kBurstWaves + (threadIdx.x >> 6);
-	uint32_t total = 0;
-	for(int c0 = 0; c0 < a.nchan; c0 += 64) {
-		const uint32_t v = c0 + lane < a.nchan ? a.nb_chan[c0 + lane] : 0u;
-		uint32_t inc = v;
-		#pragma unroll
-		for(int d = 1; d < 64; d <<= 1) { const uint32_t o = __shfl_up(inc, d); if(lane >= d) inc += o; }
-		if(c0 + lane < a.nchan) bb[c0 + lane] = total + inc - v;
-		total += __shfl(inc, 63);
-	}
-	if(lane == 0) { bb[a.nchan] = total; if(wave_id == 0 && a.df.pass != 2) a.ctl->nbursts = total; }
+	const uint32_t total = burst_offsets(a.nb_chan, a.nchan, bb, lane);
+	if(lane == 0 && wave_id == 0 && a.df.pass != 2) a.ctl->nbursts = total;
 	WAVE_SYNC();
 	if(a.df.pass == 2) {
 		const uint32_t nd = *a.df.dq_n < a.df.dq_cap ? *a.df.dq_n : a.df.dq_cap;
@@ -1984,9 +1998,7 @@
 		burst_shared_init(*a.tab, wave_id, a.ctl, sh, true);
 		for(uint32_t i = wave_id; i < nd; i += nblocks * kBurstWaves) {
 			const uint32_t g = a.df.dq[i];
-			int lo = 0, hi = a.nchan;
-			while(hi - lo > 1) { const int mid = (lo + hi) >> 1; if(bb[mid] <= g) lo = mid; else hi = mid; }
-			const int c = lo;
+			const int c = burst_chan_of(bb, a.nchan, g);
 			const Burst b = a.bursts[(size_t)c * a.cap_bursts_chan + (g - bb[c])];
 			ChanView v{ a.y + (size_t)c * a.cap, nullptr, nullptr, a.mask, a.ref, c, a.ref_launch };
 			decode_burst(b, a.freq[c], *a.tab, v, a.cnt + (size_t)c * kNumCounters, a.frames, a.pool, a.ctl, sh, &a.df, g);
@@ -2002,9 +2014,7 @@
 	}
 	burst_shared_init(*a.tab, wave_id, a.ctl, sh);
 	for(uint32_t g = wave_id; g < total; g += nblocks * kBurstWaves) {
-		int lo = 0, hi = a.nchan;
-		while(hi - lo > 1) { const int mid = (lo + hi) >> 1; if(bb[mid] <= g) lo = mid; else hi = mid; }
-		const int c = lo;
+		const int c = burst_chan_of(bb, a.nchan, g);
 		const Burst b = a.bursts[(size_t)c * a.cap_bursts_chan + (g - bb[c])];
 		ChanView v{ a.y + (size_t)c * a.cap, nullptr, nullptr, a.mask, a.ref, c, a.ref_launch };
 		decode_burst(b, a.freq[c], *a.tab, v, a.cnt + (size_t)c * kNumCounters, a.frames, a.pool, a.ctl, sh, a.df.pass ? &a.df : nullptr, g);
@@ -2016,6 +2026,50 @@
 __global__ __launch_bounds__(256, 4) void k_burst(K5Args a) {
 	extern __shared__ __align__(16) unsigned char k5_lds[];
 	burst_body(a, k5_lds, blockIdx.x, gridDim.x);
+}
+
+struct K5mArgs {
+	const cf32 *y; const Burst *bursts; const uint32_t *nb_chan; uint32_t cap_bursts_chan; int32_t nchan;
+	uint32_t cap, mask; RefChan *ref; uint32_t ref_launch;
+	ScanReq *mq; uint32_t *mq_n; uint32_t mq_cap;
+};
+__global__ __launch_bounds__(256, 4) void k_burst_mark(K5mArgs a) {
+	extern __shared__ __align__(16) unsigned char k5_lds[];
+	if((threadIdx.x >> 6) >= kBurstWaves) return;
+	BurstShared &sh = reinterpret_cast<BurstShared *>(k5_lds)[threadIdx.x >> 6];
+	uint32_t *bb = reinterpret_cast<uint32_t *>(k5_lds + sizeof(BurstShared) * kBurstWaves) + (size_t)(threadIdx.x >> 6) * (kK5MaxChan + 1);
+	const int lane = threadIdx.x & 63;
+	const uint32_t wave_id = blockIdx.x * kBurstWaves + (threadIdx.x >> 6);
+	const uint32_t total = burst_offsets(a.nb_chan, a.nchan, bb, lane);
+	WAVE_SYNC();
+	for(uint32_t g = wave_id; g < total; g += gridDim.x * kBurstWaves) {
+		const int c = burst_chan_of(bb, a.nchan, g);
+		const Burst b = a.bursts[(size_t)c * a.cap_bursts_chan + (g - bb[c])];
+		ChanView v{ a.y + (size_t)c * a.cap, nullptr, nullptr, a.mask, a.ref, c, a.ref_launch };
+		BurstMarks mk;
+		burst_mark(b, v, sh, mk);
+		if(mk.mfirst != 0xffffffffu) {
+			uint32_t pm[4] = { sh.u_pm[0], sh.u_pm[1], sh.u_pm[2], sh.u_pm[3] };
+			for(int q = 0; q < 128; q++) {
+				if(!((pm[q >> 5] >> (q & 31)) & 1u)) continue;
+				int64_t lo_, hi_;
+				burst_piece_range(mk, q, q, lo_, hi_);
+				if(ref_window_done(v, lo_, hi_)) pm[q >> 5] &= ~(1u << (q & 31));
+			}
+			if(lane == 0) {
+				const uint32_t np = (uint32_t)(popc32(pm[0]) + popc32(pm[1]) + popc32(pm[2]) + popc32(pm[3]));
+				uint32_t j = np ? atomicAdd(a.mq_n, np) : 0u;
+				for(int q = 0; q < 128; q++) {
+					if(!((pm[q >> 5] >> (q & 31)) & 1u)) continue;
+					int64_t lo_, hi_;
+					burst_piece_range(mk, q, q, lo_, hi_);
+					if(j < a.mq_cap) a.mq[j] = ScanReq{ c, REF_SYMBOLS, lo_, hi_ };
+					j++;
+				}
+			}
+		}
+		WAVE_SYNC();
+	}
 }
 
 static_assert(kNfWaves >= kBurstWaves, "a workgroup of the joint launch holds either kind");
diff --git a/dumpvdl2_amd/csrc/vdl2_core.h b/dumpvdl2_amd/csrc/vdl2_core.h
--- a/dumpvdl2_amd/csrc/vdl2_core.h
+++ b/dumpvdl2_amd/csrc/vdl2_core.h
@@ -2111,24 +2111,22 @@
 
 constexpr int kRefPieceBits = 10;
 struct ScanReq { int32_t chan, kind; int64_t lo, hi; };
-struct BurstDefer { uint32_t *dq, *dq_n; uint32_t dq_cap; ScanReq *sq; uint32_t *sq_n; uint32_t sq_cap; int32_t pass; };
-
-VDL2_HD __attribute__((always_inline)) void decode_burst(const Burst &b, uint32_t freq, const Tables &T, const ChanView &v, unsigned long long *cnt,
-		OutFrame *frames, uint8_t *pool, OutCtl *ctl, BurstShared &sh, const BurstDefer *df = nullptr, uint32_t tag = 0) {
-	const uint32_t octets = b.tl_bits / 8 + (b.tl_bits % 8 != 0);
-	uint32_t nblk = octets / kRsK, last = octets % kRsK;
-	uint32_t fec = nblk * kRsPar;
-	if(last != 0) nblk++;
-	fec += (uint32_t)fec_octets_for(last);
-	if(last == 0) last = kRsK;
-	const int npar_last = fec_octets_for(last);
+struct BurstDefer { uint32_t *dq, *dq_n; uint32_t dq_cap; ScanReq *sq; uint32_t *sq_n; uint32_t sq_cap; int32_t pass; uint32_t *late_n = nullptr; };
+
+struct BurstMarks { uint32_t mfirst, mlast; bool redo_slope, wide; int64_t w_lo, hi, P0; };
+VDL2_HD void burst_piece_range(const BurstMarks &mk, int q, int q1, int64_t &lo_, int64_t &hi_) {
+	lo_ = (mk.P0 + q) << kRefPieceBits; hi_ = ((mk.P0 + q1 + 1) << kRefPieceBits) - 1;
+	if(mk.wide) { lo_ = mk.w_lo; hi_ = mk.hi; }
+	if(lo_ < mk.w_lo) lo_ = mk.w_lo;
+	if(hi_ > mk.hi) hi_ = mk.hi;
+}
+VDL2_HD __attribute__((always_inline)) void burst_mark(const Burst &b, const ChanView &v, BurstShared &sh, BurstMarks &mk) {
 	const int nsym = b.nsym;
-	K5_BEGIN();
-
 	const int per_lane = (nsym + 63) / 64;
 	const bool ref_on = v.ref != nullptr;
-	float vdphi = b.vdphi, ppm = b.ppm;
+	const float vdphi = b.vdphi;
 	const float verr = fabsf(b.vdphi_err);
+	mk.mfirst = 0xffffffffu; mk.mlast = 0u; mk.redo_slope = false; mk.wide = false; mk.w_lo = 0; mk.hi = -1; mk.P0 = 0;
 	WAVE_FOR(l)
 		float pw = 0.f; int neg = 0; float qmin = kRefBig;
 		const int m0 = l * per_lane, m1 = m0 + per_lane < nsym ? m0 + per_lane : nsym;
@@ -2204,7 +2202,7 @@
 			const int64_t w_lo = (redo_slope && s_lo < t_lo) ? (s_lo < 0 ? 0 : s_lo) : t_lo;
 			const int64_t P0 = w_lo >> kRefPieceBits;
 			const bool wide = (hi >> kRefPieceBits) - P0 >= 128;
-			const int pass = df ? df->pass : 0;
+			mk.mfirst = mfirst; mk.mlast = mlast; mk.redo_slope = redo_slope; mk.wide = wide; mk.w_lo = w_lo; mk.hi = hi; mk.P0 = P0;
 			LANE0
 				uint32_t pm[4] = { 0u, 0u, 0u, 0u };
 				if(wide) pm[0] = 1u;
@@ -2219,8 +2217,40 @@
 					}
 				}
 				for(int i = 0; i < 4; i++) sh.u_pm[i] = pm[i];
+			LANE0_END
+		}
+	}
+}
+
+VDL2_HD __attribute__((always_inline)) void decode_burst(const Burst &b, uint32_t freq, const Tables &T, const ChanView &v, unsigned long long *cnt,
+		OutFrame *frames, uint8_t *pool, OutCtl *ctl, BurstShared &sh, const BurstDefer *df = nullptr, uint32_t tag = 0) {
+	const uint32_t octets = b.tl_bits / 8 + (b.tl_bits % 8 != 0);
+	uint32_t nblk = octets / kRsK, last = octets % kRsK;
+	uint32_t fec = nblk * kRsPar;
+	if(last != 0) nblk++;
+	fec += (uint32_t)fec_octets_for(last);
+	if(last == 0) last = kRsK;
+	const int npar_last = fec_octets_for(last);
+	K5_BEGIN();
+
+	float vdphi = b.vdphi, ppm = b.ppm;
+	BurstMarks mk;
+	burst_mark(b, v, sh, mk);
+	{
+		const uint32_t mfirst = mk.mfirst, mlast = mk.mlast;
+		if(mfirst != 0xffffffffu) {
+			const bool redo_slope = mk.redo_slope;
+			const int pass = df ? df->pass : 0;
+			bool ahead = pass == 1;
+			for(int q = 0; q < 128 && ahead; q++) {
+				if(!((sh.u_pm[q >> 5] >> (q & 31)) & 1u)) continue;
+				int64_t lo_, hi_;
+				burst_piece_range(mk, q, q, lo_, hi_);
+				ahead = ref_window_done(v, lo_, hi_);
+			}
+			LANE0
 				sh.u_defer = 0;
-				if(pass == 1) {
+				if(pass == 1 && !ahead) {
 #if VDL2_DEVICE_PASS
 					const uint32_t i = atomicAdd(df->dq_n, 1u);
 #else
@@ -2229,18 +2259,18 @@
 					if(i < df->dq_cap) {
 						df->dq[i] = tag; sh.u_defer = 1;
 						uint32_t np = 0;
-						for(int q = 0; q < 4; q++) np += (uint32_t)popc32(pm[q]);
+						for(int q = 0; q < 4; q++) np += (uint32_t)popc32(sh.u_pm[q]);
 #if VDL2_DEVICE_PASS
 						uint32_t j = atomicAdd(df->sq_n, np);
+						if(df->late_n) atomicAdd(df->late_n, np);
 #else
 						uint32_t j = *df->sq_n; *df->sq_n += np;
+						if(df->late_n) *df->late_n += np;
 #endif
 						for(int q = 0; q < 128; q++) {
-							if(!((pm[q >> 5] >> (q & 31)) & 1u)) continue;
-							int64_t lo_ = (P0 + q) << kRefPieceBits, hi_ = ((P0 + q + 1) << kRefPieceBits) - 1;
-							if(wide) { lo_ = w_lo; hi_ = hi; }
-							if(lo_ < w_lo) lo_ = w_lo;
-							if(hi_ > hi) hi_ = hi;
+							if(!((sh.u_pm[q >> 5] >> (q & 31)) & 1u)) continue;
+							int64_t lo_, hi_;
+							burst_piece_range(mk, q, q, lo_, hi_);
 							if(j < df->sq_cap) df->sq[j] = ScanReq{ v.ref_chan, REF_SYMBOLS, lo_, hi_ };
 							j++;
 						}
@@ -2250,14 +2280,12 @@
 			if(sh.u_defer) { K5_END(); return; }
 			bool ok = true;
 			{
-				for(int q = 0; q < 128 && ok; ) {
+				for(int q = 0; q < 128 && ok && !ahead; ) {
 					if(!((sh.u_pm[q >> 5] >> (q & 31)) & 1u)) { q++; continue; }
 					int q1 = q;
 					if(pass != 2) while(q1 + 1 < 128 && ((sh.u_pm[(q1 + 1) >> 5] >> ((q1 + 1) & 31)) & 1u)) q1++;
-					int64_t lo_ = (P0 + q) << kRefPieceBits, hi_ = ((P0 + q1 + 1) << kRefPieceBits) - 1;
-					if(wide) { lo_ = w_lo; hi_ = hi; }
-					if(lo_ < w_lo) lo_ = w_lo;
-					if(hi_ > hi) hi_ = hi;
+					int64_t lo_, hi_;
+					burst_piece_range(mk, q, q1, lo_, hi_);
 					ok = ref_exact_window(v, lo_, hi_, sh.xw, REF_SYMBOLS);
 					q = q1 + 1;
 				}
diff --git a/dumpvdl2_amd/csrc/vdl2hip.hip b/dumpvdl2_amd/csrc/vdl2hip.hip
--- a/dumpvdl2_amd/csrc/vdl2hip.hip
+++ b/dumpvdl2_amd/csrc/vdl2hip.hip
@@ -93,6 +93,7 @@
 	DevBuf<OutFrame> d_frames_out; DevBuf<uint8_t> d_pool_out;
 	DevBuf<EvalChunk> d_log; DevBuf<uint32_t> d_nlog;
 	DevBuf<uint32_t> d_dq; DevBuf<ScanReq> d_sq;
+	DevBuf<ScanReq> d_mq;
 	DevBuf<RefReq> d_rq; DevBuf<uint32_t> d_rqn, d_rqflag; DevBuf<RefBad> d_rqbad;
 	DevBuf<ScanReq> d_retry;
 	DevBuf<ScanReq> d_pq; Event ev_pre;
@@ -182,7 +183,7 @@
 	bool referee = true; bool ref_prescan = false;    int64_t ref_warm = 3 << 16 , ref_T = 0; DevBuf<uint8_t> d_refhist; uint64_t ref_cap = 0, ref_wp = 0;
 	struct HistPiece { int64_t s0, n; uint64_t pos; }; std::vector<HistPiece> ref_pieces;
 	DevBuf<WalkState> d_ws_snap[2], d_ws_tmp; DevBuf<unsigned long long> d_cnt_snap[2], d_cnt_tmp; uint32_t rq_cap = 8192; uint32_t sq_alloc = 8192;
-	int walk_ahead = 1; bool walk_ahead_auto = true; double walk_ahead_below = 1.1e8; int debug_force_mismatch = 0;
+	int walk_ahead = 1; bool walk_ahead_auto = true; double walk_ahead_below = 1.1e8; int debug_force_mismatch = 0; uint32_t debug_mark_cap = 0;
 	int ref_retry_mul = 2;
 	DevBuf<RefChan> d_ref[kSlots]; DevBuf<unsigned long long> d_refdone; DevBuf<uint32_t> d_refdonen, d_refstats; DevBuf<uint8_t> d_mix;
 	std::vector<uint64_t> statsd_prev;
@@ -605,12 +606,12 @@
 	else if(c->fmt == 3) { if(c->os == 20) how((k_ref_scan_multi<3, 20>), __VA_ARGS__); else if(c->os == 10) how((k_ref_scan_multi<3, 10>), __VA_ARGS__); else how((k_ref_scan_multi<3, 0>), __VA_ARGS__); } \
 	else { if(c->os == 20) how((k_ref_scan_multi<0, 20>), __VA_ARGS__); else if(c->os == 10) how((k_ref_scan_multi<0, 10>), __VA_ARGS__); else how((k_ref_scan_multi<0, 0>), __VA_ARGS__); } } while(0)
 static void launch_scans(vdl2hip_ctx *c, hipStream_t st, RefChan *ref, uint32_t launch, const ScanReq *sq, const RefReq *rq, const uint32_t *n, uint32_t cap, int64_t k_end,
-                         ScanReq *retry, uint32_t *retry_n, hipEvent_t e0 = nullptr, hipEvent_t e1 = nullptr) {
+                         ScanReq *retry, uint32_t *retry_n, hipEvent_t e0 = nullptr, hipEvent_t e1 = nullptr, const ScanReq *sq2 = nullptr, const uint32_t *n2 = nullptr, uint32_t cap2 = 0) {
 	const int rty = retry ? c->ref_retry_mul : 0;
-	LAUNCH_SCAN_MULTI(hipExtLaunchKernelGGL, dim3((cap + kScanLanes - 1) / kScanLanes), dim3(64 * kScanWaves), 0, st, e0, rty ? (hipEvent_t) nullptr : e1, 0, ref, launch,
-	                  sq, rq, n, cap, k_end, rty ? retry : (ScanReq *) nullptr, retry_n, kRetryScans, 1);
+	LAUNCH_SCAN_MULTI(hipExtLaunchKernelGGL, dim3((cap + (sq2 ? cap2 : 0u) + kScanLanes - 1) / kScanLanes), dim3(64 * kScanWaves), 0, st, e0, rty ? (hipEvent_t) nullptr : e1, 0, ref, launch,
+	                  sq, rq, n, cap, k_end, rty ? retry : (ScanReq *) nullptr, retry_n, kRetryScans, 1, sq2, n2, sq2 ? cap2 : 0u);
 	if(rty) LAUNCH_SCAN_MULTI(hipExtLaunchKernelGGL, dim3(kRetryScans / kScanLanes), dim3(64 * kScanWaves), 0, st, (hipEvent_t) nullptr, e1, 0, ref, launch,
-	                  (const ScanReq *)retry, (const RefReq *) nullptr, (const uint32_t *)retry_n, kRetryScans, k_end, (ScanReq *) nullptr, (uint32_t *) nullptr, 0u, rty);
+	                  (const ScanReq *)retry, (const RefReq *) nullptr, (const uint32_t *)retry_n, kRetryScans, k_end, (ScanReq *) nullptr, (uint32_t *) nullptr, 0u, rty, (const ScanReq *) nullptr, (const uint32_t *) nullptr, 0u);
 }
 static int launch_rest(vdl2hip_ctx *c, OutSlot &sl, OutSlot *succ);
 static void launch_stitch(vdl2hip_ctx *c, hipStream_t st, const OutSlot &sl, const K4Args &k4, int again, hipEvent_t e1 = nullptr) {
@@ -671,8 +672,15 @@
 		if(k4.rq) {
 			sl.has_chk = true;
 			hipStream_t sc_ = wa ? sp_ : sb_;
+			uint32_t mq_cap = small ? kDeferScans / 16 : std::min(c->sq_alloc, defer_scans_for(D, c->C));
+			if(c->debug_mark_cap) mq_cap = std::min(mq_cap, c->debug_mark_cap);
+			{
+				K5mArgs k5m{ c->d_y, sl.d_bursts, sl.d_nbchan, c->cap_bursts_chan, c->C, c->cap, c->cap - 1, k4.ref, k4.ref_launch - 1u, sl.d_mq, sl.d_rqn + 7, mq_cap };
+				const unsigned k5_lds = (unsigned)((sizeof(BurstShared) + 4 * (kK5MaxChan + 1)) * kBurstWaves);
+				hipLaunchKernelGGL(k_burst_mark, dim3(sl.k5_waves / kBurstWaves), dim3(64 * kBurstWaves), k5_lds, sb_, k5m);
+			}
 			if(sc_ != sb_) { HIPCHK(hipEventRecord(sl.ev_stitch, sb_)); HIPCHK(hipStreamWaitEvent(sc_, sl.ev_stitch, 0)); }
-			launch_scans(c, sc_, k4.ref, k4.ref_launch - 1u, nullptr, k4.rq, k4.rq_n, rq_cap, k1, sl.d_retry + kRetryScans, sl.d_rqn + 5);
+			launch_scans(c, sc_, k4.ref, k4.ref_launch - 1u, nullptr, k4.rq, k4.rq_n, rq_cap, k1, sl.d_retry + kRetryScans, sl.d_rqn + 5, nullptr, nullptr, sl.d_mq, sl.d_rqn + 7, mq_cap);
 			hipLaunchKernelGGL(k_ref_verify, dim3(small ? 64 : 1024), dim3(64), 0, sc_, k4);
 			HIPCHK(hipEventRecord(sl.ev_chk, sc_));
 		}
@@ -888,7 +896,7 @@
 		           sl.d_frames, sl.d_pool, sl.d_ctl, c->d_freq, c->cap, c->cap - 1, c->referee ? c->d_ref[sl.seq % kSlots] : nullptr, (uint32_t)(16 * sl.seq + 5), BurstDefer{} };
 		const bool defer5 = c->referee;
 		const uint32_t sq_cap = small ? kDeferScans / 16 : std::min(c->sq_alloc, defer_scans_for(D, c->C)), dq_cap = sq_cap / 2;
-		if(defer5) k5.df = BurstDefer{ sl.d_dq, sl.d_rqn + 1, dq_cap, sl.d_sq, sl.d_rqn + 2, sq_cap, 1 };
+		if(defer5) k5.df = BurstDefer{ sl.d_dq, sl.d_rqn + 1, dq_cap, sl.d_sq, sl.d_rqn + 2, sq_cap, 1, c->d_refstats + 12 };
 		const unsigned k5_lds = (unsigned)((sizeof(BurstShared) + 4 * (kK5MaxChan + 1)) * kBurstWaves);
 		hipEvent_t ev_last5 = defer5 ? (hipEvent_t) nullptr : EV(11);
 		if(small) hipExtLaunchKernelGGL(k_nf_burst, dim3(nf_grid + sl.k5_waves / kBurstWaves), dim3(64 * kNfWaves), std::max(nf_lds, k5_lds), s5_, EV(8), ev_last5, 0, k4b, k5, (uint32_t)nf_grid);
@@ -1137,7 +1145,7 @@
 		c->sq_alloc = defer_scans_for((int64_t)dmax, (int)count);
 		for(auto &sl : c->slot) {
 			DEV_ALLOC(sl.d_rq, c->rq_cap); DEV_ALLOC(sl.d_rqn, 8, true); DEV_ALLOC(sl.d_retry, 3 * (size_t)kRetryScans); DEV_ALLOC(sl.d_rqflag, count, true);
-			DEV_ALLOC(sl.d_dq, c->sq_alloc / 2); DEV_ALLOC(sl.d_sq, c->sq_alloc);
+			DEV_ALLOC(sl.d_dq, c->sq_alloc / 2); DEV_ALLOC(sl.d_sq, c->sq_alloc); DEV_ALLOC(sl.d_mq, c->sq_alloc);
 			DEV_ALLOC(sl.d_pq, kPreScans); DEV_CHK(sl.ev_pre.ensure(hipEventDisableTiming));
 			DEV_ALLOC(sl.d_rqbad, count, true);
 			DEV_ALLOC(sl.d_rqflag2, count, true);
@@ -1422,10 +1430,11 @@
 		for(int i = 0; i < c->C; i++) { c->stats.seg_adopted += ss[2 * i]; c->stats.seg_walked += ss[2 * i + 1]; }
 	}
 	if(c->d_refstats) {
-		uint32_t rs[11] = {0, 0, 0, 0, 0, 0, 0, 0, 0, 0, 0};
+		uint32_t rs[13] = {0, 0, 0, 0, 0, 0, 0, 0, 0, 0, 0, 0, 0};
 		if(hipMemcpy(rs, c->d_refstats, sizeof rs, hipMemcpyDeviceToHost) != hipSuccess) return VDL2HIP_E_DEVICE;
 		c->stats.referee_scans = rs[0]; c->stats.referee_cached = rs[1]; c->stats.referee_refused = rs[2]; c->stats.referee_short = rs[3];
 		c->stats.referee_candidate_scans = rs[4]; c->stats.referee_header_scans = rs[5]; c->stats.referee_symbol_scans = rs[6]; c->stats.referee_rewalks = rs[7]; c->stats.referee_redone_next = rs[8]; c->stats.referee_unmet = rs[9]; c->stats.referee_retried = rs[10];
+		c->stats.referee_symbol_pieces_ahead = rs[11]; c->stats.referee_symbol_pieces_late = rs[12];
 	}
 	memcpy(out, &c->stats, std::min(size, sizeof c->stats));
 	return (r == VDL2HIP_E_OVERFLOW || c->failed) ? VDL2HIP_OK : r;
diff --git a/dumpvdl2_amd/vdl2hip.py b/dumpvdl2_amd/vdl2hip.py
--- a/dumpvdl2_amd/vdl2hip.py
+++ b/dumpvdl2_amd/vdl2hip.py
@@ -74,7 +74,8 @@
                 ("referee_scans", C.c_uint64), ("referee_cached", C.c_uint64), ("referee_refused", C.c_uint64), ("referee_short", C.c_uint64), ("referee_rewalks", C.c_uint64),
                 ("referee_candidate_scans", C.c_uint64), ("referee_header_scans", C.c_uint64), ("referee_symbol_scans", C.c_uint64),
                 ("referee_redone_next", C.c_uint64), ("referee_unmet", C.c_uint64), ("referee_retried", C.c_uint64),
-                ("resampled_samples", C.c_uint64), ("resample_ms", C.c_double)]
+                ("resampled_samples", C.c_uint64), ("resample_ms", C.c_double),
+                ("referee_symbol_pieces_ahead", C.c_uint64), ("referee_symbol_pieces_late", C.c_uint64)]
 
 
 class SpectrumCfg(C.Structure):
diff --git a/include/vdl2hip.h b/include/vdl2hip.h
--- a/include/vdl2hip.h
+++ b/include/vdl2hip.h
@@ -195,6 +195,8 @@
 	uint64_t referee_retried;
 	uint64_t resampled_samples;
 	double   resample_ms;
+	uint64_t referee_symbol_pieces_ahead;
+	uint64_t referee_symbol_pieces_late;
 } vdl2hip_stats;
 
 int  vdl2hip_abi_version(void);
```

Result: faster. 5754 (median of 6 runs) (+5.9%).
